# vismaychuriwala/Fast-Image-Editing-with-Generative-Models

Hardware: AMD Instinct MI355X
Metric: PIE-Bench images/sec @1024^2 SSD-1B fp16 4-step (higher is better)
Workload: dtype f16; 1 GPU; ssd-1b fp16 + ControlNet-Canny(full) LCM img2img, num_inference_steps=4, strength=0.5, guidance=1.5, 1024x1024, batch=1 image per GPU, one edit at a time; unet_preset=ssd-1b-A1, controlnet_preset=controlnet-canny-sdxl-full, unet_evals=2, cfg_batch=2, parallelism=image-parallel x1, launch=hipGraph replay, weights=f16

## Files before the change

fast-image-editing-with-generative-models_amd/csrc/gemm_common.h:

```cpp
#pragma once
#include "fie_internal.h"
#include "gemm_addr.h"

namespace fie_gemm {

constexpr int BK = 64;

struct GemmArgs {
    const half_t* A1; int64_t lda1; int K1;
    const half_t* A2; int64_t lda2;
    const half_t* A3; int64_t lda3; int C2x, C3x; int64_t a3_bytes;
    int H, W, Cin, OH, OW, stride, pt, pl, ups;
    const half_t* Wt; int64_t ldw;
    half_t* C; int64_t ldc;
    int M, N, K;
    const half_t* bias;
    const half_t* rowbias; int64_t ld_rowbias; int rows_per_batch;
    const half_t* res; int64_t ldr;
    float scale; int act;
    int nbm, nbn;
    int64_t a1_bytes, a2_bytes, w_bytes;
    int taps2, oscat, opy, opx;
    int64_t w_par_stride;
    int gn_nch, gn_chunk0;
    float* gn_partial; int gn_rows, gn_G, gn_cg;
    const float* w_scale;
    unsigned* stamps;
    int epi_prefetch;
    int probe;
    int splitk; float* sk_slabs; unsigned* sk_tickets;
    float a_scale; int out_f8; float out_inv_scale;
    int order;
    int frag_ld;
    const float* ln_tab; float ln_eps;
    const float* gna_tab; int gna_silu;
};

__device__ __forceinline__ int take_parity(GemmArgs& p, int bid) {
    if (p.oscat != 2) return bid;
    const int par = bid & 3;
    p.opy = par >> 1; p.opx = par & 1; p.pt = 1 - p.opy; p.pl = 1 - p.opx;
    p.Wt += (int64_t)par * p.w_par_stride;
    p.gn_chunk0 = par * ((p.OH * p.OW) >> 5);
    return bid >> 2;
}

__host__ __device__ __forceinline__ ConvGeom conv_geom(const GemmArgs& p, int taps2) { return {p.M, p.OH, p.OW, p.H, p.W, p.Cin, p.stride, p.pt, p.pl, p.ups, taps2}; }

constexpr int kBufRsrcFlags = 0x00020000;
__device__ __forceinline__ __amdgpu_buffer_rsrc_t buf_rsrc(const void* ptr, int64_t bytes) {
    return __builtin_amdgcn_make_buffer_rsrc(const_cast<void*>(ptr), 0, (int)bytes, kBufRsrcFlags);
}

template <class F, int... I>
__device__ __forceinline__ void static_for(F&& f, std::integer_sequence<int, I...>) { (f(std::integral_constant<int, I>{}), ...); }

__device__ __forceinline__ int lds_off(int row, int chunk) { return row * BK + ((chunk ^ (row & 7)) << 3); }

typedef unsigned u32x2 __attribute__((ext_vector_type(2)));

__device__ __forceinline__ float row16_sum(float v) {
    v += __builtin_bit_cast(float, __builtin_amdgcn_update_dpp(0, __builtin_bit_cast(int, v), 0xB1, 0xF, 0xF, true));
    v += __builtin_bit_cast(float, __builtin_amdgcn_update_dpp(0, __builtin_bit_cast(int, v), 0x4E, 0xF, 0xF, true));
    v += __builtin_bit_cast(float, __builtin_amdgcn_update_dpp(0, __builtin_bit_cast(int, v), 0x141, 0xF, 0xF, true));
    v += __builtin_bit_cast(float, __builtin_amdgcn_update_dpp(0, __builtin_bit_cast(int, v), 0x140, 0xF, 0xF, true));
    return v;
}

template <int FM, int FN>
struct EpiPre {
    u32x2 bias[FN];
    u32x2 res[FM][FN];
    bool on;
};
template <int FM, int FN, int WM, int WN>
__device__ __forceinline__ void epilogue_prefetch(const GemmArgs& p, EpiPre<FM, FN>& pre, int m0, int n0, int wm, int wn, int lane) {
    const int fr = lane & 15, fq = lane >> 4;
    const int mrow = m0 + wm * WM + fr, ncol = n0 + wn * WN + fq * 4;
    pre.on = true;
#pragma unroll
    for (int i = 0; i < FN; ++i) pre.bias[i] = (u32x2){0u, 0u};
#pragma unroll
    for (int j = 0; j < FM; ++j)
#pragma unroll
        for (int i = 0; i < FN; ++i) pre.res[j][i] = (u32x2){0u, 0u};
    if (p.bias) {
        const __amdgpu_buffer_rsrc_t rb = buf_rsrc(p.bias, p.N * 2);
#pragma unroll
        for (int i = 0; i < FN; ++i) pre.bias[i] = __builtin_amdgcn_raw_buffer_load_b64(rb, (unsigned)(ncol + i * 16) * 2u, 0, 0);
    }
    if (p.res) {
        const __amdgpu_buffer_rsrc_t rs = buf_rsrc(p.res, (int)(((int64_t)(p.M - 1) * p.ldr + p.N) * 2));
#pragma unroll
        for (int j = 0; j < FM; ++j) {
            const int m = mrow + j * 16;
            const unsigned ro = m < p.M ? (unsigned)m * (unsigned)p.ldr * 2u : 0x80000000u;
#pragma unroll
            for (int i = 0; i < FN; ++i) {
                const int n = ncol + i * 16;
                pre.res[j][i] = __builtin_amdgcn_raw_buffer_load_b64(rs, ro + (n < p.N ? (unsigned)n << 1 : 0xC0000000u), 0, 0);
            }
        }
    }
}

template <int FM, int FN, int WM, int WN>
__device__ __forceinline__ void epilogue_lean(const GemmArgs& p, f32x4 (&acc)[FN][FM], int m0, int n0, int wm, int wn, int lane, const EpiPre<FM, FN>& pre) {
    const int fr = lane & 15, fq = lane >> 4;
    const int mrow = m0 + wm * WM + fr, ncol = n0 + wn * WN + fq * 4;
    const __amdgpu_buffer_rsrc_t rs_c = buf_rsrc(p.C, (int)(((int64_t)(p.M - 1) * p.ldc + p.N) * 2));
#pragma unroll
    for (int j = 0; j < FM; ++j) {
        const int m = mrow + j * 16;
        const unsigned ro = m < p.M ? (unsigned)m * (unsigned)p.ldc * 2u : 0x80000000u;
#pragma unroll
        for (int i = 0; i < FN; ++i) {
            const int n = ncol + i * 16;
            f16x4 b, r, o;
            __builtin_memcpy(&b, &pre.bias[i], 8);
            __builtin_memcpy(&r, &pre.res[j][i], 8);
#pragma unroll
            for (int q = 0; q < 4; ++q) o[q] = (half_t)(acc[i][j][q] + (float)b[q] + (float)r[q]);
            u32x2 bits;
            __builtin_memcpy(&bits, &o, 8);
            __builtin_amdgcn_raw_buffer_store_b64(bits, rs_c, ro + (n < p.N ? (unsigned)n << 1 : 0xC0000000u), 0, 0);
        }
    }
}

template <int FM, int FN, int WM, int WN>
__device__ __forceinline__ void epilogue_lean_scaled(const GemmArgs& p, f32x4 (&acc)[FN][FM], int m0, int n0, int wm, int wn, int lane, const EpiPre<FM, FN>& pre,
                                                     const f32x4 (&ws)[FN]) {
    const int fr = lane & 15, fq = lane >> 4;
    const int mrow = m0 + wm * WM + fr, ncol = n0 + wn * WN + fq * 4;
    const __amdgpu_buffer_rsrc_t rs_c = buf_rsrc(p.C, (int)(((int64_t)(p.M - 1) * p.ldc + p.N) * 2));
#pragma unroll
    for (int j = 0; j < FM; ++j) {
        const int m = mrow + j * 16;
        const unsigned ro = m < p.M ? (unsigned)m * (unsigned)p.ldc * 2u : 0x80000000u;
#pragma unroll
        for (int i = 0; i < FN; ++i) {
            const int n = ncol + i * 16;
            f16x4 b, r, o;
            __builtin_memcpy(&b, &pre.bias[i], 8);
            __builtin_memcpy(&r, &pre.res[j][i], 8);
#pragma unroll
            for (int q = 0; q < 4; ++q) o[q] = (half_t)((acc[i][j][q] * (ws[i][q] * p.a_scale) + (float)b[q]) + (float)r[q]);
            u32x2 bits;
            __builtin_memcpy(&bits, &o, 8);
            __builtin_amdgcn_raw_buffer_store_b64(bits, rs_c, ro + (n < p.N ? (unsigned)n << 1 : 0xC0000000u), 0, 0);
        }
    }
}

__device__ __forceinline__ void ln_dot(const f16x8& f, float& s, float& q) {
    const f16x2 one = {(half_t)1.f, (half_t)1.f};
#pragma unroll
    for (int t = 0; t < 4; ++t) {
        const f16x2 v = {f[2 * t], f[2 * t + 1]};
        s = __builtin_amdgcn_fdot2(v, one, s, false);
        q = __builtin_amdgcn_fdot2(v, v, q, false);
    }
}

template <int FN>
struct LnTab { f32x4 lo[FN], hi[FN]; };
__device__ __forceinline__ void ln_tab_load(const GemmArgs& p, int n, f32x4& lo, f32x4& hi) {
    const __amdgpu_buffer_rsrc_t rt = buf_rsrc(p.ln_tab, p.N * 8);
    lo = __builtin_bit_cast(f32x4, __builtin_amdgcn_raw_buffer_load_b128(rt, (unsigned)n * 8u, 0, 0));
    hi = __builtin_bit_cast(f32x4, __builtin_amdgcn_raw_buffer_load_b128(rt, (unsigned)n * 8u + 16u, 0, 0));
}

template <int FM, int FN, int WM, int WN>
__device__ __forceinline__ void epilogue_lean_ln(const GemmArgs& p, f32x4 (&acc)[FN][FM], int m0, int n0, int wm, int wn, int lane, const LnTab<FN>& tab,
                                                 const float (&mean)[FM], const float (&rstd)[FM]) {
    const int fr = lane & 15, fq = lane >> 4;
    const int mrow = m0 + wm * WM + fr, ncol = n0 + wn * WN + fq * 4;
    const __amdgpu_buffer_rsrc_t rs_c = buf_rsrc(p.C, (int)(((int64_t)(p.M - 1) * p.ldc + p.N) * 2));
#pragma unroll
    for (int j = 0; j < FM; ++j) {
        const int m = mrow + j * 16;
        const unsigned ro = m < p.M ? (unsigned)m * (unsigned)p.ldc * 2u : 0x80000000u;
#pragma unroll
        for (int i = 0; i < FN; ++i) {
            const int n = ncol + i * 16;
            f16x4 o;
            o[0] = (half_t)((acc[i][j][0] - mean[j] * tab.lo[i][0]) * rstd[j] + tab.lo[i][1]);
            o[1] = (half_t)((acc[i][j][1] - mean[j] * tab.lo[i][2]) * rstd[j] + tab.lo[i][3]);
            o[2] = (half_t)((acc[i][j][2] - mean[j] * tab.hi[i][0]) * rstd[j] + tab.hi[i][1]);
            o[3] = (half_t)((acc[i][j][3] - mean[j] * tab.hi[i][2]) * rstd[j] + tab.hi[i][3]);
            u32x2 bits;
            __builtin_memcpy(&bits, &o, 8);
            __builtin_amdgcn_raw_buffer_store_b64(bits, rs_c, ro + (n < p.N ? (unsigned)n << 1 : 0xC0000000u), 0, 0);
        }
    }
}

template <int FM, int FN, int WM, int WN, bool LN = false>
__device__ __forceinline__ void epilogue_geglu_lean(const GemmArgs& p, f32x4 (&acc)[FN][FM], int m0, int n0, int wm, int wn, int lane,
                                                    const float* mean = nullptr, const float* rstd = nullptr) {
    static_assert(FM % 4 == 0, "left-over fragment columns are transposed over four row fragments");
    const int fr = lane & 15, fq = lane >> 4;
    const int mrow = m0 + wm * WM + fr, nbase = n0 + wn * WN;
    const __amdgpu_buffer_rsrc_t rs_c = buf_rsrc(p.C, (int)(((int64_t)(p.M - 1) * p.ldc + (p.N >> 1)) * 2));
    const __amdgpu_buffer_rsrc_t rs_b = buf_rsrc(p.bias, p.bias ? p.N * 2 : 0);
    auto bias4 = [&](int i) { return __builtin_amdgcn_raw_buffer_load_b64(rs_b, (unsigned)(nbase + i * 16 + fq * 4) * 2u, 0, 0); };
    auto pair = [&](const f32x4& a, u32x2 bb) {
        f16x4 b;
        __builtin_memcpy(&b, &bb, 8);
        f16x2 o;
        o[0] = (half_t)((a[0] + (float)b[0]) * fie_gelu(a[1] + (float)b[1]) * 1.0f);
        o[1] = (half_t)((a[2] + (float)b[2]) * fie_gelu(a[3] + (float)b[3]) * 1.0f);
        unsigned bits;
        __builtin_memcpy(&bits, &o, 4);
        return bits;
    };
    auto transpose4 = [](unsigned& r0, unsigned& r1, unsigned& r2, unsigned& r3) {
        asm volatile("s_nop 1\n\tv_permlane16_swap_b32 %0, %1" : "+v"(r0), "+v"(r1));
        asm volatile("s_nop 1\n\tv_permlane16_swap_b32 %0, %1" : "+v"(r2), "+v"(r3));
        asm volatile("s_nop 1\n\tv_permlane32_swap_b32 %0, %1" : "+v"(r0), "+v"(r2));
        asm volatile("s_nop 1\n\tv_permlane32_swap_b32 %0, %1" : "+v"(r1), "+v"(r3));
    };
    auto rowoff = [&](int m) { return m < p.M ? (unsigned)m * (unsigned)p.ldc * 2u : 0x80000000u; };
    struct Tab { f32x4 lo, hi; };
    auto tab4 = [&](int i) { Tab t; ln_tab_load(p, nbase + i * 16 + fq * 4, t.lo, t.hi); return t; };
    auto pair_ln = [&](const f32x4& a, const Tab& t, int j) {
        const float mu = mean[j], rs = rstd[j];
        f16x2 o;
        o[0] = (half_t)(((a[0] - mu * t.lo[0]) * rs + t.lo[1]) * fie_gelu((a[1] - mu * t.lo[2]) * rs + t.lo[3]) * 1.0f);
        o[1] = (half_t)(((a[2] - mu * t.hi[0]) * rs + t.hi[1]) * fie_gelu((a[3] - mu * t.hi[2]) * rs + t.hi[3]) * 1.0f);
        unsigned bits;
        __builtin_memcpy(&bits, &o, 4);
        return bits;
    };
    static_for([&](auto gc) {
        constexpr int I0 = 4 * decltype(gc)::value;
        const int nst = nbase + (I0 + fq) * 16;
        const unsigned co = nst < p.N ? (unsigned)nst : 0xC0000000u;
        if constexpr (LN) {
            const Tab t0 = tab4(I0), t1 = tab4(I0 + 1), t2 = tab4(I0 + 2), t3 = tab4(I0 + 3);
#pragma unroll
            for (int j = 0; j < FM; ++j) {
                unsigned r0 = pair_ln(acc[I0][j], t0, j), r1 = pair_ln(acc[I0 + 1][j], t1, j), r2 = pair_ln(acc[I0 + 2][j], t2, j), r3 = pair_ln(acc[I0 + 3][j], t3, j);
                transpose4(r0, r1, r2, r3);
                const u32x4 v = {r0, r1, r2, r3};
                __builtin_amdgcn_raw_buffer_store_b128(v, rs_c, rowoff(mrow + j * 16) + co, 0, 0);
            }
        } else {
            const u32x2 b0 = bias4(I0), b1 = bias4(I0 + 1), b2 = bias4(I0 + 2), b3 = bias4(I0 + 3);
#pragma unroll
            for (int j = 0; j < FM; ++j) {
                unsigned r0 = pair(acc[I0][j], b0), r1 = pair(acc[I0 + 1][j], b1), r2 = pair(acc[I0 + 2][j], b2), r3 = pair(acc[I0 + 3][j], b3);
                transpose4(r0, r1, r2, r3);
                const u32x4 v = {r0, r1, r2, r3};
                __builtin_amdgcn_raw_buffer_store_b128(v, rs_c, rowoff(mrow + j * 16) + co, 0, 0);
            }
        }
    }, std::make_integer_sequence<int, FN / 4>{});
    static_for([&](auto ic) {
        constexpr int I = FN / 4 * 4 + decltype(ic)::value;
        const int n = nbase + I * 16;
        const unsigned co = n < p.N ? (unsigned)n : 0xC0000000u;
        if constexpr (LN) {
            const Tab t = tab4(I);
#pragma unroll
            for (int h = 0; h < FM / 4; ++h) {
                unsigned r0 = pair_ln(acc[I][4 * h], t, 4 * h), r1 = pair_ln(acc[I][4 * h + 1], t, 4 * h + 1), r2 = pair_ln(acc[I][4 * h + 2], t, 4 * h + 2), r3 = pair_ln(acc[I][4 * h + 3], t, 4 * h + 3);
                transpose4(r0, r1, r2, r3);
                const u32x4 v = {r0, r1, r2, r3};
                __builtin_amdgcn_raw_buffer_store_b128(v, rs_c, rowoff(mrow + (4 * h + fq) * 16) + co, 0, 0);
            }
        } else {
            const u32x2 b = bias4(I);
#pragma unroll
            for (int h = 0; h < FM / 4; ++h) {
                unsigned r0 = pair(acc[I][4 * h], b), r1 = pair(acc[I][4 * h + 1], b), r2 = pair(acc[I][4 * h + 2], b), r3 = pair(acc[I][4 * h + 3], b);
                transpose4(r0, r1, r2, r3);
                const u32x4 v = {r0, r1, r2, r3};
                __builtin_amdgcn_raw_buffer_store_b128(v, rs_c, rowoff(mrow + (4 * h + fq) * 16) + co, 0, 0);
            }
        }
    }, std::make_integer_sequence<int, FN % 4>{});
}

template <int FM, int FN, int WM, int WN, bool BUF = false, bool PATCH = false>
__device__ __forceinline__ void epilogue(const GemmArgs& p, f32x4 (&acc)[FN][FM], int m0, int n0, int wm, int wn, int lane, const EpiPre<FM, FN>* pre = nullptr) {
    const int fr = lane & 15, fq = lane >> 4;
    const bool have_pre = pre != nullptr && pre->on;
    if (p.probe == 4 && p.M > 0) return;
    const bool geglu = p.act == FIE_ACT_GEGLU;
    const int fld = PATCH ? p.frag_ld : 16;
    const int mrow = m0 + wm * FM * fld + fr, ncol = n0 + wn * WN + fq * 4;
    auto col = [&](int i) { const int n = ncol + i * 16; return n < p.N ? n : p.N - 4; };
    auto row = [&](int j) { const int m = mrow + j * fld; return m < p.M ? m : p.M - 1; };
    constexpr unsigned kRowOut = 0x80000000u, kColOut = 0xC0000000u;
    auto coff = [&](int i, bool half) { const int n = ncol + i * 16; return n < p.N ? (unsigned)n << (half ? 0 : 1) : kColOut; };
    auto roff = [&](int j, int64_t ld) { const int m = mrow + j * fld; return m < p.M ? (unsigned)m * (unsigned)ld * 2u : kRowOut; };
    auto coff_row = [&](int j) {
        const int m = mrow + j * fld;
        if (m >= p.M) return kRowOut;
        if (!p.oscat) return (unsigned)m * (unsigned)p.ldc * 2u;
        const OutPixel o = out_pixel(p.OH, p.OW, m);
        return (unsigned)((o.b * 2 * p.OH + 2 * o.oh + p.opy) * (2 * p.OW) + 2 * o.ow + p.opx) * (unsigned)p.ldc * 2u;
    };
    auto as_h4 = [](u32x2 v) { f16x4 h; __builtin_memcpy(&h, &v, 8); return h; };

    if (p.w_scale) {
        const float as = p.a_scale != 0.f ? p.a_scale : 1.f;
#pragma unroll
        for (int i = 0; i < FN; ++i) {
            float4 ws = *reinterpret_cast<const float4*>(p.w_scale + col(i));
            ws.x *= as; ws.y *= as; ws.z *= as; ws.w *= as;
#pragma unroll
            for (int j = 0; j < FM; ++j) { acc[i][j][0] *= ws.x; acc[i][j][1] *= ws.y; acc[i][j][2] *= ws.z; acc[i][j][3] *= ws.w; }
        }
    }
    if (p.bias) {
        f16x4 b[FN];
#pragma unroll
        for (int i = 0; i < FN; ++i) b[i] = have_pre ? as_h4(pre->bias[i]) : *reinterpret_cast<const f16x4*>(p.bias + col(i));
#pragma unroll
        for (int i = 0; i < FN; ++i)
#pragma unroll
            for (int j = 0; j < FM; ++j)
#pragma unroll
                for (int r = 0; r < 4; ++r) acc[i][j][r] += (float)b[i][r];
    }
    if (p.rowbias) {
#pragma unroll
        for (int j = 0; j < FM; ++j) {
            const half_t* rb = p.rowbias + (int64_t)(row(j) / p.rows_per_batch) * p.ld_rowbias;
            f16x4 b[FN];
#pragma unroll
            for (int i = 0; i < FN; ++i) b[i] = *reinterpret_cast<const f16x4*>(rb + col(i));
#pragma unroll
            for (int i = 0; i < FN; ++i)
#pragma unroll
                for (int r = 0; r < 4; ++r) acc[i][j][r] += (float)b[i][r];
        }
    }
    auto sweep = [&](auto f) {
#pragma unroll
        for (int i = 0; i < FN; ++i)
#pragma unroll
            for (int j = 0; j < FM; ++j)
#pragma unroll
                for (int r = 0; r < 4; ++r) acc[i][j][r] = f(acc[i][j][r]) * p.scale;
    };
    if (geglu) {
#pragma unroll
        for (int i = 0; i < FN; ++i)
#pragma unroll
            for (int j = 0; j < FM; ++j) {
                acc[i][j][0] = acc[i][j][0] * fie_gelu(acc[i][j][1]) * p.scale;
                acc[i][j][1] = acc[i][j][2] * fie_gelu(acc[i][j][3]) * p.scale;
            }
    } else if (p.act == FIE_ACT_SILU) sweep([](float x) { return fie_silu(x); });
    else if (p.act == FIE_ACT_GELU) sweep([](float x) { return fie_gelu(x); });
    else if (p.act == FIE_ACT_QUICK_GELU) sweep([](float x) { return fie_qgelu(x); });
    else if (p.scale != 1.f) sweep([](float x) { return x; });
    if (p.res) {
        const __amdgpu_buffer_rsrc_t rs = buf_rsrc(p.res, BUF ? ((int64_t)(p.M - 1) * p.ldr + p.N) * 2 : 0);
#pragma unroll
        for (int j = 0; j < FM; ++j) {
            f16x4 b[FN];
            if (have_pre) {
#pragma unroll
                for (int i = 0; i < FN; ++i) b[i] = as_h4(pre->res[j][i]);
            } else if constexpr (BUF) {
                const unsigned ro = roff(j, p.ldr);
#pragma unroll
                for (int i = 0; i < FN; ++i) b[i] = as_h4(__builtin_amdgcn_raw_buffer_load_b64(rs, ro + coff(i, false), 0, 0));
            } else {
                const half_t* rr = p.res + (int64_t)row(j) * p.ldr;
#pragma unroll
                for (int i = 0; i < FN; ++i) b[i] = *reinterpret_cast<const f16x4*>(rr + col(i));
            }
#pragma unroll
            for (int i = 0; i < FN; ++i)
#pragma unroll
                for (int r = 0; r < 4; ++r) acc[i][j][r] += (float)b[i][r];
            if (FM * FN > 16) __builtin_amdgcn_sched_barrier(0);
        }
    }
    if (p.gn_partial) {
        static_assert(FM % 2 == 0, "row granules are two fragments");
        const int nch = p.gn_nch ? p.gn_nch : p.gn_rows >> 5;
#pragma unroll
        for (int jj = 0; jj < FM / 2; ++jj) {
            float sum[FN], sq[FN];
#pragma unroll
            for (int i = 0; i < FN; ++i) sum[i] = sq[i] = 0.f;
#pragma unroll
            for (int dj = 0; dj < 2; ++dj) {
                const bool ok = mrow + (2 * jj + dj) * fld < p.M;
#pragma unroll
                for (int i = 0; i < FN; ++i)
#pragma unroll
                    for (int r = 0; r < 4; ++r) {
                        const float x = ok ? (float)(half_t)acc[i][2 * jj + dj][r] : 0.f;
                        sum[i] += x;
                        sq[i] += x * x;
                    }
            }
            const int mg = m0 + (wm * FM + 2 * jj) * fld;
            const int b = mg / p.gn_rows, rem = mg - b * p.gn_rows;
            const int chunk = p.gn_chunk0 + (PATCH ? ((rem / p.frag_ld) >> 1) * (p.frag_ld >> 4) + ((rem % p.frag_ld) >> 4) : rem >> 5);
#pragma unroll
            for (int i = 0; i < FN; ++i) {
                const float rs = row16_sum(sum[i]), rq = row16_sum(sq[i]);
                float ts[4], tq[4];
#pragma unroll
                for (int k = 0; k < 4; ++k) {
                    ts[k] = __builtin_bit_cast(float, __builtin_amdgcn_readlane(__builtin_bit_cast(int, rs), 16 * k));
                    tq[k] = __builtin_bit_cast(float, __builtin_amdgcn_readlane(__builtin_bit_cast(int, rq), 16 * k));
                }
                if (p.gn_cg == 16) { ts[0] = (ts[0] + ts[1]) + (ts[2] + ts[3]); tq[0] = (tq[0] + tq[1]) + (tq[2] + tq[3]); }
                else if (p.gn_cg == 8) { ts[0] += ts[1]; tq[0] += tq[1]; ts[1] = ts[2] + ts[3]; tq[1] = tq[2] + tq[3]; }
                const int ngrp = 16 / p.gn_cg;
                const int nfrag = n0 + wn * WN + i * 16;
                if (lane < ngrp && mg < p.M && nfrag + lane * p.gn_cg < p.N) {
                    const float vs = lane == 0 ? ts[0] : lane == 1 ? ts[1] : lane == 2 ? ts[2] : ts[3];
                    const float vq = lane == 0 ? tq[0] : lane == 1 ? tq[1] : lane == 2 ? tq[2] : tq[3];
                    float2* dst = reinterpret_cast<float2*>(p.gn_partial) + ((int64_t)b * nch + chunk) * p.gn_G + nfrag / p.gn_cg + lane;
                    *dst = make_float2(vs, vq);
                }
            }
        }
    }
    if constexpr (BUF) {
        if (p.out_f8) {
            const __amdgpu_buffer_rsrc_t rs8 = buf_rsrc(p.C, (int64_t)(p.M - 1) * p.ldc + (geglu ? p.N >> 1 : p.N));
            const float inv = p.out_inv_scale;
            auto q = [&](float x) { return fie_sat448(x * inv); };
#pragma unroll
            for (int j = 0; j < FM; ++j) {
                const int m = mrow + j * fld;
                const unsigned ro = m < p.M ? (unsigned)m * (unsigned)p.ldc : kRowOut;
#pragma unroll
                for (int i = 0; i < FN; ++i) {
                    const int n = ncol + i * 16;
                    if (geglu) {
                        const int pk = __builtin_amdgcn_cvt_pk_fp8_f32(q(acc[i][j][0]), q(acc[i][j][1]), 0, false);
                        __builtin_amdgcn_raw_buffer_store_b16((unsigned short)(pk & 0xffff), rs8, ro + (n < p.N ? (unsigned)(n >> 1) : kColOut), 0, 0);
                    } else {
                        int pk = __builtin_amdgcn_cvt_pk_fp8_f32(q(acc[i][j][0]), q(acc[i][j][1]), 0, false);
                        pk = __builtin_amdgcn_cvt_pk_fp8_f32(q(acc[i][j][2]), q(acc[i][j][3]), pk, true);
                        __builtin_amdgcn_raw_buffer_store_b32((unsigned)pk, rs8, ro + (n < p.N ? (unsigned)n : kColOut), 0, 0);
                    }
                }
            }
            return;
        }
    }
    const __amdgpu_buffer_rsrc_t rs_c = buf_rsrc(p.C, BUF ? ((int64_t)(p.oscat ? 4 * (int64_t)p.M : p.M) - 1) * p.ldc * 2 + (geglu ? p.N >> 1 : p.N) * 2 : 0);
#pragma unroll
    for (int j = 0; j < FM; ++j) {
        const int m = mrow + j * fld;
        const unsigned ro = coff_row(j);
#pragma unroll
        for (int i = 0; i < FN; ++i) {
            const int n = ncol + i * 16;
            if (geglu) {
                f16x2 o;
                o[0] = (half_t)acc[i][j][0]; o[1] = (half_t)acc[i][j][1];
                if constexpr (BUF) {
                    unsigned bits; __builtin_memcpy(&bits, &o, 4);
                    __builtin_amdgcn_raw_buffer_store_b32(bits, rs_c, ro + coff(i, true), 0, 0);
                } else if (m < p.M && n < p.N) {
                    *reinterpret_cast<f16x2*>(p.C + (int64_t)m * p.ldc + (n >> 1)) = o;
                }
            } else {
                f16x4 o;
#pragma unroll
                for (int r = 0; r < 4; ++r) o[r] = (half_t)acc[i][j][r];
                if constexpr (BUF) {
                    u32x2 bits; __builtin_memcpy(&bits, &o, 8);
                    __builtin_amdgcn_raw_buffer_store_b64(bits, rs_c, ro + coff(i, false), 0, 0);
                } else if (m < p.M && n < p.N) {
                    *reinterpret_cast<f16x4*>(p.C + (int64_t)m * p.ldc + n) = o;
                }
            }
        }
        __builtin_amdgcn_sched_barrier(0);
    }
}

constexpr unsigned kOob = 0x80000000u;

__device__ __forceinline__ void bload16(__amdgpu_buffer_rsrc_t rsrc, half_t* lds_dst, unsigned voff, unsigned soff) {
    __builtin_amdgcn_raw_ptr_buffer_load_lds(rsrc, (__attribute__((address_space(3))) void*)lds_dst, 16, voff, soff, 0, 0);
}

template <int N>
__device__ __forceinline__ void wait_vm() {
    static_assert(N >= 0 && N < 64, "vmcnt is a 6-bit counter");
    asm volatile("s_waitcnt vmcnt(%0)" ::"n"(N) : "memory");
}

template <int N>
__device__ __forceinline__ void wait_vm_barrier() {
    static_assert(N >= 0 && N < 64, "vmcnt is a 6-bit counter");
    asm volatile("s_waitcnt vmcnt(%0)\n\ts_barrier" ::"n"(N) : "memory");
}

template <int FM, int FN, int NW>
__device__ __forceinline__ bool splitk_reduce(const GemmArgs& p, f32x4 (&acc)[FN][FM], int tile, int slice, int tid, void* lds) {
    constexpr int kTile = FM * FN * NW * 64 * 4;
    const int S = p.splitk;
    float* base = p.sk_slabs + (size_t)tile * S * kTile;
    {
        const __amdgpu_buffer_rsrc_t rs = buf_rsrc(base + (size_t)slice * kTile, kTile * 4);
// ... 60 lines not shown
```

fast-image-editing-with-generative-models_amd/csrc/gemm_conv.hip:

```cpp
#include <algorithm>
#include <cstdio>
#include <cstdlib>
#include <cstring>
#include <utility>

#include "gemm_common.h"
#include "gemm_tiles.h"

using namespace fie_gemm;

namespace {

template <int BM, int BN, int MODE>
__global__ __launch_bounds__(256) void gemm_kernel(GemmArgs p) {
    constexpr int WM = BM / 2, WN = BN / 2;
    constexpr int FM = WM / 16, FN = WN / 16;
    constexpr int RA = BM / 32, RW = BN / 32;
    __shared__ __attribute__((aligned(16))) half_t smem[2 * (BM + BN) * BK];

    const int tid = threadIdx.x;
    const int lane = tid & 63, wave = tid >> 6;
    const int wm = wave & 1, wn = wave >> 1;

    const int bid = xcd_remap(blockIdx.x, gridDim.x);
// ... 40 lines not shown
            while (ci >= p.Cin) { ci -= p.Cin; ++tap; }
        } else {
            const bool k1 = k < p.K1;
            const half_t* src = k1 ? p.A1 : p.A2;
            const int64_t ld = k1 ? p.lda1 : p.lda2;
            const int kk = k1 ? k : k - p.K1;
#pragma unroll
            for (int i = 0; i < RA; ++i) {
                const bool ok = a_row[i].ok && k < p.K;
                ra[i] = ok ? *reinterpret_cast<const f16x8*>(src + a_base[i] * ld + kk) : zero8;
            }
        }
#pragma unroll
        for (int i = 0; i < RW; ++i)
            rw[i] = *reinterpret_cast<const f16x8*>(p.Wt + (int64_t)(n0 + r0 + 32 * i) * p.ldw + k);
    };
    auto store_tiles = [&](int buf) {
        half_t* sa = smem + buf * (BM + BN) * BK;
        half_t* sw = sa + BM * BK;
#pragma unroll
        for (int i = 0; i < RA; ++i) *reinterpret_cast<f16x8*>(sa + lds_off(r0 + 32 * i, c8)) = ra[i];
#pragma unroll
        for (int i = 0; i < RW; ++i) *reinterpret_cast<f16x8*>(sw + lds_off(r0 + 32 * i, c8)) = rw[i];
    };

    f32x4 acc[FN][FM];
#pragma unroll
    for (int i = 0; i < FN; ++i)
#pragma unroll
        for (int j = 0; j < FM; ++j) acc[i][j] = (f32x4){0.f, 0.f, 0.f, 0.f};

    const int nk = (p.K + BK - 1) / BK;
    load_tiles(0);
    store_tiles(0);
    __syncthreads();

    const int fr = lane & 15, fq = lane >> 4;
    for (int kt = 0; kt < nk; ++kt) {
        const int buf = kt & 1;
        if (kt + 1 < nk) load_tiles(kt + 1);
        const half_t* sa = smem + buf * (BM + BN) * BK;
        const half_t* sw = sa + BM * BK;
#pragma unroll
        for (int kk = 0; kk < 2; ++kk) {
            f16x8 fw[FN], fa[FM];
#pragma unroll
            for (int i = 0; i < FN; ++i)
                fw[i] = *reinterpret_cast<const f16x8*>(sw + lds_off(wn * WN + i * 16 + fr, kk * 4 + fq));
#pragma unroll
            for (int j = 0; j < FM; ++j)
                fa[j] = *reinterpret_cast<const f16x8*>(sa + lds_off(wm * WM + j * 16 + fr, kk * 4 + fq));
#pragma unroll
            for (int i = 0; i < FN; ++i)
#pragma unroll
                for (int j = 0; j < FM; ++j)
                    acc[i][j] = __builtin_amdgcn_mfma_f32_16x16x32_f16(fw[i], fa[j], acc[i][j], 0, 0, 0);
        }
        if (kt + 1 < nk) store_tiles(buf ^ 1);
        __syncthreads();
    }

    epilogue<FM, FN, WM, WN>(p, acc, m0, n0, wm, wn, lane);
}

template <int NP, int ST>
__device__ __forceinline__ void wait_stage(int later) {
    if (ST >= 3 && later >= 1) wait_vm_barrier<(ST >= 3 ? 1 : 0) * NP>();
    else wait_vm_barrier<0>();
}

template <int OFF>
__device__ __forceinline__ f16x8 lds_read16_async(unsigned addr) {
    f16x8 v;
    asm volatile("ds_read_b128 %0, %1 offset:%2" : "=v"(v) : "v"(addr), "n"(OFF));
    return v;
}
template <int N, int... I>
__device__ __forceinline__ void read_frags(f16x8 (&f)[N], unsigned addr, std::integer_sequence<int, I...>) {
    ((f[I] = lds_read16_async<I * 16 * BK * 2>(addr)), ...);
}

template <int BM, int BN, int ST, int MODE, int NW, bool PF = false, bool STAMP = false, bool ALT = false, int LEAN = 0>
__global__ __launch_bounds__(NW * 64) void gemm3_kernel(GemmArgs p) {
    constexpr bool LNF = LEAN == 2;
    static_assert(!LNF || (MODE == 0 && !STAMP), "LayerNorm fold: GEMM view only");
    static_assert(!ALT || (NW == 8 && MODE == 0 && !PF && !STAMP), "ALT: 8-wave GEMM-view tiles without the fragment prefetch");
    constexpr int WGN = (LEAN == 2 && BM * BN / (NW * 256) <= 16 && (BM / NW) % 16 == 0) ? 1 : (BN / (NW / 2)) % 16 == 0 ? NW / 2 : 1, WGM = NW / WGN;
    constexpr int WM = BM / WGM, WN = BN / WGN;
    constexpr int FM = WM / 16, FN = WN / 16;
    constexpr int NPW = BN / 8;
    constexpr int RA = BM / (8 * NW), RW = (NPW + NW - 1) / NW;
    constexpr int NP = RA + RW;
    constexpr int STAGE = (BM + BN) * BK;
    extern __shared__ __attribute__((aligned(16))) half_t smem[];

    const int tid = threadIdx.x;
    const int lane = tid & 63;
    const int wave = __builtin_amdgcn_readfirstlane(tid >> 6);
    const int wm = wave % WGM, wn = wave / WGM;

    const int bid_all = xcd_remap(blockIdx.x, gridDim.x);
    const int nsplit = p.splitk > 1 ? p.splitk : 1;
    const int tile_all = bid_all / nsplit, slice = bid_all - tile_all * nsplit;
    const int bid = take_parity(p, tile_all);
    const int m0 = (p.order ? bid % p.nbm : bid / p.nbn) * BM;
    const int n0 = (p.order ? bid / p.nbm : bid % p.nbn) * BN;
    const int lr = lane >> 3;
    const int c8 = (lane & 7) ^ lr;

    const int live = p.probe == 1 ? 0 : 1;
    const __amdgpu_buffer_rsrc_t rs_a1 = buf_rsrc(p.A1, (int)p.a1_bytes * live);
    const __amdgpu_buffer_rsrc_t rs_a2 = buf_rsrc(p.A2, (int)p.a2_bytes * live);
    const __amdgpu_buffer_rsrc_t rs_w = buf_rsrc(p.Wt, (int)p.w_bytes * live);
    const __amdgpu_buffer_rsrc_t rs_a3 = buf_rsrc(p.A3, (int)p.a3_bytes * live);
    const int lm0 = p.probe == 2 ? 0 : m0, ln0 = p.probe == 2 ? 0 : n0;

    unsigned a_off1[RA], a_off2[RA];
    unsigned a_off3[RA];
    const ConvGeom g = conv_geom(p, p.taps2);
    ConvRow a_row[RA];
    unsigned a_img[RA];
#pragma unroll
    for (int i = 0; i < RA; ++i) {
        const int m = lm0 + (wave + NW * i) * 8 + lr;
        if (MODE == 2) {
            a_row[i] = conv_row(g, m);
            a_img[i] = (unsigned)a_row[i].b * (unsigned)(p.H * p.W) * (unsigned)p.Cin * 2u;
            a_off1[i] = kOob;
            a_off2[i] = a_row[i].ok ? (unsigned)m * (unsigned)p.lda2 * 2u + c8 * 16u : kOob;
            a_off3[i] = a_row[i].ok ? (unsigned)m * (unsigned)p.lda3 * 2u + c8 * 16u : kOob;
        } else {
            a_off1[i] = a_off2[i] = a_off3[i] = a_img[i] = 0;
            a_row[i] = ConvRow{};
        }
    }
    const unsigned a_base1 = (unsigned)(lm0 + wave * 8 + lr) * (unsigned)p.lda1 * 2u + c8 * 16u;
    const unsigned a_base2 = (unsigned)(lm0 + wave * 8 + lr) * (unsigned)p.lda2 * 2u + c8 * 16u;
    const unsigned a_step1 = (unsigned)(NW * 8) * (unsigned)p.lda1 * 2u, a_step2 = (unsigned)(NW * 8) * (unsigned)p.lda2 * 2u;
    const unsigned w_base = (unsigned)(ln0 + wave * 8 + lr) * (unsigned)p.ldw * 2u + c8 * 16u;
    const unsigned w_step = (unsigned)(NW * 8) * (unsigned)p.ldw * 2u;

    const int csteps = MODE == 2 ? p.Cin / BK : 1;
    const int k1_steps = p.K1 / BK;
    const int nk_all = (p.K + BK - 1) / BK;
    const KSlice ks(nk_all, slice, nsplit, csteps);
    const int kbeg = ks.kbeg, nk = ks.nk;
    const bool ktail = (p.K % BK) != 0;
    int ftap = ks.ftap, cs = ks.cs;
    bool tap_fresh = true;

    const int ntaps = conv_taps(g);
    auto issue = [&](int kt, int stage) {
        half_t* sa = smem + stage * STAGE;
        if (MODE == 2 && ftap >= ntaps) {
            const int e = kt - ntaps * csteps, x2 = p.C2x / BK;
            if (e < x2) {
#pragma unroll
                for (int i = 0; i < RA; ++i) bload16(rs_a2, sa + (wave + NW * i) * 512, a_off2[i], (unsigned)e * (BK * 2));
            } else {
#pragma unroll
                for (int i = 0; i < RA; ++i) bload16(rs_a3, sa + (wave + NW * i) * 512, a_off3[i], (unsigned)(e - x2) * (BK * 2));
            }
        } else if (MODE == 2) {
            if (cs == 0 || tap_fresh) {
                tap_fresh = false;
                const TapYX t = tap_yx(g, ftap);
#pragma unroll
                for (int i = 0; i < RA; ++i)
                    a_off1[i] = conv_inside(g, a_row[i], t.ky, t.kx) ? a_img[i] + (unsigned)conv_index(g, a_row[i], t.ky, t.kx) * (unsigned)p.Cin * 2u + c8 * 16u : kOob;
            }
            const unsigned so = (unsigned)cs * (BK * 2);
#pragma unroll
            for (int i = 0; i < RA; ++i) bload16(rs_a1, sa + (wave + NW * i) * 512, a_off1[i], so);
            if (++cs == csteps) { cs = 0; ++ftap; }
        } else {
            if (ktail && kt == nk_all - 1) {
                const bool in_k = kt * BK + c8 * 8 < p.K;
#pragma unroll
                for (int i = 0; i < RA; ++i) bload16(rs_a1, sa + (wave + NW * i) * 512, in_k ? a_base1 + (unsigned)i * a_step1 : kOob, (unsigned)kt * (BK * 2));
            } else if (kt < k1_steps || k1_steps == 0) {
                const unsigned so = (unsigned)kt * (BK * 2);
#pragma unroll
                for (int i = 0; i < RA; ++i) bload16(rs_a1, sa + (wave + NW * i) * 512, a_base1 + (unsigned)i * a_step1, so);
            } else {
                const unsigned so = (unsigned)(kt - k1_steps) * (BK * 2);
#pragma unroll
                for (int i = 0; i < RA; ++i) bload16(rs_a2, sa + (wave + NW * i) * 512, a_base2 + (unsigned)i * a_step2, so);
            }
        }
    };
    auto issue_w = [&](int kt, int stage) {
        half_t* sw = smem + stage * STAGE + BM * BK;
        const unsigned sow = (unsigned)kt * (BK * 2);
#pragma unroll
        for (int i = 0; i < RW; ++i) {
            const int ii = (NPW % NW == 0 || wave + NW * i < NPW) ? i : 0;
            bload16(rs_w, sw + (wave + NW * ii) * 512, w_base + (unsigned)ii * w_step, sow);
        }
    };

    const int grp = wave >> 2, lw = wave & 3;
    const unsigned alt_a1 = (unsigned)(lm0 + lw * 8 + lr) * (unsigned)p.lda1 * 2u + c8 * 16u, alt_a2 = (unsigned)(lm0 + lw * 8 + lr) * (unsigned)p.lda2 * 2u + c8 * 16u;
    const unsigned alt_sa1 = 32u * (unsigned)p.lda1 * 2u, alt_sa2 = 32u * (unsigned)p.lda2 * 2u;
    const unsigned alt_w = (unsigned)(ln0 + lw * 8 + lr) * (unsigned)p.ldw * 2u + c8 * 16u, alt_sw = 32u * (unsigned)p.ldw * 2u;
    auto issue_alt = [&](int kt, int stage) {
        half_t* sa = smem + stage * STAGE;
        half_t* sw = sa + BM * BK;
        if (ktail && kt == nk_all - 1) {
            const bool in_k = kt * BK + c8 * 8 < p.K;
#pragma unroll
            for (int i = 0; i < 2 * RA; ++i) bload16(rs_a1, sa + (lw + 4 * i) * 512, in_k ? alt_a1 + (unsigned)i * alt_sa1 : kOob, (unsigned)kt * (BK * 2));
        } else if (kt < k1_steps || k1_steps == 0) {
            const unsigned so = (unsigned)kt * (BK * 2);
#pragma unroll
            for (int i = 0; i < 2 * RA; ++i) bload16(rs_a1, sa + (lw + 4 * i) * 512, alt_a1 + (unsigned)i * alt_sa1, so);
        } else {
            const unsigned so = (unsigned)(kt - k1_steps) * (BK * 2);
#pragma unroll
            for (int i = 0; i < 2 * RA; ++i) bload16(rs_a2, sa + (lw + 4 * i) * 512, alt_a2 + (unsigned)i * alt_sa2, so);
        }
        const unsigned sow = (unsigned)kt * (BK * 2);
#pragma unroll
        for (int i = 0; i < 2 * RW; ++i) bload16(rs_w, sw + (lw + 4 * i) * 512, alt_w + (unsigned)i * alt_sw, sow);
    };

    f32x4 acc[FN][FM];
#pragma unroll
    for (int i = 0; i < FN; ++i)
#pragma unroll
        for (int j = 0; j < FM; ++j) acc[i][j] = (f32x4){0.f, 0.f, 0.f, 0.f};

    EpiPre<FM, FN> pre;
    pre.on = false;
    LnTab<(LNF && FM * FN <= 16) ? FN : 1> ln_pre;
    if constexpr (FM * FN <= 16) {
        if constexpr (LNF) {
        } else if (LEAN || (nsplit == 1 && p.epi_prefetch)) epilogue_prefetch<FM, FN, WM, WN>(p, pre, m0, n0, wm, wn, lane);
    }
    constexpr int LJ = LNF ? FM : 1;
    float ln_s[LJ], ln_q[LJ];
#pragma unroll
    for (int t = 0; t < LJ; ++t) ln_s[t] = ln_q[t] = 0.f;
    auto ln_unit = [&](auto jc, auto tc, const f16x8& f) {
        constexpr int j = decltype(jc)::value, t = decltype(tc)::value;
        const f16x2 one = {(half_t)1.f, (half_t)1.f};
        const f16x2 v = {f[2 * t], f[2 * t + 1]};
        ln_s[j] = __builtin_amdgcn_fdot2(v, one, ln_s[j], false);
        ln_q[j] = __builtin_amdgcn_fdot2(v, v, ln_q[j], false);
    };
    auto ln_slice = [&](auto ic, auto nic, auto j0c, auto cntc, const f16x8* fa) {
        if constexpr (LNF) {
            constexpr int I = decltype(ic)::value, NI = decltype(nic)::value, J0 = decltype(j0c)::value, U = 4 * decltype(cntc)::value;
            constexpr int u0 = I * U / NI, u1 = (I + 1) * U / NI;
            static_for([&](auto uc) {
                constexpr int u = u0 + decltype(uc)::value;
                ln_unit(std::integral_constant<int, J0 + u / 4>{}, std::integral_constant<int, u % 4>{}, fa[u / 4]);
            }, std::make_integer_sequence<int, u1 - u0>{});
        }
    };
    auto ln_pin = [&]() {
        if constexpr (LNF) {
#pragma unroll
            for (int t = 0; t < LJ; ++t) asm volatile("" : "+v"(ln_s[t]), "+v"(ln_q[t]));
        }
    };
    using c0_t = std::integral_constant<int, 0>;

#pragma unroll
    for (int s = 0; s < ST - 1; ++s)
        if (s < nk) { issue(kbeg + s, s); issue_w(kbeg + s, s); }

    const int fr = lane & 15, fq = lane >> 4;
    int stage = 0, fill = ST - 1;
    auto frags = [&](f16x8* fw, f16x8* fa, const half_t* sa, int kk) {
        const half_t* sw = sa + BM * BK;
#pragma unroll
        for (int i = 0; i < FN; ++i) fw[i] = *reinterpret_cast<const f16x8*>(sw + lds_off(wn * WN + i * 16 + fr, kk * 4 + fq));
#pragma unroll
        for (int j = 0; j < FM; ++j) fa[j] = *reinterpret_cast<const f16x8*>(sa + lds_off(wm * WM + j * 16 + fr, kk * 4 + fq));
    };
    auto mfmas = [&](const f16x8* fw, const f16x8* fa) {
        if (NW == 8) __builtin_amdgcn_s_setprio(1);
        static_for([&](auto ic) {
            constexpr int i = decltype(ic)::value;
#pragma unroll
            for (int j = 0; j < FM; ++j) acc[i][j] = __builtin_amdgcn_mfma_f32_16x16x32_f16(fw[i], fa[j], acc[i][j], 0, 0, 0);
            ln_slice(ic, std::integral_constant<int, FN>{}, std::integral_constant<int, 0>{}, std::integral_constant<int, FM>{}, fa);
        }, std::make_integer_sequence<int, FN>{});
        if (NW == 8) __builtin_amdgcn_s_setprio(0);
    };
    unsigned seg[12] = {0, 0, 0, 0, 0, 0, 0, 0, 0, 0, 0, 0}, tprev = 0;
    auto stamp = [&](int i) {
        if constexpr (STAMP) {
            __builtin_amdgcn_sched_barrier(0);
            const unsigned t = (unsigned)__builtin_amdgcn_s_memtime();
            seg[i] += t - tprev;
            tprev = t;
            __builtin_amdgcn_sched_barrier(0);
        }
    };
    if constexpr (STAMP) tprev = seg[9] = (unsigned)__builtin_amdgcn_s_memtime();
    if constexpr (PF) {
        static_assert(FM + FN <= 15, "lgkmcnt is a 4-bit counter");
        const unsigned lds0 = (unsigned)(uintptr_t)(__attribute__((address_space(3))) half_t*)smem;
        unsigned a_rd[2], w_rd[2];
#pragma unroll
        for (int kk = 0; kk < 2; ++kk) {
            a_rd[kk] = lds0 + 2u * (unsigned)lds_off(wm * WM + fr, kk * 4 + fq);
            w_rd[kk] = lds0 + 2u * (unsigned)(BM * BK + lds_off(wn * WN + fr, kk * 4 + fq));
        }
        f16x8 fw0[FN], fa0[FM], fw1[FN], fa1[FM];
        auto reads = [&](f16x8 (&fw)[FN], f16x8 (&fa)[FM], int st, int kk) {
            const unsigned so = (unsigned)st * (STAGE * 2);
            read_frags(fw, w_rd[kk] + so, std::make_integer_sequence<int, FN>{});
            read_frags(fa, a_rd[kk] + so, std::make_integer_sequence<int, FM>{});
        };
        auto landed = [&](f16x8 (&fw)[FN], f16x8 (&fa)[FM]) {
#pragma unroll
            for (int i = 0; i < FN; ++i) asm volatile("" : "+v"(fw[i]));
#pragma unroll
            for (int j = 0; j < FM; ++j) asm volatile("" : "+v"(fa[j]));
        };
        wait_stage<NP, ST>(min(ST - 2, nk - 1));
        reads(fw0, fa0, 0, 0);
        for (int kt = 0; kt < nk; ++kt) {
            stamp(kt == 0 ? 7 : 0);
            const bool more = kt + ST - 1 < nk && p.probe != 3;
            if (more) { issue(kbeg + kt + ST - 1, fill); if (NW != 8) issue_w(kbeg + kt + ST - 1, fill); }
            ln_pin();
            reads(fw1, fa1, stage, 1);
            asm volatile("s_waitcnt lgkmcnt(%0)" ::"n"(FM + FN) : "memory");
            landed(fw0, fa0);
            mfmas(fw0, fa0);
            if (more && NW == 8) issue_w(kbeg + kt + ST - 1, fill);
            stage = stage + 1 == ST ? 0 : stage + 1;
            fill = fill + 1 == ST ? 0 : fill + 1;
            asm volatile("s_waitcnt lgkmcnt(0)" ::: "memory");
            landed(fw1, fa1);
            if (kt + 1 < nk) {
                wait_stage<NP, ST>(min(kt + ST - 1, nk - 1) - (kt + 1));
                ln_pin();
                reads(fw0, fa0, stage, 0);
            }
            mfmas(fw1, fa1);
        }
    } else
    for (int kt = 0; kt < nk; ++kt) {
        const int later = min(kt + ST - 2, nk - 1) - kt;
        if constexpr (ALT && ST >= 3) {
            if (later >= 1 && kt >= ST - 1 && (kt & 1) != grp) wait_vm_barrier<2 * NP>();
            else wait_vm_barrier<0>();
        } else
        wait_stage<NP, ST>(later);
        stamp(kt == 0 ? 7 : 0);
        const bool more = kt + ST - 1 < nk;
        const half_t* sa = smem + stage * STAGE;
#pragma unroll
        for (int kk = 0; kk < 2; ++kk) {
            if (more && p.probe != 3) {
                if constexpr (ALT) {
                    if (kk == 0 && ((kt + ST - 1) & 1) == grp) issue_alt(kbeg + kt + ST - 1, fill);
                } else {
                    if (kk == 0) { issue(kbeg + kt + ST - 1, fill); if (NW != 8) issue_w(kbeg + kt + ST - 1, fill); }
                    else if (NW == 8) issue_w(kbeg + kt + ST - 1, fill);
                }
            }
            stamp(1 + 3 * kk);
            if constexpr (FM * FN > 16) {
                constexpr int HM = FM / 2;
                const half_t* sw = sa + BM * BK;
                f16x8 fw[FN];
#pragma unroll
                for (int i = 0; i < FN; ++i) fw[i] = *reinterpret_cast<const f16x8*>(sw + lds_off(wn * WN + i * 16 + fr, kk * 4 + fq));
#pragma unroll
                for (int jh = 0; jh < 2; ++jh) {
                    f16x8 fa[HM];
#pragma unroll
                    for (int j = 0; j < HM; ++j) fa[j] = *reinterpret_cast<const f16x8*>(sa + lds_off(wm * WM + (jh * HM + j) * 16 + fr, kk * 4 + fq));
                    __builtin_amdgcn_s_setprio(1);
                    static_for([&](auto ic) {
                        constexpr int i = decltype(ic)::value;
#pragma unroll
                        for (int j = 0; j < HM; ++j) acc[i][jh * HM + j] = __builtin_amdgcn_mfma_f32_16x16x32_f16(fw[i], fa[j], acc[i][jh * HM + j], 0, 0, 0);
                        if (jh == 0) ln_slice(ic, std::integral_constant<int, FN>{}, c0_t{}, std::integral_constant<int, HM>{}, fa);
                        else ln_slice(ic, std::integral_constant<int, FN>{}, std::integral_constant<int, HM>{}, std::integral_constant<int, HM>{}, fa);
                    }, std::make_integer_sequence<int, FN>{});
                    __builtin_amdgcn_s_setprio(0);
                }
            } else {
                f16x8 fw[FN], fa[FM];
                frags(fw, fa, sa, kk);
                if constexpr (STAMP) asm volatile("s_waitcnt lgkmcnt(0)" ::: "memory");
                stamp(2 + 3 * kk);
                mfmas(fw, fa);
                stamp(3 + 3 * kk);
            }
        }
        stage = stage + 1 == ST ? 0 : stage + 1;
        fill = fill + 1 == ST ? 0 : fill + 1;
    }
    stamp(11);
    float ln_mean[LNF ? FM : 1], ln_rstd[LNF ? FM : 1];
    if constexpr (LNF && FM * FN <= 16) {
#pragma unroll
        for (int i = 0; i < FN; ++i) ln_tab_load(p, n0 + wn * WN + i * 16 + (lane >> 4) * 4, ln_pre.lo[i], ln_pre.hi[i]);
    }
    if constexpr (LNF) {
        const float inv_k = 1.f / (float)p.K;
#pragma unroll
        for (int j = 0; j < FM; ++j) {
            float sx = ln_s[j], sq = ln_q[j];
            sx += __shfl_xor(sx, 16); sx += __shfl_xor(sx, 32);
            sq += __shfl_xor(sq, 16); sq += __shfl_xor(sq, 32);
            const float mu = sx * inv_k;
            ln_mean[j] = mu;
            ln_rstd[j] = rsqrtf(fmaxf(sq * inv_k - mu * mu, 0.f) + p.ln_eps);
        }
    }
    if constexpr (FM * FN <= 16 && !LEAN) {
        if (nsplit > 1 && !splitk_reduce<FM, FN, NW>(p, acc, tile_all, slice, tid, smem)) return;
    }
    if constexpr (LNF && FM * FN > 16) {
        epilogue_geglu_lean<FM, FN, WM, WN, true>(p, acc, m0, n0, wm, wn, lane, ln_mean, ln_rstd);
    } else if constexpr (LNF) {
        epilogue_lean_ln<FM, FN, WM, WN>(p, acc, m0, n0, wm, wn, lane, ln_pre, ln_mean, ln_rstd);
    } else
    if constexpr (FM * FN > 16) {
        if (p.act == FIE_ACT_GEGLU && p.epi_prefetch && !p.rowbias && !p.res && p.scale == 1.f && !p.gn_partial && !p.out_f8 && !p.w_scale && !p.oscat && p.probe == 0) {
            epilogue_geglu_lean<FM, FN, WM, WN>(p, acc, m0, n0, wm, wn, lane);
        } else {
        static_for([&](auto cc) {
            constexpr int C = decltype(cc)::value;
            epilogue<FM, 2, WM, WN, true>(p, reinterpret_cast<f32x4(&)[2][FM]>(acc[2 * C]), m0, n0 + 32 * C, wm, wn, lane);
        }, std::make_integer_sequence<int, FN / 2>{});
        if constexpr (FN & 1)
            epilogue<FM, 1, WM, WN, true>(p, reinterpret_cast<f32x4(&)[1][FM]>(acc[FN - 1]), m0, n0 + 16 * (FN - 1), wm, wn, lane);
        }
    } else {
        if constexpr (LEAN == 1) epilogue_lean<FM, FN, WM, WN>(p, acc, m0, n0, wm, wn, lane, pre);
        else epilogue<FM, FN, WM, WN, true>(p, acc, m0, n0, wm, wn, lane, &pre);
    }
    if constexpr (STAMP) {
        asm volatile("s_waitcnt vmcnt(0)" ::: "memory");
        stamp(8);
        seg[10] = tprev;
        if (p.stamps && lane == 0) {
#pragma unroll
            for (int i = 0; i < 12; ++i) p.stamps[((size_t)bid * NW + wave) * 12 + i] = seg[i];
        }
    }
}

enum Family { kGeneric, kRing, kPhased, kHalo, kHaloEdge, kThin };
enum : unsigned { kSplitK = 1, kStamps = 2, kGemmOnly = 4, kLnFold = 8, kPF = 16, kAlt = 32 };
using LaunchFn = int (*)(fie_ctx*, GemmArgs&, dim3 grid);
struct Tile {
    int code, bm, bn;
    Family family;
    const char* name;
    unsigned flags;
    int w8, x8;
    LaunchFn gemm, conv, ln;
    hipError_t (*attr)();
};

template <int BM, int BN, int ST, int NW, unsigned F = 0>
struct RingTile {
    static constexpr bool PF = F & kPF, STAMP = F & kStamps, ALT = F & kAlt;
    static constexpr int lds = ST * (BM + BN) * BK * (int)sizeof(half_t);
    template <int MODE>
    static constexpr bool has_lean = MODE == 0 && !STAMP && BM * BN / (NW * 64) <= 64;
    static_assert(!((F & kLnFold) && STAMP) && !((F & kSplitK) && (STAMP || BM * BN / (NW * 64) > 64)), "no LN fold or split-K with stamps; split-K on <= 16 fragments per lane");
    template <int MODE, int LEAN>
    static constexpr auto kernel() { return &gemm3_kernel<BM, BN, ST, MODE, NW, PF, STAMP, ALT, LEAN>; }
    template <int MODE, bool LN = false>
    static int launch(fie_ctx* ctx, GemmArgs& a, dim3 grid) {
        auto k = kernel<MODE, LN ? 2 : 0>();
        if constexpr (!LN && has_lean<MODE>) {
            if (a.epi_prefetch && a.splitk <= 1 && !a.rowbias && a.act == FIE_ACT_NONE && a.scale == 1.f && !a.gn_partial && !a.out_f8 && !a.w_scale && !a.oscat &&
                a.probe == 0)
                k = kernel<MODE, 1>();
        }
        fie_launch(ctx, k, grid, dim3(NW * 64), lds, a);
        FIE_LAUNCH_CHECK();
        return FIE_OK;
    }
    static hipError_t attr() {
        hipError_t e = hipSuccess;
        auto set = [&](auto* k) { if (e == hipSuccess) e = hipFuncSetAttribute(reinterpret_cast<const void*>(k), hipFuncAttributeMaxDynamicSharedMemorySize, lds); };
        set(kernel<0, 0>());
        if constexpr (has_lean<0>) set(kernel<0, 1>());
        if constexpr (!(F & kGemmOnly)) set(kernel<2, 0>());
        if constexpr (F & kLnFold) set(kernel<0, 2>());
        return e;
    }
    static constexpr Tile row(int code, const char* name, int w8, int x8) {
        Tile t = {code, BM, BN, kRing, name, F, w8, x8, &launch<0>, nullptr, nullptr, &attr};
        if constexpr (!(F & kGemmOnly)) t.conv = &launch<2>;
        if constexpr (F & kLnFold) t.ln = &launch<0, true>;
        return t;
    }
};

template <int BM, int BN, int MODE>
int launch_generic(fie_ctx* ctx, GemmArgs& a, dim3 grid) {
    fie_launch(ctx, (gemm_kernel<BM, BN, MODE>), grid, dim3(256), 0, a);
    FIE_LAUNCH_CHECK();
    return FIE_OK;
}
template <int BM, int BN>
constexpr Tile generic_row(int code, int w8, int x8) { return {code, BM, BN, kGeneric, "gemm_kernel", 0, w8, x8, &launch_generic<BM, BN, 0>, &launch_generic<BM, BN, 1>}; }
template <int CONV, int VARIANT>
int launch_phased(fie_ctx* ctx, GemmArgs& a, dim3) { return fie_launch_gemm8(ctx, a, CONV, VARIANT); }
template <int VARIANT>
int launch_halo(fie_ctx* ctx, GemmArgs& a, dim3) { return fie_launch_conv_halo(ctx, a, VARIANT); }
int launch_thin(fie_ctx* ctx, GemmArgs& a, dim3) { return fie_launch_conv_thin(ctx, a); }

constexpr Tile kTiles[] = {
    generic_row<128, 128>(1, 62, 43),
    generic_row<128, 64>(2, 42, 42),
    generic_row<64, 64>(3, 43, 43),
    RingTile<128, 64, 3, 4, kSplitK | kLnFold>::row(42, "gemm3_kernel", 42, 42),
    RingTile<64, 64, 3, 4, kSplitK>::row(43, "gemm3_kernel", 43, 43),
    RingTile<128, 64, 2, 4, kSplitK>::row(44, "gemm3_kernel", 42, 42),
    RingTile<64, 64, 2, 4, kSplitK>::row(46, "gemm3_kernel", 43, 43),
    RingTile<128, 96, 3, 4, kSplitK>::row(47, "gemm3_kernel", 62, 47),
    RingTile<128, 80, 3, 4, kSplitK>::row(48, "gemm3_kernel", 62, 0),
    RingTile<128, 128, 3, 8, kSplitK>::row(51, "gemm3_kernel", 62, 51),
    RingTile<128, 128, 2, 8, kSplitK>::row(52, "gemm3_kernel", 52, 52),
    RingTile<192, 128, 2, 8, kSplitK>::row(54, "gemm3_kernel", 54, 54),
    RingTile<256, 256, 2, 8>::row(61, "gemm3_kernel", 62, 62),
    RingTile<256, 128, 3, 8, kSplitK>::row(62, "gemm3_kernel", 62, 62),
    RingTile<256, 320, 2, 8, kGemmOnly>::row(63, "gemm3_kernel", 62, 63),
    RingTile<256, 320, 2, 8, kGemmOnly | kAlt | kLnFold>::row(64, "gemm3_kernel", 62, 63),
    RingTile<128, 128, 3, 8, kPF | kSplitK>::row(95, "gemm3_kernel+prefetch", 62, 51),
    RingTile<256, 128, 3, 8, kPF | kSplitK | kLnFold>::row(96, "gemm3_kernel+prefetch", 62, 62),
    RingTile<256, 128, 3, 8, kStamps>::row(97, "gemm3_kernel+prefetch", 62, 0),
    RingTile<256, 128, 3, 8, kPF | kStamps>::row(98, "gemm3_kernel+prefetch", 62, 0),
    RingTile<128, 64, 3, 4, kStamps>::row(94, "gemm3_kernel+prefetch", 62, 0),
    {81, 256, 256, kPhased, "gemm8_kernel", 0, 62, 62, &launch_phased<0, 0>, &launch_phased<1, 0>},
    {82, 256, 256, kPhased, "gemm8_kernel", 0, 62, 0, &launch_phased<0, 1>, &launch_phased<1, 1>},
    {71, 256, 128, kHalo, "conv_halo_kernel", 0, 62, 0, nullptr, &launch_halo<0>},
    {73, 256, 128, kHalo, "conv_halo_kernel", kStamps, 62, 0, nullptr, &launch_halo<1>},
    {72, 256, 128, kHalo, "conv_halo2_kernel", 0, 62, 0, nullptr, &launch_halo<2>},
    {74, 256, 128, kHalo, "conv_halo2_kernel", kStamps, 62, 0, nullptr, &launch_halo<4>},
    {76, 256, 128, kHalo, "conv_halo2_kernel", 0, 62, 0, nullptr, &launch_halo<5>},
    {78, 256, 128, kHaloEdge, "conv_halo2_kernel+edge", 0, 62, 0, nullptr, &launch_halo<6>},
    {77, 64, 16, kThin, "conv_thin_kernel", 0, 62, 0, &launch_thin, &launch_thin},
};
constexpr const Tile* find_tile(int code) {
    for (const Tile& t : kTiles)
        if (t.code == code) return &t;
    return nullptr;
}
constexpr bool is_family(int code, Family f) { return find_tile(code) && find_tile(code)->family == f; }

constexpr int kCandF16[] = {43, 46, 42, 44, 51, 52, 54, 96, 81, 63, 47, 48, 64, 72, 78};
constexpr int kCandW8[] = {43, 42, 62, 52, 54};
constexpr int kCandX8[] = {43, 42, 47, 51, 52, 54, 62, 63};
struct SplitCand { int code, per_cu; };
constexpr SplitCand kSplitF16[] = {{96, 1}, {95, 1}, {47, 1}, {54, 2}, {52, 2}};
constexpr SplitCand kSplitX8[] = {{62, 1}, {51, 1}, {47, 1}, {54, 2}, {52, 2}};

template <size_t N>
constexpr bool f8_built(const fie_f8_tile (&built)[N], int code) {
    const Tile* t = find_tile(code);
    for (const fie_f8_tile& b : built)
        if (t && b.code == code && b.bm == t->bm && b.bn == t->bn) return true;
    return false;
}
constexpr int table_error() {
    for (const Tile& t : kTiles) {
        int n = 0;
        for (const Tile& u : kTiles) n += u.code == t.code;
        if (n != 1) return 1;
        if (!f8_built(kFieW8Tiles, t.w8) || (t.x8 && !f8_built(kFieX8Tiles, t.x8))) return 2;
        if ((t.flags & kSplitK) && t.family != kRing) return 3;
        if ((!t.conv && !(t.flags & kGemmOnly)) || (!t.gemm && t.family != kHalo && t.family != kHaloEdge)) return 4;
    }
    for (int c : kCandF16) if (!find_tile(c)) return 5;
// ... 8 lines not shown
template <int MODE>
int heuristic_code(const fie_ctx* ctx, const GemmArgs& a, bool dma_ok) {
    auto blocks = [&](int bm, int bn) { return (int64_t)((a.M + bm - 1) / bm) * ((a.N + bn - 1) / bn); };
    const int64_t cus = ctx->num_cus;
    const int64_t b256 = blocks(256, 256), b62 = blocks(256, 128), b51 = blocks(128, 128), b42 = blocks(128, 64);
    int code;
    if (!dma_ok) {
        code = b42 >= cus ? 2 : 3;
    } else if (MODE == 1 && fie_conv_halo_ok(a) && 4 * (int64_t)(a.M / 256) * ((a.N + 127) / 128) >= 3 * cus && a.C2x + a.C3x <= 4 * BK &&
               std::find(std::begin(ctx->tune_exclude), std::end(ctx->tune_exclude), 72) == std::end(ctx->tune_exclude)) {
        code = 72;
    } else if (MODE == 1 && fie_conv_halo_edge_ok(a) && 4 * fie_conv_halo_patches(a) * ((a.N + 127) / 128) >= 3 * cus && a.C2x + a.C3x <= 4 * BK &&
               std::find(std::begin(ctx->tune_exclude), std::end(ctx->tune_exclude), 78) == std::end(ctx->tune_exclude)) {
        code = 78;
    } else if (MODE == 1) {
        if (!a.A2 && ((b256 >= cus && (a.N % 256 == 0 || (a.N % 128 != 0 && a.K >= 5760))) ||
            (a.N % 256 == 0 && a.K >= 8192 && 2 * b256 >= cus))) code = 81;
        else if (a.N % 128 == 0 && b62 >= 150) code = 96;
        else if (a.N % 128 == 0 && a.K >= 5760 && b51 >= 100) code = 51;
        else if (2 * b42 < 3 * cus) code = 43;
        else code = 42;
    } else if (MODE == 0 && a.N % 320 == 0 && a.N >= 5120 && 4 * blocks(256, 320) >= 3 * cus) {
        code = 64;
    } else if (a.N % 256 == 0 && a.K >= 4096 && b256 >= cus) {
        code = 81;
    } else if (a.N % 128 == 0 && b62 >= 150 && (a.N >= 1536 || a.K >= 2048 || a.M >= 16384)) {
        code = 96;
    } else if (a.N >= 2048 && a.K >= 1024 && b51 >= cus) {
        code = 51;
    } else if (a.K <= 640 && a.N <= 640) {
        code = 43;
    } else if (b42 >= cus * 7 / 2 || a.K >= 4096 || (a.K >= 1024 && b42 >= cus)) {
        code = 42;
    } else {
        code = 43;
    }
    return code;
}

constexpr int64_t kSkTickets = 4096;

inline int splitk_fit(const fie_ctx* ctx, const GemmArgs& a, const Tile& t, int want) {
    const int bm = t.bm, bn = t.bn;
    if (want <= 1 || !(t.flags & kSplitK) || !ctx->sk_ws || !ctx->splitk_mode || (a.w_scale && a.a_scale == 0.f)) return 1;
    const int64_t tiles = (int64_t)((a.M + bm - 1) / bm) * ((a.N + bn - 1) / bn) * (a.oscat == 2 ? 4 : 1);
    const int nk = (a.K + BK - 1) / BK / (a.a_scale != 0.f ? 2 : 1);
    int s = want;
    while (s > 1 && (nk / s < 4 || tiles > kSkTickets || (int64_t)(kSkTickets * 4 + tiles * s * bm * bn * 4) > ctx->sk_bytes)) --s;
    return s;
}

template <int MODE>
int run_code(fie_ctx* ctx, GemmArgs& a, int code, int order, bool dma_ok, int split = 1) {
    const Tile* t = find_tile(code);
    FIE_REQUIRE(t != nullptr, "unknown tile code %d", code);
    const Family fam = t->family;
    FIE_REQUIRE(fam == kGeneric || fam == kThin || dma_ok, "tile code %d: shape not eligible for the LDS-DMA kernels (operands >= 2 GiB, Cin %% 64 != 0, or A = [A1 | A2] with K1 %% 64 != 0 or K %% 64 != 0)", code);
    FIE_REQUIRE(!(a.taps2 && (fam == kGeneric || a.w_scale)), "tile code %d: the 2x2 parity convs run on the f16 LDS-DMA kernels only", code);
    FIE_REQUIRE(!(MODE == 1 && a.A2 && (fam == kGeneric || fam == kPhased || a.w_scale)), "tile code %d: conv + 1x1 side inputs run on the f16 ring kernels and the halo-resident kernel (72) only", code);
    FIE_REQUIRE(!(fam == kHalo && (MODE != 1 || !dma_ok || !fie_conv_halo_ok(a))), "tile code %d (halo-resident conv): stride-1 same-size 3x3 conv with H, W %% 16 == 0, Cin %% 64 == 0, f16 weights only", code);
    FIE_REQUIRE(!(fam == kHaloEdge && (MODE != 1 || !dma_ok || !fie_conv_halo_edge_ok(a))), "tile code 78 (halo-resident conv, edge patches): stride-1 same-size 3x3 conv with H or W %% 16 != 0, "
                "Cin %% 64 == 0, Cin >= 128, N %% 64 == 0, f16 weights, no activation / scale / GroupNorm sums only");
    if (order < 0) {
        const int64_t nbm = (a.M + t->bm - 1) / t->bm, nbn = (a.N + t->bn - 1) / t->bn;
        const int64_t per_xcd = (nbm * nbn + 7) / 8;
        const double a_tile = (double)t->bm * a.K * 2 * (MODE == 1 ? 1.0 / 9 : 1.0), w_tile = (double)t->bn * a.K * 2;
        auto fabric = [&](int64_t fast, int64_t slow, double fast_tile, double slow_tile) {
            const int64_t rows = (per_xcd + fast - 1) / fast;
            return (double)(rows < slow ? rows : slow) * slow_tile + (double)(per_xcd < fast ? per_xcd : fast) * fast_tile;
        };
        order = fabric(nbm, nbn, a_tile, w_tile) < fabric(nbn, nbm, w_tile, a_tile) ? 1 : 0;
    }
    const bool x8 = a.w_scale && a.a_scale != 0.f;
    if (x8) {
        FIE_REQUIRE(dma_ok && !a.A2 && !a.taps2, "fp8 activations: plain GEMM / 3x3 conv views on the LDS-DMA kernels only");
        FIE_REQUIRE(t->x8 != 0, "tile code %d has no fp8-activation kernel", code);
        t = find_tile(t->x8);
        if (MODE == 1 && (t->flags & kGemmOnly)) t = find_tile(62);
    } else if (a.w_scale) {
        FIE_REQUIRE(dma_ok, "fp8 weights: shape not eligible for the LDS-DMA kernels (operands >= 2 GiB, Cin %% 64 != 0, or A = [A1 | A2] with K1 %% 64 != 0 or K %% 64 != 0)");
        t = find_tile(t->w8);
    }
    code = t->code;
    a.nbm = (a.M + t->bm - 1) / t->bm;
    a.nbn = (a.N + t->bn - 1) / t->bn;
    split = splitk_fit(ctx, a, *t, split);
    a.splitk = split;
    a.sk_tickets = static_cast<unsigned*>(ctx->sk_ws);
    a.sk_slabs = reinterpret_cast<float*>(static_cast<char*>(ctx->sk_ws) + kSkTickets * 4);
    a.order = order;
    a.probe = ctx->gemm_probe;
    a.epi_prefetch = ctx->epi_prefetch;
    a.stamps = (t->flags & kStamps) ? ctx->gemm_stamps : nullptr;
    if (x8) snprintf(ctx->last_kernel, sizeof(ctx->last_kernel), "gemm3x8_kernel<%dx%d> (gemm, fp8 activations x fp8 weights, tile code %d)", t->bm, t->bn, code);
    else if (a.w_scale) snprintf(ctx->last_kernel, sizeof(ctx->last_kernel), "gemm3w8_kernel<%dx%d> (%s, fp8 weights, tile code %d)", t->bm, t->bn, MODE == 1 ? "conv3x3" : "gemm", code);
    else snprintf(ctx->last_kernel, sizeof(ctx->last_kernel), "%s<%dx%d> (%s, tile code %d)", t->name, t->bm, t->bn, MODE == 1 ? "conv3x3" : "gemm", code);
    if (split > 1) snprintf(ctx->last_kernel + strlen(ctx->last_kernel) - 1, 24, ", split-K %d)", split);
    if (ctx->oplog) {
        char rebuild[256];
        snprintf(rebuild, sizeof(rebuild), " | b=%d pad=%d C2=%d C3=%d K1=%d parity=%d w8=%d bias=%d rowbias=%d rpb=%d res=%d act=%d scale=%.9g gn=%d gnrows=%d f8out=%d ln=%d gna=%d",
                 MODE == 1 ? a.M / (a.OH * a.OW) : 1, MODE == 1 && !a.taps2 && a.pt == 0 ? 1 : 0, a.C2x, a.C3x, a.K1, a.taps2, a.w_scale ? (a.a_scale != 0.f ? 2 : 1) : 0,
                 a.bias != nullptr, a.rowbias != nullptr, a.rowbias ? a.rows_per_batch : 0, a.res != nullptr, a.act, (double)a.scale, a.gn_partial ? a.gn_G : 0,
                 a.gn_partial ? a.gn_rows : 0, a.out_f8, a.ln_tab != nullptr, a.gna_tab != nullptr);
        if (MODE == 1)
            FIE_DESC(ctx, "conv M=%d N=%d K=%d in=%dx%dx%d s%d u%d%s%s code=%d flop=%.0f%s", a.M * (a.oscat == 2 ? 4 : 1), a.N, a.K, a.H, a.W, a.Cin, a.stride, a.ups,
                     a.taps2 ? " up2x-parity" : "", a.A2 ? " +1x1" : "", code + 10000 * (split > 1 ? split : 0), 2.0 * a.M * a.N * a.K * (a.oscat == 2 ? 4 : 1), rebuild);
        else
            FIE_DESC(ctx, "gemm M=%d N=%d K=%d act=%d%s%s%s code=%d flop=%.0f%s", a.M, a.N, a.K, a.act, a.res ? " +res" : "", a.ln_tab ? " +ln" : "", a.w_scale ? (a.a_scale != 0.f ? " a8w8" : " w8") : "",
                     code + 10000 * (split > 1 ? split : 0), 2.0 * a.M * a.N * a.K, rebuild);
    }
    if (x8) return fie_launch_gemm_x8(ctx, a, code, MODE == 1);
    if (a.w_scale) return fie_launch_gemm_w8(ctx, a, MODE == 1, code);
    const dim3 grid((unsigned)(a.nbm * a.nbn * (a.oscat == 2 ? 4 : 1) * split));
    if (a.ln_tab) {
        FIE_REQUIRE(MODE == 0 && t->ln && split == 1, "LayerNorm-folded GEMM: tile code %d not built for it", code);
        FIE_REQUIRE((code == 64) == (a.act == FIE_ACT_GEGLU), "LayerNorm-folded GEMM: GEGLU runs on tile 64 and nothing else does (code %d, act %d)", code, a.act);
        return t->ln(ctx, a, grid);
    }
    const LaunchFn fn = MODE == 1 ? t->conv : t->gemm;
    FIE_REQUIRE(fn != nullptr, "tile code %d (%dx%d%s) is built for the GEMM view only", code, t->bm, t->bn, (t->flags & kAlt) ? ", alternating refill" : "");
    return fn(ctx, a, grid);
}

constexpr size_t kFlushBytes = 384u << 20;

template <int MODE>
std::vector<int> tune_candidates(const fie_ctx* ctx, const GemmArgs& a, int guess) {
    static const bool use47 = !(getenv("FIE_TUNE_47") && getenv("FIE_TUNE_47")[0] == '0');
    std::vector<int> out;
    auto blocks = [&](int bm, int bn) { return (int64_t)((a.M + bm - 1) / bm) * ((a.N + bn - 1) / bn); };
    const bool x8 = a.w_scale && a.a_scale != 0.f;
    const int* cand = x8 ? kCandX8 : a.w_scale ? kCandW8 : kCandF16;
    const size_t ncand = x8 ? std::size(kCandX8) : a.w_scale ? std::size(kCandW8) : std::size(kCandF16);
    auto excluded = [&](int c) {
        for (int e : ctx->tune_exclude)
            if (e == c) return e != 0;
        return false;
    };
    for (size_t i = 0; i < ncand; ++i) {
        const int c = cand[i];
        if (c == guess || excluded(c)) continue;
        if ((c == 43 || c == 46) && blocks(64, 64) > 64 * ctx->num_cus) continue;
        if ((c == 81 || c == 96 || c == 62) && 2 * blocks(256, 128) < ctx->num_cus) continue;
        if ((c == 63 || c == 64) && (MODE != 0 || a.N % 320 != 0 || 2 * blocks(256, 320) < ctx->num_cus)) continue;
        if (c == 47 && !use47) continue;
        if (c == 48 && (a.N % 80 != 0 || blocks(128, 80) > 2 * ctx->num_cus)) continue;
        if (x8 && MODE == 1 && c == 63) continue;
        if (x8 && (c == 62 || c == 51) && 2 * blocks(c == 62 ? 256 : 128, 128) < ctx->num_cus) continue;
        if (c == 81 && MODE == 1 && a.A2) continue;
        if (c == 72 && (MODE != 1 || !fie_conv_halo_ok(a) || 2 * (int64_t)(a.M / 256) * ((a.N + 127) / 128) < ctx->num_cus)) continue;
        if (c == 78 && (MODE != 1 || !fie_conv_halo_edge_ok(a) || 2 * fie_conv_halo_patches(a) * ((a.N + 127) / 128) < ctx->num_cus)) continue;
        out.push_back(c);
    }
    if ((!a.w_scale || x8) && ctx->sk_ws && ctx->splitk_mode && !excluded(10000)) {
        for (const SplitCand& c : x8 ? kSplitX8 : kSplitF16) {
            if (excluded(c.code)) continue;
            const Tile& t = *find_tile(c.code);
            const int64_t nb = blocks(t.bm, t.bn) * (a.oscat == 2 ? 4 : 1);
            if (nb >= ctx->num_cus * c.per_cu) continue;
            for (int sp = 2; sp <= 4; ++sp) {
                if (nb * sp > (int64_t)ctx->num_cus * c.per_cu * 21 / 20) break;
                if (splitk_fit(ctx, a, t, sp) != sp) continue;
                out.push_back(c.code + 10000 * sp);
            }
        }
    }
    return out;
}

template <int MODE>
int autotune(fie_ctx* ctx, GemmArgs& a, int guess, bool dma_ok) {
    const size_t bytes = (size_t)a.M * (a.oscat ? 4 : 1) * (size_t)a.ldc * sizeof(half_t);
    if (bytes > ctx->tune_bytes) {
        if (ctx->tune_buf) (void)hipFree(ctx->tune_buf);
        ctx->tune_buf = nullptr;
        ctx->tune_bytes = 0;
        if (hipMalloc(&ctx->tune_buf, bytes) != hipSuccess) { (void)hipGetLastError(); return guess; }
        ctx->tune_bytes = bytes;
    }
    if (!ctx->tune_flush && hipMalloc(&ctx->tune_flush, kFlushBytes) != hipSuccess) { (void)hipGetLastError(); ctx->tune_flush = nullptr; return guess; }
    hipEvent_t e0, e1;
    if (hipEventCreate(&e0) != hipSuccess || hipEventCreate(&e1) != hipSuccess) return guess;
    (void)hipDeviceSynchronize();
    GemmArgs t = a;
    t.C = static_cast<half_t*>(ctx->tune_buf);
    auto time_of = [&](int code, int split = 1) -> float {
        float ms[7];
        for (int rep = -1; rep < 7; ++rep) {
            (void)hipMemsetAsync(ctx->tune_flush, rep & 1, kFlushBytes, ctx->stream);
            if ((size_t)a.a1_bytes <= kFlushBytes) (void)hipMemcpyAsync(ctx->tune_flush, a.A1, (size_t)a.a1_bytes, hipMemcpyDeviceToDevice, ctx->stream);
            if (a.A2 && a.A2 != a.A1 && (size_t)a.a2_bytes <= kFlushBytes) (void)hipMemcpyAsync(ctx->tune_flush, a.A2, (size_t)a.a2_bytes, hipMemcpyDeviceToDevice, ctx->stream);
            (void)hipEventRecord(e0, ctx->stream);
            if (run_code<MODE>(ctx, t, code, -1, dma_ok, split) != FIE_OK) return 1e30f;
            (void)hipEventRecord(e1, ctx->stream);
            if (hipEventSynchronize(e1) != hipSuccess) return 1e30f;
            if (rep >= 0) (void)hipEventElapsedTime(&ms[rep], e0, e1);
        }
        std::sort(ms, ms + 7);
        return (ms[2] + ms[3] + ms[4]) / 3.f;
    };
    static const bool verbose = getenv("FIE_TUNE_VERBOSE") && getenv("FIE_TUNE_VERBOSE")[0] == '1';
    const float t_guess = time_of(guess);
    if (verbose) fprintf(stderr, "[fie tune] %s M=%d N=%d K=%d: rule %d %.1f us", MODE == 1 ? "conv" : "gemm", a.M, a.N, a.K, guess, t_guess * 1e3f);
    int best = guess;
    float t_best = t_guess * 0.97f;
    for (const int enc : tune_candidates<MODE>(ctx, a, guess)) {
        const int c = enc % 10000, sp = enc / 10000 > 1 ? enc / 10000 : 1;
        const float tc = time_of(c, sp);
        if (verbose) {
            if (sp > 1) fprintf(stderr, ", %d/s%d %.1f", c, sp, tc * 1e3f);
            else fprintf(stderr, ", %d %.1f", c, tc * 1e3f);
        }
        if (tc < t_best) { t_best = tc; best = enc; }
    }
    if (verbose) fprintf(stderr, " -> %d\n", best);
    (void)hipEventDestroy(e0);
    (void)hipEventDestroy(e1);
    return best;
}

template <int MODE>
int launch(fie_ctx* ctx, GemmArgs& a) {
    const int64_t c_span = ((int64_t)((a.oscat ? 4 * (int64_t)a.M : a.M) - 1) * a.ldc + a.N) * 2, r_span = a.res ? ((int64_t)(a.M - 1) * a.ldr + a.N) * 2 : 0;
    const bool dma_ok = a.a1_bytes < (1ll << 31) && a.a2_bytes < (1ll << 31) && a.w_bytes < (1ll << 31) && c_span <= (1ll << 30) && r_span <= (1ll << 30) &&
                        (MODE == 1 ? a.Cin % (a.a_scale != 0.f ? 2 * BK : BK) == 0 : (a.K1 == a.K || (a.K1 % BK == 0 && a.K % BK == 0)));
    FIE_REQUIRE(!(MODE == 1 && a.A2 && !dma_ok), "conv + 1x1 side inputs: tensors too large for the LDS-DMA kernels");
    if (MODE == 1 && a.gna_tab) {
        FIE_REQUIRE(dma_ok && fie_conv_halo_gna_ok(a), "fie_conv3x3_gn_nhwc_f16: shape / epilogue not built for the fused form (ask fie_conv3x3_gn_ok first)");
        return run_code<MODE>(ctx, a, 72, -1, dma_ok, 1);
    }
    if (MODE == 0 && a.ln_tab) {
        FIE_REQUIRE(dma_ok, "fie_gemm_ln_f16: operands too large for the LDS-DMA kernels");
        auto blocks = [&](int bm, int bn) { return (int64_t)((a.M + bm - 1) / bm) * ((a.N + bn - 1) / bn); };
        int code;
        if (a.act == FIE_ACT_GEGLU) code = 64;
        else if (a.N % 128 == 0 && blocks(256, 128) >= 150 && (a.N >= 1536 || a.M >= 16384)) code = 96;
        else code = 42;
        const int forced = ctx->force_tile % 1000;
        if (forced && find_tile(forced) && find_tile(forced)->ln && (forced == 64) == (a.act == FIE_ACT_GEGLU)) code = forced;
        return run_code<MODE>(ctx, a, code, -1, dma_ok, 1);
    }
    int code = heuristic_code<MODE>(ctx, a, dma_ok);
    int order = -1;
    int split = 1;
    bool pinned = false;
    auto decode = [&](int v) { split = v / 10000 > 1 ? v / 10000 : 1; v %= 10000; order = v >= 2000 ? 1 : v >= 1000 ? 0 : -1; code = v % 1000; };
    for (int i = 0; i < ctx->n_overrides; ++i) {
        const fie_tile_override& o = ctx->overrides[i];
        if (o.mode == (MODE == 1) && o.M == a.M && o.N == a.N && o.K == a.K) { decode(o.code); pinned = true; }
    }
    if (ctx->force_tile) { decode(ctx->force_tile); pinned = true; }
    const fie_tune_key key{MODE, a.M, a.N, a.K, a.K1, MODE == 1 ? a.stride * 2 + a.ups + 8 * a.taps2 + 16 * (a.A2 != nullptr) + 32 * (a.A3 != nullptr) : 0, a.w_scale == nullptr ? 0 : a.a_scale != 0.f ? 2 : 1};
    auto note_candidates = [&](int rule, const std::vector<int>& cands) {
        char line[256];
        int n = snprintf(line, sizeof(line), "%s M=%d N=%d K=%d K1=%d geom=%d w8=%d rule=%d cands=", MODE == 1 ? "conv" : "gemm", key.M, key.N, key.K, key.K1, key.geom, key.w8, rule);
        for (size_t i = 0; i < cands.size() && n < (int)sizeof(line) - 8; ++i) n += snprintf(line + n, sizeof(line) - n, i ? ",%d" : "%d", cands[i]);
        ctx->tune_cands->push_back(line);
    };
    if (MODE == 1 && !pinned && !ctx->gemm_probe && fie_conv_thin_ok(a) && a.M >= 131072 &&
        std::find(std::begin(ctx->tune_exclude), std::end(ctx->tune_exclude), 77) == std::end(ctx->tune_exclude)) {
        if (ctx->tune_cands) note_candidates(77, {});
        return run_code<MODE>(ctx, a, 77, 0, dma_ok, 1);
    }
    if (ctx->tune_cands && !pinned && !ctx->gemm_probe) {
        note_candidates(code, dma_ok ? tune_candidates<MODE>(ctx, a, code) : std::vector<int>{});
        return run_code<MODE>(ctx, a, code, order, dma_ok, split);
    }
    if (ctx->autotune && !pinned && dma_ok && !ctx->gemm_probe) {
        auto it = ctx->tuned.find(key);
        if (it != ctx->tuned.end()) {
            decode(it->second);
        } else if (ctx->autotune == 1 && !ctx->recording) {
            hipStreamCaptureStatus cap = hipStreamCaptureStatusNone;
            if (hipStreamIsCapturing(ctx->stream, &cap) == hipSuccess && cap == hipStreamCaptureStatusNone) {
                const int best = autotune<MODE>(ctx, a, code, dma_ok);
                ctx->tuned[key] = best;
                decode(best);
            }
        }
    }
    if (MODE == 1 && !pinned && ((is_family(code, kHalo) && !fie_conv_halo_ok(a)) || (is_family(code, kHaloEdge) && !fie_conv_halo_edge_ok(a)))) {
        code = heuristic_code<MODE>(ctx, a, dma_ok);
        order = -1;
        split = 1;
    }
    return run_code<MODE>(ctx, a, code, order, dma_ok, split);
}

int check_epilogue(const char* who, int N, int64_t ldc, const void* res, int64_t ldr, int act) {
    FIE_REQUIRE(act >= FIE_ACT_NONE && act <= FIE_ACT_GEGLU, "%s: unknown act %d", who, act);
    FIE_REQUIRE(N % 4 == 0, "%s: N=%d must be a multiple of 4", who, N);
    FIE_REQUIRE(ldc % 4 == 0 || act == FIE_ACT_GEGLU, "%s: ldc=%lld must be a multiple of 4", who, (long long)ldc);
    FIE_REQUIRE(!res || ldr % 4 == 0, "%s: ldr=%lld must be a multiple of 4", who, (long long)ldr);
    FIE_REQUIRE(!(res && act == FIE_ACT_GEGLU), "%s: GEGLU epilogue takes no residual", who);
    return FIE_OK;
}

__global__ void pack_rows_kernel(const half_t* src, int64_t ld_src, int N, int K, half_t* dst, int64_t ldw, int Npad,
                                 int interleave2) {
    const int64_t total = (int64_t)Npad * ldw;
    for (int64_t i = blockIdx.x * (int64_t)blockDim.x + threadIdx.x; i < total; i += (int64_t)gridDim.x * blockDim.x) {
        const int n = (int)(i / ldw), k = (int)(i - (int64_t)n * ldw);
        half_t v = (half_t)0.f;
        if (n < N && k < K) {
            const int sn = interleave2 ? ((n & 1) ? (N / 2 + (n >> 1)) : (n >> 1)) : n;
            v = src[(int64_t)sn * ld_src + k];
        }
        dst[i] = v;
    }
}

__global__ void pack_conv_kernel(const half_t* src, int Cout, int Cin, int cin_pad, half_t* dst, int64_t ldw, int Npad) {
    const int64_t total = (int64_t)Npad * ldw;
    for (int64_t i = blockIdx.x * (int64_t)blockDim.x + threadIdx.x; i < total; i += (int64_t)gridDim.x * blockDim.x) {
        const int n = (int)(i / ldw), k = (int)(i - (int64_t)n * ldw);
        half_t v = (half_t)0.f;
        const int tap = k / cin_pad, ci = k - tap * cin_pad;
        if (n < Cout && tap < 9 && ci < Cin) v = src[((int64_t)n * Cin + ci) * 9 + tap];
        dst[i] = v;
    }
}

}

int fie_gemm_init(void) {
    hipError_t e = hipSuccess;
    for (const Tile& t : kTiles)
        if (e == hipSuccess && t.attr) e = t.attr();
    if (e != hipSuccess) {
        fie_set_error("gemm: hipFuncSetAttribute failed: %s", hipGetErrorString(e));
        return FIE_EHIP;
    }
    return FIE_OK;
}

extern "C" {

int fie_debug_force_tile(fie_ctx* ctx, int t) {
    FIE_REQUIRE(ctx != nullptr, "fie_debug_force_tile: ctx is NULL");
    ctx->force_tile = t;
    return FIE_OK;
}

int fie_debug_tile_override(fie_ctx* ctx, const char* spec) {
    FIE_REQUIRE(ctx != nullptr, "fie_debug_tile_override: ctx is NULL");
    ctx->n_overrides = 0;
    if (!spec) return 0;
    const char* q = spec;
    while (*q && ctx->n_overrides < 32) {
        fie_tile_override o;
        int used = 0;
        if (sscanf(q, "%d,%d,%d,%d=%d%n", &o.mode, &o.M, &o.N, &o.K, &o.code, &used) != 5) break;
        ctx->overrides[ctx->n_overrides++] = o;
        q += used;
        if (*q == ';') ++q;
    }
    return ctx->n_overrides;
}

int fie_debug_gemm_probe(fie_ctx* ctx, int mode) {
    FIE_REQUIRE(ctx != nullptr && mode >= 0 && mode <= 4, "fie_debug_gemm_probe: bad argument");
    ctx->gemm_probe = mode;
    return FIE_OK;
}

int fie_debug_epilogue_prefetch(fie_ctx* ctx, int on) {
    FIE_REQUIRE(ctx != nullptr, "fie_debug_epilogue_prefetch: ctx is NULL");
    ctx->epi_prefetch = on ? 1 : 0;
// ... 50 lines not shown
}

int fie_gemm_autotune_report(fie_ctx* ctx, char* buf, int cap) {
    FIE_REQUIRE(ctx != nullptr && buf != nullptr && cap > 0, "fie_gemm_autotune_report: bad argument");
    int n = 0;
    buf[0] = 0;
    for (const auto& kv : ctx->tuned) {
        const fie_tune_key& k = kv.first;
        const int w = snprintf(buf + n, (size_t)(cap - n), "%s M=%d N=%d K=%d K1=%d geom=%d w8=%d -> %d\n", k.mode ? "conv" : "gemm", k.M, k.N, k.K, k.K1, k.geom, k.w8, kv.second);
        if (w < 0 || w >= cap - n) break;
        n += w;
    }
    return (int)ctx->tuned.size();
}

int fie_gemm_autotune_load(fie_ctx* ctx, const char* text) {
    FIE_REQUIRE(ctx != nullptr && text != nullptr, "fie_gemm_autotune_load: NULL argument");
    int n = 0;
    for (const char* q = text; *q;) {
        char kind[8] = "";
        fie_tune_key k{};
        int code = 0;
        if (sscanf(q, "%7s M=%d N=%d K=%d K1=%d geom=%d w8=%d -> %d", kind, &k.M, &k.N, &k.K, &k.K1, &k.geom, &k.w8, &code) == 8 &&
            (!strcmp(kind, "gemm") || !strcmp(kind, "conv")) && code > 0) {
            k.mode = kind[0] == 'c';
            ctx->tuned[k] = code;
            ++n;
        }
        const char* nl = strchr(q, '\n');
        if (!nl) break;
        q = nl + 1;
    }
    return n;
}

int fie_debug_gemm_stamps(fie_ctx* ctx, void* buf) {
    FIE_REQUIRE(ctx != nullptr, "fie_debug_gemm_stamps: NULL ctx");
    ctx->gemm_stamps = static_cast<unsigned*>(buf);
    return FIE_OK;
}

const char* fie_debug_last_gemm_kernel(fie_ctx* ctx) { return ctx ? ctx->last_kernel : ""; }

int fie_debug_tune_candidates(fie_ctx* ctx, int on) {
    FIE_REQUIRE(ctx != nullptr, "fie_debug_tune_candidates: ctx is NULL");
    delete ctx->tune_cands;
    ctx->tune_cands = on ? new std::vector<std::string>() : nullptr;
    return FIE_OK;
}

int64_t fie_debug_tune_candidates_read(fie_ctx* ctx, char* buf, int64_t cap) {
    if (!ctx || !ctx->tune_cands) return 0;
    int64_t n = 0;
    for (const std::string& l : *ctx->tune_cands) n += (int64_t)l.size() + 1;
    if (buf && cap > n) {
        char* q = buf;
        for (const std::string& l : *ctx->tune_cands) { memcpy(q, l.data(), l.size()); q += l.size(); *q++ = '\n'; }
        *q = 0;
    }
    return n;
}

struct GnTarget { float* partial; int64_t rows; int groups; };
static GnTarget grab_gn_target(fie_ctx* ctx) {
    GnTarget t = {nullptr, 0, 0};
    if (ctx) { t = {ctx->gn_target, ctx->gn_target_rows, ctx->gn_target_groups}; ctx->gn_target = nullptr; }
    return t;
}

static int take_gn_target(const char* who, const GnTarget& t, GemmArgs& a) {
    if (!t.partial) return FIE_OK;
    a.gn_partial = t.partial;
    a.gn_rows = (int)t.rows;
    a.gn_G = t.groups;
    FIE_REQUIRE(a.act != FIE_ACT_GEGLU && a.N % a.gn_G == 0, "%s: GroupNorm statistics: N=%d not divisible into %d groups", who, a.N, a.gn_G);
    a.gn_cg = a.N / a.gn_G;
    FIE_REQUIRE(a.gn_cg == 4 || a.gn_cg == 8 || a.gn_cg == 16, "%s: GroupNorm statistics need 4, 8 or 16 channels per group (got %d)", who, a.gn_cg);
    FIE_REQUIRE(a.gn_rows > 0 && a.gn_rows % 32 == 0 && a.M % a.gn_rows == 0, "%s: GroupNorm statistics: M=%d rows, %d per image (must be a multiple of 32)", who, a.M, a.gn_rows);
    return FIE_OK;
}

static int gemm_impl(const char* who, fie_ctx* ctx, const void* A1, int64_t lda1, int K1, const void* A2, int64_t lda2,
                     const void* Wpacked, int64_t ldw, const float* w_scale, void* C, int64_t ldc, int M, int N, int K, const void* bias,
                     const void* rowbias, int64_t ld_rowbias, int rows_per_batch, const void* residual, int64_t ldr, float scale, int act) {
    const GnTarget gn = grab_gn_target(ctx);
    FIE_REQUIRE(ctx && A1 && Wpacked && C, "%s: NULL ctx/A1/W/C", who);
    FIE_REQUIRE(M > 0 && N > 0 && K > 0, "%s: bad shape M=%d N=%d K=%d", who, M, N, K);
    FIE_REQUIRE(K % 8 == 0 && K1 % 8 == 0 && K1 > 0 && K1 <= K, "%s: K=%d K1=%d must be multiples of 8", who, K, K1);
    FIE_REQUIRE(lda1 % 8 == 0 && lda1 >= K1, "%s: lda1=%lld invalid", who, (long long)lda1);
    FIE_REQUIRE(K1 == K || (A2 && lda2 % 8 == 0 && lda2 >= K - K1), "%s: A2/lda2 invalid for K1 < K", who);
    FIE_REQUIRE(ldw % BK == 0 && ldw >= K, "%s: ldw=%lld must be a multiple of 64 covering K", who, (long long)ldw);
    FIE_REQUIRE(!rowbias || rows_per_batch > 0, "%s: rowbias needs rows_per_batch", who);
    if (int e = check_epilogue(who, N, ldc, residual, ldr, act)) return e;
    GemmArgs a = {};
    a.A1 = (const half_t*)A1; a.lda1 = lda1; a.K1 = K1; a.A2 = (const half_t*)A2; a.lda2 = lda2;
    a.Wt = (const half_t*)Wpacked; a.ldw = ldw; a.w_scale = w_scale; a.C = (half_t*)C; a.ldc = ldc; a.M = M; a.N = N; a.K = K;
    a.bias = (const half_t*)bias; a.rowbias = (const half_t*)rowbias; a.ld_rowbias = ld_rowbias;
    a.rows_per_batch = rows_per_batch > 0 ? rows_per_batch : 1;
    a.res = (const half_t*)residual; a.ldr = ldr; a.scale = scale; a.act = act;
    a.a1_bytes = ((int64_t)(M - 1) * lda1 + K1) * 2;
    a.a2_bytes = A2 ? ((int64_t)(M - 1) * lda2 + (K - K1)) * 2 : 0;
    a.w_bytes = fie_roundup(N, 128) * ldw * (w_scale ? 1 : 2);
    if (int rc = take_gn_target(who, gn, a)) return rc;
    return launch<0>(ctx, a);
}

int fie_gemm_f16(fie_ctx* ctx, const void* A1, int64_t lda1, int K1, const void* A2, int64_t lda2,
                 const void* Wpacked, int64_t ldw, void* C, int64_t ldc, int M, int N, int K, const void* bias,
                 const void* rowbias, int64_t ld_rowbias, int rows_per_batch, const void* residual, int64_t ldr,
                 float scale, int act) {
    return gemm_impl("fie_gemm_f16", ctx, A1, lda1, K1, A2, lda2, Wpacked, ldw, nullptr, C, ldc, M, N, K, bias, rowbias, ld_rowbias,
                     rows_per_batch, residual, ldr, scale, act);
}

int fie_gemm_ln_f16(fie_ctx* ctx, const void* X, int64_t ldx, const void* Wfolded, int64_t ldw, const float* ln_tab, float eps, void* C, int64_t ldc,
                    int M, int N, int K, int act) {
    const GnTarget gn = grab_gn_target(ctx);
    (void)gn;
    FIE_REQUIRE(ctx && X && Wfolded && ln_tab && C, "fie_gemm_ln_f16: NULL ctx/X/W/ln_tab/C");
    FIE_REQUIRE(M > 0 && N > 0 && K > 0 && K % BK == 0, "fie_gemm_ln_f16: bad shape M=%d N=%d K=%d (K must be a multiple of 64)", M, N, K);
    FIE_REQUIRE(ldx % 8 == 0 && ldx >= K, "fie_gemm_ln_f16: ldx=%lld invalid", (long long)ldx);
    FIE_REQUIRE(ldw % BK == 0 && ldw >= K, "fie_gemm_ln_f16: ldw=%lld must be a multiple of 64 covering K", (long long)ldw);
    FIE_REQUIRE(act == FIE_ACT_NONE || (act == FIE_ACT_GEGLU && N % 320 == 0), "fie_gemm_ln_f16: act %d (none, or GEGLU with N %% 320 == 0)", act);
    FIE_REQUIRE(eps > 0.f, "fie_gemm_ln_f16: eps must be positive");
    if (int e = check_epilogue("fie_gemm_ln_f16", N, ldc, nullptr, 0, act)) return e;
    GemmArgs a = {};
    a.A1 = (const half_t*)X; a.lda1 = ldx; a.K1 = K;
    a.Wt = (const half_t*)Wfolded; a.ldw = ldw; a.C = (half_t*)C; a.ldc = ldc; a.M = M; a.N = N; a.K = K;
    a.rows_per_batch = 1; a.scale = 1.f; a.act = act;
    a.a1_bytes = ((int64_t)(M - 1) * ldx + K) * 2;
    a.w_bytes = fie_roundup(N, 128) * ldw * 2;
    a.ln_tab = ln_tab; a.ln_eps = eps;
    return launch<0>(ctx, a);
}

int fie_gemm_w8_f16(fie_ctx* ctx, const void* A1, int64_t lda1, int K1, const void* A2, int64_t lda2, const void* W8packed,
                    int64_t ldw, const float* w_scale, void* C, int64_t ldc, int M, int N, int K, const void* bias, const void* rowbias,
                    int64_t ld_rowbias, int rows_per_batch, const void* residual, int64_t ldr, float scale, int act) {
    FIE_REQUIRE(w_scale != nullptr, "fie_gemm_w8_f16: w_scale is NULL");
    return gemm_impl("fie_gemm_w8_f16", ctx, A1, lda1, K1, A2, lda2, W8packed, ldw, w_scale, C, ldc, M, N, K, bias, rowbias, ld_rowbias,
                     rows_per_batch, residual, ldr, scale, act);
}

int fie_gemm_x8_f16(fie_ctx* ctx, const void* A8, int64_t lda, const void* W8packed, int64_t ldw, const float* w_scale, float a_scale, void* C, int64_t ldc,
                    int M, int N, int K, const void* bias, const void* rowbias, int64_t ld_rowbias, int rows_per_batch, const void* residual, int64_t ldr,
                    float scale, int act, int out_f8, float out_inv_scale) {
    const char* who = "fie_gemm_x8_f16";
    (void)grab_gn_target(ctx);
    FIE_REQUIRE(ctx && A8 && W8packed && w_scale && C, "%s: NULL ctx/A/W/scale/C", who);
    FIE_REQUIRE(M > 0 && N > 0 && K > 0 && K % 16 == 0 && lda % 16 == 0 && lda >= K, "%s: bad shape M=%d N=%d K=%d lda=%lld (K, lda %% 16 == 0)", who, M, N, K, (long long)lda);
    FIE_REQUIRE(ldw % 128 == 0 && ldw >= K, "%s: ldw=%lld must be a multiple of 128 covering K", who, (long long)ldw);
    FIE_REQUIRE(a_scale > 0.f && (!out_f8 || out_inv_scale > 0.f), "%s: scales must be positive", who);
    FIE_REQUIRE(!rowbias || rows_per_batch > 0, "%s: rowbias needs rows_per_batch", who);
    if (int e = check_epilogue(who, N, out_f8 ? 4 : ldc, residual, ldr, act)) return e;
    FIE_REQUIRE(!out_f8 || (ldc % 4 == 0 && !residual), "%s: fp8 output: ldc %% 4 == 0, no residual", who);
    GemmArgs a = {};
    a.A1 = (const half_t*)A8; a.lda1 = lda; a.K1 = K;
    a.Wt = (const half_t*)W8packed; a.ldw = ldw; a.w_scale = w_scale; a.a_scale = a_scale; a.C = (half_t*)C; a.ldc = ldc; a.M = M; a.N = N; a.K = K;
    a.bias = (const half_t*)bias; a.rowbias = (const half_t*)rowbias; a.ld_rowbias = ld_rowbias;
    a.rows_per_batch = rows_per_batch > 0 ? rows_per_batch : 1;
    a.res = (const half_t*)residual; a.ldr = ldr; a.scale = scale; a.act = act;
    a.out_f8 = out_f8; a.out_inv_scale = out_inv_scale;
    a.a1_bytes = (int64_t)(M - 1) * lda + K;
    a.w_bytes = fie_roundup(N, 128) * ldw;
    return launch<0>(ctx, a);
}

static int conv_impl(const char* who, fie_ctx* ctx, const void* X, int B, int H, int W, int Cin, int upsample2x, int stride, int pad_mode,
                     const void* Wpacked, int64_t ldw, const float* w_scale, void* Y, int64_t ldc, int Cout, const void* bias,
                     const void* rowbias, int64_t ld_rowbias, const void* residual, int64_t ldr, float scale, int act,
                     const void* X2 = nullptr, int64_t ld2 = 0, int C2 = 0, const void* X3 = nullptr, int64_t ld3 = 0, int C3 = 0,
                     const float* gna_tab = nullptr, int gna_silu = 0) {
    const GnTarget gn = grab_gn_target(ctx);
    FIE_REQUIRE(ctx && X && Wpacked && Y, "%s: NULL ctx/X/W/Y", who);
    FIE_REQUIRE(B > 0 && H > 0 && W > 0 && Cin > 0 && Cout > 0, "%s: bad shape", who);
    FIE_REQUIRE(Cin % 8 == 0, "%s: Cin=%d must be a multiple of 8 (pad the tensor)", who, Cin);
    FIE_REQUIRE(stride == 1 || stride == 2, "%s: stride %d", who, stride);
    FIE_REQUIRE(pad_mode == 0 || pad_mode == 1, "%s: pad_mode %d", who, pad_mode);
    FIE_REQUIRE(act != FIE_ACT_GEGLU, "%s: GEGLU not supported", who);
    FIE_REQUIRE((X2 != nullptr) == (C2 > 0) && (X3 != nullptr) == (C3 > 0) && (!X3 || X2) && C2 % BK == 0 && C3 % BK == 0 && (!X2 || (Cin % BK == 0 && !w_scale && ld2 >= C2 && (!X3 || ld3 >= C3))),
                "%s: side inputs need Cin, C2, C3 %% 64 == 0 (C2=%d C3=%d)", who, C2, C3);
    const int K = 9 * Cin + C2 + C3;
    FIE_REQUIRE(ldw % BK == 0 && ldw >= K, "%s: ldw=%lld must be a multiple of 64 covering 9*Cin (+ side inputs)", who, (long long)ldw);
    if (int e = check_epilogue(who, Cout, ldc, residual, ldr, act)) return e;
    const int ups = upsample2x ? 1 : 0;
    const int Hin = H << ups, Win = W << ups;
    const int pads = pad_mode == 0 ? 2 : 1;
    const int OH = (Hin + pads - 3) / stride + 1, OW = (Win + pads - 3) / stride + 1;
    FIE_REQUIRE((int64_t)B * OH * OW < (1ll << 31), "%s: too many output pixels", who);
    GemmArgs a = {};
    a.A1 = (const half_t*)X; a.H = H; a.W = W; a.Cin = Cin; a.OH = OH; a.OW = OW; a.stride = stride;
    a.pt = a.pl = pad_mode == 0 ? 1 : 0; a.ups = ups;
    a.Wt = (const half_t*)Wpacked; a.ldw = ldw; a.w_scale = w_scale; a.C = (half_t*)Y; a.ldc = ldc;
    a.M = B * OH * OW; a.N = Cout; a.K = K; a.K1 = K;
    a.bias = (const half_t*)bias; a.rowbias = (const half_t*)rowbias; a.ld_rowbias = ld_rowbias;
    a.rows_per_batch = OH * OW; a.res = (const half_t*)residual; a.ldr = ldr; a.scale = scale; a.act = act;
    a.a1_bytes = (int64_t)B * H * W * Cin * 2;
    a.a2_bytes = 0;
    if (X2) {
        FIE_REQUIRE(stride == 1 && !ups && pad_mode == 0, "%s: side inputs need the plain same-size conv", who);
        a.A2 = (const half_t*)X2; a.lda2 = ld2; a.C2x = C2; a.a2_bytes = ((int64_t)(a.M - 1) * ld2 + C2) * 2;
        a.A3 = (const half_t*)X3; a.lda3 = ld3; a.C3x = C3; a.a3_bytes = X3 ? ((int64_t)(a.M - 1) * ld3 + C3) * 2 : 0;
        FIE_REQUIRE(a.a2_bytes < (1ll << 31) && a.a3_bytes < (1ll << 31), "%s: side inputs too large", who);
    }
    a.w_bytes = fie_roundup(Cout, 128) * ldw * (w_scale ? 1 : 2);
    a.gna_tab = gna_tab; a.gna_silu = gna_silu;
    if (int rc = take_gn_target(who, gn, a)) return rc;
    return launch<1>(ctx, a);
}

int fie_conv3x3_x8_nhwc_f16(fie_ctx* ctx, const void* X8, int B, int H, int W, int Cin, int upsample2x, int stride, int pad_mode, const void* W8packed,
                            int64_t ldw, const float* w_scale, float a_scale, void* Y, int64_t ldc, int Cout, const void* bias, const void* rowbias,
                            int64_t ld_rowbias, const void* residual, int64_t ldr, float scale, int act) {
    const char* who = "fie_conv3x3_x8_nhwc_f16";
    const GnTarget gn = grab_gn_target(ctx);
    FIE_REQUIRE(ctx && X8 && W8packed && w_scale && Y, "%s: NULL ctx/X/W/scale/Y", who);
// ... 120 lines not shown
```

fast-image-editing-with-generative-models_amd/hip.py:

```python
import ctypes
import numbers
import os
import subprocess

import torch

from . import header

_CSRC = os.path.join(os.path.dirname(os.path.abspath(__file__)), "csrc")
LIB_PATH = os.environ.get("FIE_LIB_PATH") or os.path.join(_CSRC, "libfie_hip.so")

_P, _I, _F = ctypes.c_void_p, ctypes.c_int, ctypes.c_float

ACT_NONE, ACT_SILU, ACT_GELU, ACT_QUICK_GELU, ACT_GEGLU = (header.DEFINES["ACT_" + n] for n in ("NONE", "SILU", "GELU", "QUICK_GELU", "GEGLU"))
ACT_RELU = header.DEFINES["ACT_RELU"]
SIGNATURES = {name: args for name, (_, args) in header.FUNCTIONS.items()}

_lib = None


def build(force=False):
    if force:
        subprocess.run(["make", "-C", _CSRC, "clean"], check=True, capture_output=True)
    r = subprocess.run(["make", "-C", _CSRC, "-j4"], capture_output=True, text=True)
    if r.returncode != 0:
        raise RuntimeError("building libfie_hip.so failed:\n" + r.stdout[-4000:] + r.stderr[-4000:])
    return LIB_PATH


def lib():
    global _lib
    if _lib is None:
        if not os.path.exists(LIB_PATH):
            raise RuntimeError(f"{LIB_PATH} is missing: run `python -c 'import __graft_entry__ as g; g.build()'` "
                               "(there is no non-HIP fallback for the hot path)")
        _lib = ctypes.CDLL(LIB_PATH)
        for name, (ret, args) in header.FUNCTIONS.items():
            fn = getattr(_lib, name)
            fn.argtypes, fn.restype = args, ret
    return _lib


def last_gemm_kernel(ctx=None):
    ctx = ctx or context(torch.cuda.current_device())
    return lib().fie_debug_last_gemm_kernel(ctx.h).decode()


class FieError(RuntimeError):
    pass


def fold_layernorm_tables(w, bias, gamma, beta, geglu=False):
    w = w.float()
    n = w.shape[0]
    wf = (w * gamma.float()[None, :]).to(torch.float16)
    b = w @ beta.float()
    if bias is not None:
        b = b + bias.float()
    tab = torch.stack([wf.float().sum(1), b], 1)
    if geglu:
        tab = torch.stack([tab[: n // 2], tab[n // 2:]], 1).reshape(n, 2)
    return wf, tab.contiguous()


def _chk(rc):
    if rc != 0:
        raise FieError(f"libfie_hip error {rc}: {lib().fie_last_error().decode()}")


def _p(t):
    return None if t is None else t.data_ptr()


GRAPH_NAMES = ("unet_forward", "controlnet_forward", "vae_encode", "vae_decode", "clip_text_forward")


class VaeConfig(ctypes.Structure):
    _fields_ = header.STRUCTS["fie_vae_config"]


class ClipConfig(ctypes.Structure):
    _fields_ = header.STRUCTS["fie_clip_config"]


class UnetConfig(ctypes.Structure):
    _fields_ = header.STRUCTS["fie_unet_config"]


class Program:

    def __init__(self, ctx):
        self.ctx, self.h, self.keep, self.outputs = ctx, _P(), [], None

    def __len__(self):
        return lib().fie_program_launches(self.h)

    def run(self):
        self.ctx.sync_stream()
        _chk(lib().fie_program_run(self.ctx.h, self.h))
        return self.outputs

    def register(self, name):
        assert name in GRAPH_NAMES, name
        _chk(lib().fie_graph_register(self.ctx.h, name.encode(), self.h))

    def close(self):
        if self.h:
            lib().fie_program_destroy(self.ctx.h, self.h)
            self.h = _P()


class W8:

    def __init__(self, q, scale):
        self.q, self.scale = q, scale

    def stride(self, d):
        return self.q.stride(d)

    def dequant(self):
        return self.q.view(torch.float8_e4m3fn).float() * self.scale[:, None]


class Context:

    def __init__(self, device=0, dtype=torch.float16):
        if dtype not in (torch.float16, torch.float32):
            raise ValueError(f"dtype {dtype} not supported (float16 or float32)")
        self.dtype = dtype
        self.f32 = dtype == torch.float32
        if not torch.cuda.is_available():
            raise RuntimeError("no HIP device visible: the fie_amd hot path has no CPU fallback")
        self.device = torch.device("cuda", device)
        h = _P()
        _chk(lib().fie_ctx_create(device, None, ctypes.byref(h)))
        self.h = h
        self._err = torch.zeros(4, device=self.device, dtype=torch.int32)
        self._err_host = torch.zeros(4, dtype=torch.int32).pin_memory()
        _chk(lib().fie_ctx_error_flag(self.h, self._err.data_ptr()))
        self._stream = None
        self._gn_ws = {}
        self._gn_stats = {}
        self._ws_retired = []
        self._gn_gen = 0
        self._sk_ws = {}
        self._sk_bound = None
        self._sk_pinned = False
        self._cap_stream = None
        self._prog_ws = []
        self.splitk_bytes = int(os.environ.get("FIE_SPLITK_MB", "96")) << 20
        self.gn_from_epilogue = os.environ.get("FIE_GN_FROM_EPILOGUE", "1") != "0"
        self.gn_quads = os.environ.get("FIE_GN_QUADS", "1") != "0"
        self._epi_prefetch = True
        self.up2x_parity = os.environ.get("FIE_UP2X_PARITY", "1") != "0"
        self.ln_fold = os.environ.get("FIE_LN_FOLD", "1") != "0"
        self.kv_group = os.environ.get("FIE_KV_GROUP", "1") != "0"
        self.ln_fold_which = os.environ.get("FIE_LN_FOLD_WHICH", "qkv,q2")
        self.ln_fold_ff1 = os.environ.get("FIE_LN_FOLD_FF1", "0") != "0"
        self.conv_plus_shortcut = os.environ.get("FIE_CONV_PLUS", "1") != "0"
        self._resize_tables = {}
        self.ws_tag = 0
        self._keep = None
        self.w8 = False
        self.a8 = os.environ.get("FIE_A8", "1") != "0"
        self.gn_fuse_conv = os.environ.get("FIE_GN_FUSE_CONV", "0") == "1"
        self.calib = False
        self.tune_frozen = os.environ.get("FIE_TUNE_FROZEN", "0") == "1"
        self.tune_table_entries = 0
        self.load_tune_table()

    def fetch_device_errors(self):
        self._err_host.copy_(self._err, non_blocking=True)

    def check_device_errors(self, fetch=True):
        if fetch:
            self.fetch_device_errors()
            torch.cuda.current_stream(self.device).synchronize()
        code = int(self._err_host[0])
        if code:
            self._err.zero_()
            self._err_host.zero_()
            what = {1: "fie_time_embed_f16: the in-launch barrier timed out (a workgroup never arrived); the timestep embedding of that "
                       "launch is invalid"}.get(code, "unknown device error")
            raise FieError(f"device error {code}: {what}")

    def sync_stream(self):
        s = torch.cuda.current_stream(self.device).cuda_stream
        if s != self._stream:
            _chk(lib().fie_ctx_set_stream(self.h, s))
            self._stream = s

    def load_tune_table(self, path=None):
        path = path or os.environ.get("FIE_TUNE_TABLE")
        if not path or self.f32:
            return 0
        with open(path) as f:
            n = lib().fie_gemm_autotune_load(self.h, f.read().encode())
        if n < 0:
            raise FieError(f"fie_gemm_autotune_load: {lib().fie_last_error().decode()}")
        self.tune_table_entries = n
        return n

    def _bind_splitk(self):
        if self._sk_pinned or self.f32 or not self.splitk_bytes:
            return
        key = (self._stream, self.ws_tag)
        if key == self._sk_bound:
            return
        ws = self._sk_ws.get(key)
        if ws is None:
            ws = self._sk_ws[key] = torch.zeros(self.splitk_bytes, device=self.device, dtype=torch.uint8)
        _chk(lib().fie_splitk_workspace(self.h, ws.data_ptr(), ws.numel()))
        self._sk_bound = key

    def capture_stream(self):
        if self._cap_stream is None:
            self._cap_stream = torch.cuda.Stream(device=self.device)
        with torch.cuda.stream(self._cap_stream):
            self.sync_stream()
            self._bind_splitk()
        torch.cuda.synchronize(self.device)
        return self._cap_stream

    def splitk_counters_clear(self):
        torch.cuda.synchronize(self.device)
        live = list(self._sk_ws.values()) + [w for w in (r() for r in self._prog_ws) if w is not None]
        return all(int(ws[:16384].view(torch.int32).abs().max()) == 0 for ws in live)

    def record(self):
        import contextlib

        @contextlib.contextmanager
        def cm():
            prog = Program(self)
            self.sync_stream()
            own = None
            if not self.f32 and self.splitk_bytes:
                own = torch.zeros(self.splitk_bytes, device=self.device, dtype=torch.uint8)
                prog.keep.append(own)
                import weakref
                self._prog_ws = [r for r in self._prog_ws if r() is not None] + [weakref.ref(own)]
# ... 84 lines not shown
    def gemm_probe(self, mode):
        _chk(lib().fie_debug_gemm_probe(self.h, int(mode)))

    @property
    def epi_prefetch(self):
        return self._epi_prefetch

    @epi_prefetch.setter
    def epi_prefetch(self, on):
        _chk(lib().fie_debug_epilogue_prefetch(self.h, int(bool(on))))
        self._epi_prefetch = bool(on)

    def tile_override(self, spec):
        return lib().fie_debug_tile_override(self.h, spec.encode() if spec else None)

    def close(self):
        if self.h:
            lib().fie_ctx_destroy(self.h)
            self.h = None

    def pack_linear(self, w, geglu=False, quant=True):
        self.sync_stream()
        if self.f32:
            w = w.to(self.device, torch.float32)
            if geglu:
                n = w.shape[0]
                w = torch.stack([w[: n // 2], w[n // 2:]], 1).reshape(n, -1)
            return w.contiguous()
        w = w.to(self.device, torch.float16).contiguous()
        n, k = w.shape
        npad, kpad = (n + 127) // 128 * 128, (k + 63) // 64 * 64
        if self.w8 and quant and self.a8:
            kpad = (k + 127) // 128 * 128
        if self.w8 and quant:
            q = torch.empty((npad, kpad), device=self.device, dtype=torch.uint8)
            scale = torch.empty((npad,), device=self.device, dtype=torch.float32)
            _chk(lib().fie_pack_rows_f8(self.h, _p(w), k, n, k, _p(q), kpad, npad, _p(scale), int(geglu)))
            return W8(q, scale)
        out = torch.empty((npad, kpad), device=self.device, dtype=torch.float16)
        _chk(lib().fie_pack_rows_f16(self.h, _p(w), k, n, k, _p(out), kpad, npad, int(geglu)))
        return out

    def pack_conv3x3(self, w, cin_pad=None, quant=True):
        self.sync_stream()
        if self.f32:
            co, ci = w.shape[:2]
            cp = cin_pad or (ci + 7) // 8 * 8
            out = torch.zeros((co, 3, 3, cp), device=self.device, dtype=torch.float32)
            out[..., :ci] = w.to(self.device, torch.float32).permute(0, 2, 3, 1)
            return out.reshape(co, 9 * cp)
        w = w.to(self.device, torch.float16).contiguous()
        co, ci = w.shape[:2]
        cin_pad = cin_pad or (ci + 7) // 8 * 8
        npad, kpad = (co + 127) // 128 * 128, (9 * cin_pad + 63) // 64 * 64
        if self.w8 and quant and cin_pad % 64 == 0:
            q = torch.empty((npad, kpad), device=self.device, dtype=torch.uint8)
            scale = torch.empty((npad,), device=self.device, dtype=torch.float32)
            _chk(lib().fie_pack_conv3x3_f8(self.h, _p(w), co, ci, cin_pad, _p(q), kpad, npad, _p(scale)))
            return W8(q, scale)
        out = torch.empty((npad, kpad), device=self.device, dtype=torch.float16)
        _chk(lib().fie_pack_conv3x3_f16(self.h, _p(w), co, ci, cin_pad, _p(out), kpad, npad))
        return out

    def _gn_stats_arm(self, rows_total, n, rows_per_image, groups):
        if not self.gn_from_epilogue or self.f32 or not groups or n % groups:
            return None
        if rows_per_image % 32 or rows_total % rows_per_image:
            return None
        cg, pgroups = n // groups, groups
        if cg not in (4, 8, 16):
            if cg % 4 or rows_per_image < 4096 or not self.gn_quads:
                return None
            pgroups = n // 4
        b = rows_total // rows_per_image
        need = lib().fie_gn_stats_bytes(b, rows_per_image, pgroups)
        key = (self._stream, self.ws_tag)
        buf = self._scratch(self._gn_stats, key, need)
        if self._keep is not None:
            self._keep.append(buf)
        _chk(lib().fie_gn_stats_target(self.h, _p(buf), rows_per_image, pgroups))
        self._gn_gen += 1
        return (buf, groups, n, rows_per_image, b, self._gn_gen, key, pgroups)

    def gemm(self, a, wp, n, out=None, a2=None, bias=None, rowbias=None, rows_per_batch=0, residual=None, scale=1.0,
             act=ACT_NONE, k=None, gn_stats=None, a_scale=1.0, out_f8=False, out_inv_scale=1.0):
        self.sync_stream()
        self._bind_splitk()
        m, k1 = a.shape
        ktot = k1 + (a2.shape[1] if a2 is not None else 0)
        if k is not None:
            assert k == ktot
        nout = n // 2 if act == ACT_GEGLU else n
        if out is None:
            out = self._alloc((m, nout), torch.uint8 if out_f8 else None)
        assert a.stride(1) == 1 and out.stride(1) == 1
        if self.f32:
            return self.gemm_f32(a, wp, n, out, a2=a2, bias=bias, rowbias=rowbias, rows_per_batch=rows_per_batch, residual=residual, scale=scale, act=act)
        if a.dtype == torch.uint8:
            assert isinstance(wp, W8) and a2 is None and wp.stride(0) % 128 == 0, "fp8 activations need fp8 weights packed with Kpad % 128 == 0"
            if out_f8 and out.dtype != torch.uint8:
                raise ValueError("out_f8 needs a uint8 output tensor")
            _chk(lib().fie_gemm_x8_f16(self.h, _p(a), a.stride(0), _p(wp.q), wp.stride(0), _p(wp.scale), float(a_scale), _p(out), out.stride(0), m, n, ktot,
                                       _p(bias), _p(rowbias), rowbias.stride(0) if rowbias is not None else 0, rows_per_batch, _p(residual),
                                       residual.stride(0) if residual is not None else 0, float(scale), act, int(out_f8), float(out_inv_scale)))
            return out
        if isinstance(wp, W8):
            _chk(lib().fie_gemm_w8_f16(self.h, _p(a), a.stride(0), k1, _p(a2), a2.stride(0) if a2 is not None else 0,
                                       _p(wp.q), wp.stride(0), _p(wp.scale), _p(out), out.stride(0), m, n, ktot, _p(bias), _p(rowbias),
                                       rowbias.stride(0) if rowbias is not None else 0, rows_per_batch, _p(residual),
                                       residual.stride(0) if residual is not None else 0, float(scale), act))
            return out
        tag = self._gn_stats_arm(m, n, gn_stats[0], gn_stats[1]) if gn_stats and act != ACT_GEGLU and out.stride(0) == n else None
        _chk(lib().fie_gemm_f16(self.h, _p(a), a.stride(0), k1, _p(a2), a2.stride(0) if a2 is not None else 0,
                                _p(wp), wp.stride(0), _p(out), out.stride(0), m, n, ktot, _p(bias), _p(rowbias),
                                rowbias.stride(0) if rowbias is not None else 0, rows_per_batch, _p(residual),
                                residual.stride(0) if residual is not None else 0, float(scale), act))
        out._gn_tag = tag
        return out

    def gemm_f32(self, a, wp, n, out=None, a2=None, bias=None, rowbias=None, rows_per_batch=0, residual=None, scale=1.0, act=ACT_NONE):
        self.sync_stream()
        m, k1 = a.shape
        ktot = k1 + (a2.shape[1] if a2 is not None else 0)
        if out is None:
            out = self._alloc((m, n // 2 if act == ACT_GEGLU else n), torch.float32)
        assert a.stride(1) == 1 and out.stride(1) == 1 and a.dtype == torch.float32 and wp.dtype == torch.float32 and out.dtype == torch.float32
        _chk(lib().fie_gemm_f32(self.h, _p(a), a.stride(0), k1, _p(a2), a2.stride(0) if a2 is not None else 0, _p(wp),
                                wp.stride(0), 0, _p(out), out.stride(0), m, n, ktot, _p(bias), _p(rowbias),
                                rowbias.stride(0) if rowbias is not None else 0, rows_per_batch, _p(residual),
                                residual.stride(0) if residual is not None else 0, float(scale), act, 1, 1, 0, 0, 0, 0, 0, 0))
        return out

    def fold_layernorm(self, w, bias, gamma, beta, geglu=False):
        dev = lambda t: None if t is None else t.to(self.device)
        wf, tab = fold_layernorm_tables(dev(w), dev(bias), dev(gamma), dev(beta), geglu=geglu)
        return self.pack_linear(wf, geglu=geglu, quant=False), tab

    def gemm_ln(self, x, wp, n, tab, eps=1e-5, act=ACT_NONE, out=None):
        self.sync_stream()
        m, k = x.shape
        nout = n // 2 if act == ACT_GEGLU else n
        if out is None:
            out = self._alloc((m, nout))
        assert x.stride(1) == 1 and out.stride(1) == 1 and tab.dtype == torch.float32 and tab.shape == (n, 2) and not self.f32
        _chk(lib().fie_gemm_ln_f16(self.h, _p(x), x.stride(0), _p(wp), wp.stride(0), _p(tab), float(eps), _p(out), out.stride(0), m, n, k, act))
        out._gn_tag = None
        return out

    def conv3x3_plus(self, x, wp, cout, x2, x3=None, bias=None, rowbias=None, scale=1.0, act=ACT_NONE, gn_groups=None, out=None):
        self.sync_stream()
        self._bind_splitk()
        b, h, w, cin = x.shape
        assert x.is_contiguous() and not self.f32 and x2.stride(1) == 1 and (x3 is None or x3.stride(1) == 1)
        if out is None:
            out = self._alloc((b, h, w, cout))
        tag = self._gn_stats_arm(b * h * w, cout, h * w, gn_groups) if gn_groups else None
        _chk(lib().fie_conv3x3_plus_nhwc_f16(self.h, _p(x), b, h, w, cin, _p(wp), wp.stride(0), _p(out), out.stride(2), cout, _p(bias), _p(rowbias),
                                             rowbias.stride(0) if rowbias is not None else 0, float(scale), act, _p(x2), x2.stride(0), x2.shape[1],
                                             _p(x3), x3.stride(0) if x3 is not None else 0, x3.shape[1] if x3 is not None else 0))
        out._gn_tag = tag
        return out

    def pack_conv_up2x(self, w):
        w = w.to(self.device, torch.float32)
        sets = (((0,), (1, 2)), ((0, 1), (2,)))
        mats = []
        for py in range(2):
            for px in range(2):
                taps = [sum(w[:, :, ky, kx] for ky in sets[py][a] for kx in sets[px][b]) for a in range(2) for b in range(2)]
                mats.append(self.pack_linear(torch.stack(taps, 1).reshape(w.shape[0], -1).to(torch.float16), quant=False))
        return torch.stack(mats).contiguous()

    def conv_up2x(self, x, wp4, cout, bias=None, rowbias=None, scale=1.0, act=ACT_NONE, gn_groups=None, out=None):
        self.sync_stream()
        self._bind_splitk()
        b, h, w, cin = x.shape
        assert x.is_contiguous() and not self.f32 and cin % 64 == 0
        if out is None:
            out = self._alloc((b, 2 * h, 2 * w, cout))
        tag = self._gn_stats_arm(b * 4 * h * w, cout, 4 * h * w, gn_groups) if gn_groups else None
        _chk(lib().fie_conv_up2x_nhwc_f16(self.h, _p(x), b, h, w, cin, _p(wp4), wp4.stride(1), wp4.shape[1], _p(out), out.stride(2), cout,
                                          _p(bias), _p(rowbias), rowbias.stride(0) if rowbias is not None else 0, float(scale), act))
        out._gn_tag = tag
        return out

    def conv3x3(self, x, wp, cout, out=None, stride=1, pad_mode=0, upsample=False, bias=None, rowbias=None,
                residual=None, scale=1.0, act=ACT_NONE, ldc=None, gn_groups=None, a_scale=1.0):
        self.sync_stream()
        self._bind_splitk()
        b, h, w, cin = x.shape
        assert x.is_contiguous()
        hin, win = (h * 2, w * 2) if upsample else (h, w)
        pads = 2 if pad_mode == 0 else 1
        oh, ow = (hin + pads - 3) // stride + 1, (win + pads - 3) // stride + 1
        ldc = ldc or cout
        if out is None:
            out = self._alloc((b, oh, ow, ldc), zero=ldc != cout)
        if x.dtype == torch.uint8:
            assert isinstance(wp, W8) and cin % 128 == 0 and wp.stride(0) % 128 == 0
            tag = self._gn_stats_arm(b * oh * ow, cout, oh * ow, gn_groups) if gn_groups and ldc == cout else None
            _chk(lib().fie_conv3x3_x8_nhwc_f16(self.h, _p(x), b, h, w, cin, int(upsample), stride, pad_mode, _p(wp.q), wp.stride(0), _p(wp.scale), float(a_scale),
                                               _p(out), out.stride(2), cout, _p(bias), _p(rowbias), rowbias.stride(0) if rowbias is not None else 0,
                                               _p(residual), residual.stride(2) if residual is not None else 0, float(scale), act))
            out._gn_tag = tag
            return out
        if isinstance(wp, W8):
            _chk(lib().fie_conv3x3_w8_nhwc_f16(self.h, _p(x), b, h, w, cin, int(upsample), stride, pad_mode, _p(wp.q), wp.stride(0),
                                               _p(wp.scale), _p(out), out.stride(2), cout, _p(bias), _p(rowbias),
                                               rowbias.stride(0) if rowbias is not None else 0, _p(residual),
                                               residual.stride(2) if residual is not None else 0, float(scale), act))
            return out
        if self.f32:
            out = self.conv3x3_f32(x, wp, cout, out, stride=stride, pad_mode=pad_mode, upsample=upsample, bias=bias, rowbias=rowbias, residual=residual,
                                   scale=scale, act=act)
            out._gn_tag = None
            return out
        tag = self._gn_stats_arm(b * oh * ow, cout, oh * ow, gn_groups) if gn_groups and ldc == cout else None
        _chk(lib().fie_conv3x3_nhwc_f16(self.h, _p(x), b, h, w, cin, int(upsample), stride, pad_mode, _p(wp),
                                        wp.stride(0), _p(out), out.stride(2), cout, _p(bias), _p(rowbias),
                                        rowbias.stride(0) if rowbias is not None else 0, _p(residual),
                                        residual.stride(2) if residual is not None else 0, float(scale), act))
        out._gn_tag = tag
        return out

    def conv3x3_f32(self, x, wp, cout, out, stride=1, pad_mode=0, upsample=False, bias=None, rowbias=None, residual=None, scale=1.0, act=ACT_NONE):
        self.sync_stream()
        b, h, w, cin = x.shape
# ... 711 lines not shown
```

fast-image-editing-with-generative-models_amd/nn.py:

```python
import torch

from . import hip
from .presets import time_embed_dim

F16 = torch.float16


def _dev(ctx, t):
    return t.to(ctx.device, ctx.dtype).contiguous()


class Linear:
    def __init__(self, ctx, sd, name, geglu=False, w=None, b=None, quant=True):
        w = sd[name + ".weight"] if w is None else w
        b = sd.get(name + ".bias") if b is None and name else b
        w = w.reshape(w.shape[0], -1)
        self.n, self.k = w.shape
        self.act = hip.ACT_GEGLU if geglu else hip.ACT_NONE
        self.wp = ctx.pack_linear(w, geglu=geglu, quant=quant)
        if b is not None:
            b = _dev(ctx, b)
            if geglu:
                b = torch.stack([b[: self.n // 2], b[self.n // 2:]], 1).reshape(-1).contiguous()
        self.b = b
        self.a8 = isinstance(self.wp, hip.W8) and ctx.a8 and self.wp.stride(0) % 128 == 0 and self.k % 16 == 0

    def __call__(self, ctx, a, a2=None, residual=None, act=None, scale=1.0, out=None, rowbias=None, rows_per_batch=0, gn_stats=None,
                 a_scale=1.0, out_f8=False, out_inv_scale=1.0):
        return ctx.gemm(a, self.wp, self.n, a2=a2, bias=self.b, residual=residual, scale=scale, out=out,
                        act=self.act if act is None else act, rowbias=rowbias, rows_per_batch=rows_per_batch, gn_stats=gn_stats,
                        a_scale=a_scale, out_f8=out_f8, out_inv_scale=out_inv_scale)


class Conv3:
    def __init__(self, ctx, sd, name, cin_pad=None, cout_pad=None):
        w = sd[name + ".weight"]
        self.cout, self.cin = w.shape[:2]
        self.cin_pad = cin_pad or (self.cin + 7) // 8 * 8
        self.ldc = cout_pad or self.cout
        self.n = (self.cout + 3) // 4 * 4
        a8_ok = bool(ctx.w8 and ctx.a8 and getattr(ctx, "a8_conv", True) and self.cin_pad == self.cin and self.cin % 128 == 0
                     and name.endswith((".conv1", ".conv2")))
        self.wp = ctx.pack_conv3x3(w, self.cin_pad, quant=self.cout < 1280 or a8_ok)
        self.a8 = a8_ok and isinstance(self.wp, hip.W8) and self.wp.stride(0) % 128 == 0
        self.wp4 = None
        if ("upsamplers" in name and self.cin % 64 == 0 and self.cin_pad == self.cin and ctx.up2x_parity and not ctx.f32
                and torch.is_tensor(self.wp) and self.ldc <= self.n == self.cout):
            self.wp4 = ctx.pack_conv_up2x(w)
        b = sd.get(name + ".bias")
        if b is not None:
            bb = torch.zeros(self.n, dtype=ctx.dtype, device=ctx.device)
            bb[: self.cout] = b.to(ctx.device, ctx.dtype)
            b = bb
        self.b = b

    def __call__(self, ctx, x, stride=1, pad_mode=0, upsample=False, rowbias=None, residual=None, act=hip.ACT_NONE, gn_groups=None, a_scale=1.0):
        if upsample and self.wp4 is not None and ctx.up2x_parity and residual is None and stride == 1 and pad_mode == 0:
            return ctx.conv_up2x(x, self.wp4, self.n, bias=self.b, rowbias=rowbias, act=act, gn_groups=gn_groups)
        return ctx.conv3x3(x, self.wp, self.n, stride=stride, pad_mode=pad_mode, upsample=upsample, bias=self.b,
                           rowbias=rowbias, residual=residual, act=act, ldc=max(self.ldc, self.n), gn_groups=gn_groups, a_scale=a_scale)


class Norm:
    def __init__(self, ctx, sd, name):
        self.g, self.b = _dev(ctx, sd[name + ".weight"]), _dev(ctx, sd[name + ".bias"])


class Resnet:
    def __init__(self, ctx, sd, p, groups, eps, temb_slot=None):
        self.groups, self.eps = groups, eps
        self.n1, self.n2 = Norm(ctx, sd, p + "norm1"), Norm(ctx, sd, p + "norm2")
        self.c1, self.c2 = Conv3(ctx, sd, p + "conv1"), Conv3(ctx, sd, p + "conv2")
        self.sc = Linear(ctx, sd, p + "conv_shortcut") if p + "conv_shortcut.weight" in sd else None
        self.temb_slot = temb_slot
        self.s8, self.amax = [1.0, 1.0], None
        self.wp_plus = None
        if self.sc is not None and torch.is_tensor(self.c2.wp) and torch.is_tensor(self.sc.wp) and self.c2.wp.dtype == torch.float16:
            k2, ksc = 9 * self.c2.cin_pad, sd[p + "conv_shortcut.weight"].shape[1]
            if self.c2.cin % 64 == 0 and self.c2.cin_pad == self.c2.cin and ksc % 64 == 0 and self.c2.n == self.c2.cout == self.sc.n and self.c2.ldc <= self.c2.n:
                self.wp_plus = torch.cat([self.c2.wp[:, :k2], self.sc.wp[:, :ksc]], 1).contiguous()
                zero = torch.zeros(self.c2.n, dtype=self.c2.wp.dtype, device=self.c2.wp.device)
                self.b_plus = (self.c2.b if self.c2.b is not None else zero) + (self.sc.b if self.sc.b is not None else zero)

    def _gn_conv(self, ctx, x, norm, conv, residual=None):
        if not (torch.is_tensor(conv.wp) and conv.wp.dtype == torch.float16 and conv.cin_pad == conv.cin == x.shape[-1] and conv.ldc <= conv.n == conv.cout
                and ctx.conv3x3_gn_ok(x, conv.n, self.groups)):
            return None
        coef = ctx.groupnorm_coef(x, norm.g, norm.b, self.groups, self.eps)
        if coef is None:
            return None
        return ctx.conv3x3_gn(x, coef, True, conv.wp, conv.n, bias=conv.b, residual=residual, gn_groups=self.groups)

    def __call__(self, ctx, x, temb_all=None, skip=None):
        b, h, w, _ = x.shape
        if skip is None and self.temb_slot is None and not ctx.calib:
            y = self._gn_conv(ctx, x, self.n1, self.c1)
            if y is not None:
                if self.sc is None:
                    out = self._gn_conv(ctx, y, self.n2, self.c2, residual=x)
                    if out is not None:
                        return out
                return self._tail(ctx, x, y, skip)
        calib = ctx.calib and self.amax is not None
        q1, q2 = self.c1.a8 and not calib, self.c2.a8 and self.wp_plus is None and not calib
        y = ctx.groupnorm(x, self.n1.g, self.n1.b, self.groups, self.eps, True, x2=skip, out_f8=q1, out_inv_scale=1.0 / self.s8[0])
        if calib and self.c1.a8:
            ctx.amax_into(y, self.amax[0:1])
        rb = temb_all[:, self.temb_slot[0]:self.temb_slot[1]] if self.temb_slot is not None else None
        y = self.c1(ctx, y, rowbias=rb, gn_groups=self.groups, a_scale=self.s8[0] if q1 else 1.0)
        return self._tail(ctx, x, y, skip, calib, q2)

    def _tail(self, ctx, x, y, skip, calib=False, q2=False):
        b, h, w, _ = x.shape
        y = ctx.groupnorm(y, self.n2.g, self.n2.b, self.groups, self.eps, True, out_f8=q2, out_inv_scale=1.0 / self.s8[1])
        if calib and self.c2.a8 and self.wp_plus is None:
            ctx.amax_into(y, self.amax[1:2])
        if self.wp_plus is not None and ctx.conv_plus_shortcut and x.shape[-1] % 64 == 0 and (skip is None or skip.shape[-1] % 64 == 0):
            return ctx.conv3x3_plus(y, self.wp_plus, self.c2.n, x.view(b * h * w, -1), None if skip is None else skip.view(b * h * w, -1),
                                    bias=self.b_plus, gn_groups=self.groups)
        if self.sc is not None:
            res = self.sc(ctx, x.view(b * h * w, -1), a2=None if skip is None else skip.view(b * h * w, -1))
            res = res.view(b, h, w, -1)
        else:
            res = x
        return self.c2(ctx, y, residual=res, gn_groups=self.groups, a_scale=self.s8[1] if q2 else 1.0)


class TBlock:
    def __init__(self, ctx, sd, p, c, head_dim):
        self.c, self.heads, self.hd = c, c // head_dim, head_dim
        self.ln = [Norm(ctx, sd, p + f"norm{i}") for i in (1, 2, 3)]
        wqkv = torch.cat([sd[p + f"attn1.to_{n}.weight"] for n in "qkv"], 0)
        self.qkv = Linear(ctx, None, None, w=wqkv)
        self.o1 = Linear(ctx, sd, p + "attn1.to_out.0")
        self.q2 = Linear(ctx, sd, p + "attn2.to_q")
        self._kv_raw = torch.cat([sd[p + "attn2.to_k.weight"], sd[p + "attn2.to_v.weight"]], 0)
        self.kv2 = Linear(ctx, None, None, w=self._kv_raw)
        self.kv_net, self.kv_slot = None, None
        self.o2 = Linear(ctx, sd, p + "attn2.to_out.0")
        self.ff1 = Linear(ctx, sd, p + "ff.net.0.proj", geglu=True)
        self.ff2 = Linear(ctx, sd, p + "ff.net.2")
        self.kv_cache = None
        self.folded = None
        if (not ctx.f32 and not ctx.w8 and c % 64 == 0 and (8 * c) % 320 == 0 and all(torch.is_tensor(l.wp) for l in (self.qkv, self.q2, self.ff1))):
            ln = [(sd[p + f"norm{i}.weight"], sd[p + f"norm{i}.bias"]) for i in (1, 2, 3)]
            self.folded = (ctx.fold_layernorm(wqkv, None, *ln[0]),
                           ctx.fold_layernorm(sd[p + "attn2.to_q.weight"], sd.get(p + "attn2.to_q.bias"), *ln[1]),
                           ctx.fold_layernorm(sd[p + "ff.net.0.proj.weight"], sd.get(p + "ff.net.0.proj.bias"), *ln[2], geglu=True))
        self.a8 = all(l.a8 for l in (self.qkv, self.o1, self.q2, self.o2, self.ff1, self.ff2)) and head_dim == 64
        self.s8, self.amax = [1.0] * 6, None

    def _text_kv(self, ctx, text):
        if self.kv_cache is None:
            net = self.kv_net
            if net is not None and ctx.kv_group and not ctx.calib:
                if net._kv_out is None:
                    net._kv_out = net.kv_all(ctx, text)
                self.kv_cache = net._kv_out[:, self.kv_slot[0]:self.kv_slot[1]]
            else:
                self.kv_cache = self.kv2(ctx, text)
        return self.kv_cache

    def _call_a8(self, ctx, h, text, batch, tokens, text_len):
        c, s = self.c, self.s8
        y = ctx.layernorm(h, self.ln[0].g, self.ln[0].b, out_f8=True, out_inv_scale=1.0 / s[0])
        qkv = self.qkv(ctx, y, a_scale=s[0])
        a = ctx.attention(qkv[:, :c], qkv[:, c:2 * c], qkv[:, 2 * c:], self.heads, self.hd, tokens, tokens, batch, out_f8=True, out_inv_scale=1.0 / s[1])
        h = self.o1(ctx, a, residual=h, a_scale=s[1])
        y = ctx.layernorm(h, self.ln[1].g, self.ln[1].b, out_f8=True, out_inv_scale=1.0 / s[2])
        q = self.q2(ctx, y, a_scale=s[2])
        kv = self._text_kv(ctx, text)[:batch * text_len]
        a = ctx.attention(q, kv[:, :c], kv[:, c:], self.heads, self.hd, tokens, text_len, batch, out_f8=True, out_inv_scale=1.0 / s[3])
        h = self.o2(ctx, a, residual=h, a_scale=s[3])
        y = ctx.layernorm(h, self.ln[2].g, self.ln[2].b, out_f8=True, out_inv_scale=1.0 / s[4])
        f = self.ff1(ctx, y, a_scale=s[4], out_f8=True, out_inv_scale=1.0 / s[5])
        return self.ff2(ctx, f, residual=h, a_scale=s[5])

    def __call__(self, ctx, h, text, batch, tokens, text_len):
        am = self.amax if ctx.calib and self.a8 else None
        if self.a8 and am is None:
            return self._call_a8(ctx, h, text, batch, tokens, text_len)
        rec = (lambda t, i: ctx.amax_into(t, am[i:i + 1])) if am is not None else (lambda t, i: None)
        c = self.c
        if self.folded is not None and ctx.ln_fold and am is None:
            (wq, tq), (w2, t2), (wf, tf) = self.folded
            which = ctx.ln_fold_which
            qkv = ctx.gemm_ln(h, wq, 3 * c, tq) if "qkv" in which else self.qkv(ctx, ctx.layernorm(h, self.ln[0].g, self.ln[0].b))
            a = ctx.attention(qkv[:, :c], qkv[:, c:2 * c], qkv[:, 2 * c:], self.heads, self.hd, tokens, tokens, batch)
            h = self.o1(ctx, a, residual=h)
            q = ctx.gemm_ln(h, w2, c, t2) if "q2" in which else self.q2(ctx, ctx.layernorm(h, self.ln[1].g, self.ln[1].b))
            kv = self._text_kv(ctx, text)[:batch * text_len]
            a = ctx.attention(q, kv[:, :c], kv[:, c:], self.heads, self.hd, tokens, text_len, batch)
            h = self.o2(ctx, a, residual=h)
            f = ctx.gemm_ln(h, wf, 8 * c, tf, act=hip.ACT_GEGLU) if ctx.ln_fold_ff1 else self.ff1(ctx, ctx.layernorm(h, self.ln[2].g, self.ln[2].b))
            return self.ff2(ctx, f, residual=h)
        y = ctx.layernorm(h, self.ln[0].g, self.ln[0].b)
        rec(y, 0)
        qkv = self.qkv(ctx, y)
        a = ctx.attention(qkv[:, :c], qkv[:, c:2 * c], qkv[:, 2 * c:], self.heads, self.hd, tokens, tokens, batch)
        rec(a, 1)
        h = self.o1(ctx, a, residual=h)
        y = ctx.layernorm(h, self.ln[1].g, self.ln[1].b)
        rec(y, 2)
        q = self.q2(ctx, y)
        kv = self._text_kv(ctx, text)[:batch * text_len]
        a = ctx.attention(q, kv[:, :c], kv[:, c:], self.heads, self.hd, tokens, text_len, batch)
        rec(a, 3)
        h = self.o2(ctx, a, residual=h)
        y = ctx.layernorm(h, self.ln[2].g, self.ln[2].b)
        rec(y, 4)
        f = self.ff1(ctx, y)
        rec(f, 5)
        return self.ff2(ctx, f, residual=h)


class Transformer2D:
    def __init__(self, ctx, sd, p, c, depth, head_dim, groups):
        self.groups = groups
        self.norm = Norm(ctx, sd, p + "norm")
        self.pin, self.pout = Linear(ctx, sd, p + "proj_in"), Linear(ctx, sd, p + "proj_out")
        self.blocks = [TBlock(ctx, sd, f"{p}transformer_blocks.{k}.", c, head_dim) for k in range(depth)]

    def __call__(self, ctx, x, text, text_len):
        b, hh, ww, c = x.shape
        xt = x.view(b * hh * ww, c)
        h = ctx.groupnorm(x, self.norm.g, self.norm.b, self.groups, 1e-6, False).view(b * hh * ww, c)
        h = self.pin(ctx, h)
        for blk in self.blocks:
            h = blk(ctx, h, text, b, hh * ww, text_len)
        o = self.pout(ctx, h, residual=xt, gn_stats=(hh * ww, self.groups))
        y = o.view(b, hh, ww, c)
        y._gn_tag = getattr(o, "_gn_tag", None)
        return y

    def reset(self):
        for blk in self.blocks:
            blk.kv_cache = None


class _CondNet:

    def __init__(self, ctx, cfg, sd):
        self.ctx, self.cfg = ctx, cfg
        g, eps, hd = cfg["norm_num_groups"], cfg["norm_eps"], cfg["head_dim"]
        chans = cfg["block_out_channels"]
        self.temb_names = []
        self.conv_in = Conv3(ctx, sd, "conv_in", cin_pad=8)
        self.t1, self.t2 = Linear(ctx, sd, "time_embedding.linear_1", quant=False), Linear(ctx, sd, "time_embedding.linear_2", quant=False)
        self.a1, self.a2 = Linear(ctx, sd, "add_embedding.linear_1", quant=False), Linear(ctx, sd, "add_embedding.linear_2", quant=False)
        te_dim, ch0 = time_embed_dim(cfg), chans[0]
        self.te = None
        if not ctx.f32 and te_dim % 64 == 0 and ch0 % 32 == 0 and ch0 <= 512:
            self.te = tuple(_dev(ctx, sd[k]) for k in ("time_embedding.linear_1.weight", "time_embedding.linear_1.bias",
                                                       "time_embedding.linear_2.weight", "time_embedding.linear_2.bias"))
            self.te_ws = {}
        self.down = []
        for i in range(len(chans)):
            layers = []
            for j in range(cfg["layers_per_block"]):
                r = self._resnet(sd, f"down_blocks.{i}.resnets.{j}.", g, eps)
                d = cfg["down_attn"][i][j]
                t = Transformer2D(ctx, sd, f"down_blocks.{i}.attentions.{j}.", chans[i], d, hd, g) if d else None
                layers.append((r, t))
            ds = Conv3(ctx, sd, f"down_blocks.{i}.downsamplers.0.conv") if i != len(chans) - 1 else None
            self.down.append((layers, ds))
        self.mid = [(self._resnet(sd, "mid_block.resnets.0.", g, eps), None)]
        for k in range(1, cfg["mid_resnets"]):
            t = Transformer2D(ctx, sd, f"mid_block.attentions.{k - 1}.", chans[-1], cfg["mid_attn"], hd, g) \
                if cfg["mid_attn"] else None
            self.mid.append((self._resnet(sd, f"mid_block.resnets.{k}.", g, eps), t))
        self._sd = sd

    def _resnet(self, sd, p, g, eps):
        r = Resnet(self.ctx, sd, p, g, eps)
        self.temb_names.append((p, r))
        return r

    def _finish_temb(self, sd):
        ws, bs, col = [], [], 0
        for p, r in self.temb_names:
            w = sd[p + "time_emb_proj.weight"]
            ws.append(w)
            bs.append(sd[p + "time_emb_proj.bias"])
            r.temb_slot = (col, col + w.shape[0])
            col += w.shape[0]
        self.temb_proj = Linear(self.ctx, None, None, w=torch.cat(ws, 0), b=torch.cat(bs, 0), quant=False)
        self._sd = None
        self._finish_kv()

    def _finish_kv(self):
        ctx = self.ctx
        blocks = [b for t in self.transformers() for b in t.blocks]
        self.kv_all, self._kv_out = None, None
        if len(blocks) > 1 and not ctx.f32 and not ctx.w8 and all(b._kv_raw is not None for b in blocks):
            self.kv_all = Linear(ctx, None, None, w=torch.cat([b._kv_raw for b in blocks], 0))
            off = 0
            for b in blocks:
                b.kv_net, b.kv_slot = self, (off, off + 2 * b.c)
                off += 2 * b.c
        for b in blocks:
            b._kv_raw = None

    def transformers(self):
        for layers, _ in self.down:
            for _, t in layers:
                if t:
                    yield t
        for _, t in self.mid:
            if t:
                yield t

    def begin_image(self, pooled, time_ids):
        ctx, cfg = self.ctx, self.cfg
        b = pooled.shape[0]
        ad = cfg["addition_time_embed_dim"]
        add_in = ctx._alloc((b, cfg["projection_class_embeddings_input_dim"]))
        add_in[:, : pooled.shape[1]] = pooled
        ctx.sinusoid(time_ids, ad, add_in, col0=pooled.shape[1])
        self.add_emb = self.a2(ctx, self.a1(ctx, add_in, act=hip.ACT_SILU))
        for t in self.transformers():
            t.reset()
        self._kv_out = None

    def time_rowbias(self, t_dev):
        ctx = self.ctx
        ch0 = self.cfg["block_out_channels"][0]
        add_emb = self.add_emb[:t_dev.shape[0]]
        if self.te is not None and t_dev.shape[0] <= 4:
            ctx.sync_stream()
            key = (ctx._stream, ctx.ws_tag)
            ws = self.te_ws.get(key)
            if ws is None:
                ws = self.te_ws[key] = ctx.time_embed_workspace(self.te[0].shape[0])
            return self.temb_proj(ctx, ctx.time_embed(t_dev, *self.te, ws, add=add_emb))
        s = ctx._alloc((t_dev.shape[0], ch0))
        ctx.sinusoid(t_dev, ch0, s)
        semb = self.t2(ctx, self.t1(ctx, s, act=hip.ACT_SILU), rowbias=add_emb, rows_per_batch=1, act=hip.ACT_SILU)
        return self.temb_proj(ctx, semb)

    def encode(self, x, temb_all, text, text_len):
        ctx = self.ctx
        skips = [x]
        for layers, ds in self.down:
            for r, t in layers:
                x = r(ctx, x, temb_all)
                if t:
                    x = t(ctx, x, text, text_len)
                skips.append(x)
            if ds is not None:
                x = ds(ctx, x, stride=2, gn_groups=self.cfg["norm_num_groups"])
                skips.append(x)
        for r, t in self.mid:
            if t:
                x = t(ctx, x, text, text_len)
            x = r(ctx, x, temb_all)
        return skips, x


class UNet(_CondNet):
    def __init__(self, ctx, cfg, sd):
        super().__init__(ctx, cfg, sd)
        g, eps, hd = cfg["norm_num_groups"], cfg["norm_eps"], cfg["head_dim"]
        rev = list(reversed(cfg["block_out_channels"]))
        self.up = []
        for i in range(len(rev)):
            layers = []
            for j in range(cfg["layers_per_block"] + 1):
                r = self._resnet(sd, f"up_blocks.{i}.resnets.{j}.", g, eps)
                d = cfg["up_attn"][i][j]
                t = Transformer2D(ctx, sd, f"up_blocks.{i}.attentions.{j}.", rev[i], d, hd, g) if d else None
                layers.append((r, t))
            us = Conv3(ctx, sd, f"up_blocks.{i}.upsamplers.0.conv") if i != len(rev) - 1 else None
            self.up.append((layers, us))
        self.norm_out = Norm(ctx, sd, "conv_norm_out")
        self.conv_out = Conv3(ctx, sd, "conv_out")
        self._finish_temb(sd)

    def transformers(self):
        yield from super().transformers()
        for layers, _ in self.up:
            for _, t in layers:
                if t:
                    yield t

    def decode(self, x, skips, temb_all, text, text_len):
        ctx, cfg = self.ctx, self.cfg
        skips = list(skips)
        for layers, us in self.up:
            for r, t in layers:
                x = r(ctx, x, temb_all, skip=skips.pop())
                if t:
                    x = t(ctx, x, text, text_len)
            if us is not None:
                x = us(ctx, x, upsample=True)
        y = ctx.groupnorm(x, self.norm_out.g, self.norm_out.b, cfg["norm_num_groups"], cfg["norm_eps"], True)
        return self.conv_out(ctx, y)


class ControlNet(_CondNet):
    def __init__(self, ctx, cfg, sd):
        super().__init__(ctx, cfg, sd)
        p = "controlnet_cond_embedding."
        nb = len(cfg["conditioning_embedding_out_channels"]) - 1
        self.ce_in = Conv3(ctx, sd, p + "conv_in", cin_pad=8)
        self.ce_blocks = [(Conv3(ctx, sd, f"{p}blocks.{2 * i}"), Conv3(ctx, sd, f"{p}blocks.{2 * i + 1}")) for i in range(nb)]
        self.ce_out = Conv3(ctx, sd, p + "conv_out")
        n_skip = 1 + sum(cfg["layers_per_block"] + (1 if i != len(cfg["block_out_channels"]) - 1 else 0)
                         for i in range(len(cfg["block_out_channels"])))
        self.zero = [Linear(ctx, sd, f"controlnet_down_blocks.{i}") for i in range(n_skip)]
        self.zero_mid = Linear(ctx, sd, "controlnet_mid_block")
        self._finish_temb(sd)

    def cond_embedding(self, cond):
        ctx = self.ctx
        c = self.ce_in(ctx, cond, act=hip.ACT_SILU)
        for a, b in self.ce_blocks:
            c = a(ctx, c, act=hip.ACT_SILU)
            c = b(ctx, c, stride=2, act=hip.ACT_SILU)
        return self.ce_out(ctx, c)

    def encode_cond(self, x_in, cond_emb, temb_all, text, text_len):
        x = self.conv_in(self.ctx, x_in, residual=cond_emb)
        return self.encode(x, temb_all, text, text_len)

    def add_residuals(self, skips, mid, scale, unet_skips, unet_mid):
        ctx = self.ctx
        out = []
        for z, s, u in zip(self.zero, skips, unet_skips):
            b, h, w, c = s.shape
            out.append(z(ctx, s.view(-1, c), scale=scale, residual=u.view(-1, c)).view(b, h, w, c))
        b, h, w, c = mid.shape
        m = self.zero_mid(ctx, mid.view(-1, c), scale=scale, residual=unet_mid.view(-1, c)).view(b, h, w, c)
        return out, m
```

include/fie.h:

```cpp
#ifndef FIE_H_
#define FIE_H_

#include <stdint.h>

#ifdef __cplusplus
extern "C" {
#endif

#define FIE_OK 0
#define FIE_EINVAL (-1)
#define FIE_EHIP (-2)
#define FIE_ENODEV (-3)

#define FIE_DEVERR_TIME_EMBED_BARRIER 1u

#define FIE_ACT_NONE 0
#define FIE_ACT_SILU 1
#define FIE_ACT_GELU 2
#define FIE_ACT_QUICK_GELU 3
#define FIE_ACT_GEGLU 4
#define FIE_ACT_RELU 5

typedef struct fie_ctx fie_ctx;

// ... 7 lines not shown
typedef struct fie_vae_config {
    int latent_h, latent_w;
    int num_blocks;
    int block_out_channels[8];
    int layers_per_block;
    int norm_num_groups;
    float norm_eps;
    int out_channels;
    const char* prefix;
} fie_vae_config;
typedef struct fie_clip_config {
    int batch, tokens;
    int hidden, heads, layers, intermediate;
    int projection_dim;
    int quick_gelu;
    float eps;
} fie_clip_config;
typedef struct fie_unet_config {
    int batch;
    int latent_h, latent_w;
    int text_len;
    int num_blocks;
    int block_out_channels[4];
    int layers_per_block;
    int down_attn[4][4];
    int up_attn[4][4];
    int mid_attn;
    int mid_resnets;
    int head_dim;
    int norm_num_groups;
    float norm_eps;
    int cross_attention_dim;
    int addition_time_embed_dim;
    int pooled_dim;
    int num_cond_channels;
    int cond_channels[8];
} fie_unet_config;
int fie_weights_register(fie_ctx* ctx, const char* name, const void* ptr, int64_t n, int64_t ld);
int fie_weights_clear(fie_ctx* ctx);
int fie_weights_clear_prefix(fie_ctx* ctx, const char* prefix);
int64_t fie_vae_decode_workspace_bytes(const fie_vae_config* cfg, int latent_h, int latent_w);
int fie_vae_decode_f16(fie_ctx* ctx, const fie_vae_config* cfg, const void* z, void* out, void* workspace, int64_t workspace_bytes);
int64_t fie_vae_encode_workspace_bytes(const fie_vae_config* cfg);
int fie_vae_encode_f16(fie_ctx* ctx, const fie_vae_config* cfg, const void* x, void* moments, void* workspace, int64_t workspace_bytes);
int64_t fie_clip_text_workspace_bytes(const fie_clip_config* cfg);
int fie_clip_text_forward_f16(fie_ctx* ctx, const fie_clip_config* cfg, const char* prefix, const int32_t* ids, const int32_t* eos_rows, void* penultimate,
                              void* pooled, void* workspace, int64_t workspace_bytes);
int fie_unet_num_residuals(const fie_unet_config* cfg);
int64_t fie_unet_workspace_bytes(const fie_unet_config* cfg);
int fie_unet_forward_f16(fie_ctx* ctx, const fie_unet_config* cfg, const char* prefix, const void* x, const float* t, const void* text, const void* pooled,
                         const float* time_ids, const void* const* down_residuals, const void* mid_residual, void* eps_out, void* workspace,
                         int64_t workspace_bytes);
int64_t fie_controlnet_workspace_bytes(const fie_unet_config* cfg);
int fie_controlnet_forward_f16(fie_ctx* ctx, const fie_unet_config* cfg, const char* prefix, const void* x, const float* t, const void* text, const void* pooled,
                               const float* time_ids, const void* cond, float conditioning_scale, void* const* down_out, void* mid_out, void* workspace,
                               int64_t workspace_bytes);
int64_t fie_unet_step_cache_bytes(const fie_unet_config* cfg, int controlnet);
int fie_step_cache_bind(fie_ctx* ctx, const char* prefix, void* ptr, int64_t bytes);
int fie_step_cache_reset(fie_ctx* ctx, const char* prefix);
int fie_add_f16(fie_ctx* ctx, const void* a, const void* b, void* out, int64_t n);
int fie_copy_rows_f16(fie_ctx* ctx, const void* src, int64_t ld_src, void* dst, int64_t ld_dst, int rows, int cols);

typedef struct fie_program fie_program;
int fie_program_begin(fie_ctx* ctx, fie_program** out);
int fie_program_end(fie_ctx* ctx);
int fie_program_launches(const fie_program* p);
int fie_program_run(fie_ctx* ctx, fie_program* p);
int fie_program_destroy(fie_ctx* ctx, fie_program* p);
int fie_graph_register(fie_ctx* ctx, const char* name, fie_program* p);
int fie_unet_forward(fie_ctx* ctx);
int fie_controlnet_forward(fie_ctx* ctx);
int fie_vae_encode(fie_ctx* ctx);
int fie_vae_decode(fie_ctx* ctx);
int fie_clip_text_forward(fie_ctx* ctx);

int fie_gemm_f16(fie_ctx* ctx, const void* A1, int64_t lda1, int K1, const void* A2, int64_t lda2,
                 const void* Wpacked, int64_t ldw, void* C, int64_t ldc, int M, int N, int K,
                 const void* bias, const void* rowbias, int64_t ld_rowbias, int rows_per_batch,
                 const void* residual, int64_t ldr, float scale, int act);

int fie_gemm_ln_f16(fie_ctx* ctx, const void* X, int64_t ldx, const void* Wfolded, int64_t ldw, const float* ln_tab, float eps, void* C, int64_t ldc,
                    int M, int N, int K, int act);

int fie_conv3x3_nhwc_f16(fie_ctx* ctx, const void* X, int B, int H, int W, int Cin, int upsample2x, int stride,
                         int pad_mode, const void* Wpacked, int64_t ldw, void* Y, int64_t ldc, int Cout,
                         const void* bias, const void* rowbias, int64_t ld_rowbias,
                         const void* residual, int64_t ldr, float scale, int act);

int fie_attention_f16(fie_ctx* ctx, const void* Q, int64_t ldq, const void* K, int64_t ldk, const void* V,
                      int64_t ldv, void* O, int64_t ldo, int B, int H, int Tq, int Tk, int D, float scale,
                      int causal);

int64_t fie_groupnorm_workspace_bytes(int B, int64_t rows_per_image, int groups);
int fie_groupnorm_nhwc_f16(fie_ctx* ctx, const void* X1, int C1, const void* X2, int C2, void* Y, int B,
                           int64_t rows_per_image, int groups, const void* gamma, const void* beta, float eps,
                           int silu, void* workspace);

int fie_layernorm_f16(fie_ctx* ctx, const void* X, int64_t ldx, void* Y, int64_t ldy, int64_t rows, int C,
                      const void* gamma, const void* beta, float eps);

int fie_sinusoid_f16(fie_ctx* ctx, const float* vals, int B, int nvals, int dim, void* out, int64_t ld_out,
                     int col0);

int64_t fie_time_embed_workspace_bytes(int E);
int fie_time_embed_f16(fie_ctx* ctx, const float* t, int B, int C0, int E, const void* W1, const void* b1, const void* W2,
                       const void* b2, const void* add, int64_t ld_add, void* out, int64_t ld_out, void* workspace);

int fie_clip_embed_f16(fie_ctx* ctx, const int32_t* ids, int B, int T, int C, const void* tok_table,
                       const void* pos_table, void* out);

int fie_pixels_in_u8_f16(fie_ctx* ctx, const uint8_t* src, int H, int W, int normalize, void* dst, int copies);
int fie_pixels_out_f16_u8(fie_ctx* ctx, const void* src, int64_t ld_in, int H, int W, uint8_t* dst);

int fie_latent_prep(fie_ctx* ctx, const void* moments, const float* eps_post, const float* noise, int64_t HW,
                    float scaling_factor, float sqrt_ab, float sqrt_1mab, float* latents_out, void* model_in,
                    int copies);

int fie_lcm_step(fie_ctx* ctx, const void* eps, int64_t ld_eps, int nb, float guidance, float* latents,
                 const float* noise, int64_t HW, float sqrt_ab_t, float sqrt_1mab_t, float c_skip, float c_out,
                 float sqrt_ab_prev, float sqrt_1mab_prev, void* model_in, int copies, float inv_scaling,
                 void* decode_in);

int fie_pack_rows_f16(fie_ctx* ctx, const void* src, int64_t ld_src, int N, int K, void* dst, int64_t ldw,
                      int Npad, int interleave2);
int fie_pack_conv3x3_f16(fie_ctx* ctx, const void* src_oihw, int Cout, int Cin, int cin_pad, void* dst,
                         int64_t ldw, int Npad);

int fie_pack_rows_f8(fie_ctx* ctx, const void* src, int64_t ld_src, int N, int K, void* dst, int64_t ldw, int Npad, float* scales,
                     int interleave2);
int fie_pack_conv3x3_f8(fie_ctx* ctx, const void* src_oihw, int Cout, int Cin, int cin_pad, void* dst, int64_t ldw, int Npad,
                        float* scales);
int fie_gemm_w8_f16(fie_ctx* ctx, const void* A1, int64_t lda1, int K1, const void* A2, int64_t lda2, const void* W8packed,
                    int64_t ldw, const float* w_scale, void* C, int64_t ldc, int M, int N, int K, const void* bias,
                    const void* rowbias, int64_t ld_rowbias, int rows_per_batch, const void* residual, int64_t ldr, float scale,
                    int act);
int fie_conv3x3_w8_nhwc_f16(fie_ctx* ctx, const void* X, int B, int H, int W, int Cin, int upsample2x, int stride, int pad_mode,
                            const void* W8packed, int64_t ldw, const float* w_scale, void* Y, int64_t ldc, int Cout,
                            const void* bias, const void* rowbias, int64_t ld_rowbias, const void* residual, int64_t ldr,
                            float scale, int act);

int fie_gemm_x8_f16(fie_ctx* ctx, const void* A8, int64_t lda, const void* W8packed, int64_t ldw, const float* w_scale, float a_scale, void* C, int64_t ldc,
                    int M, int N, int K, const void* bias, const void* rowbias, int64_t ld_rowbias, int rows_per_batch, const void* residual, int64_t ldr,
                    float scale, int act, int out_f8, float out_inv_scale);
int fie_layernorm_f16_o8(fie_ctx* ctx, const void* X, int64_t ldx, void* Y8, int64_t ldy8, int64_t rows, int C, const void* gamma, const void* beta,
                         float eps, float inv_scale);
int fie_attention_f16_o8(fie_ctx* ctx, const void* Q, int64_t ldq, const void* K, int64_t ldk, const void* V, int64_t ldv, void* O8, int64_t ldo8,
                         int B, int H, int Tq, int Tk, int D, float scale, int causal, float inv_scale);
int fie_quantize_f8(fie_ctx* ctx, const void* X, int64_t ldx, void* Y8, int64_t ldy, int64_t rows, int C, float inv_scale);
int fie_amax_f16(fie_ctx* ctx, const void* X, int64_t ldx, int64_t rows, int C, float* amax);
int fie_groupnorm_nhwc_f16_o8(fie_ctx* ctx, const void* X1, int C1, const void* X2, int C2, void* Y8, int B, int64_t rows_per_image, int groups,
                              const void* gamma, const void* beta, float eps, int silu, void* workspace, float inv_scale);
int fie_groupnorm_stats_nhwc_f16_o8(fie_ctx* ctx, const void* X, int C, void* Y8, int B, int64_t rows_per_image, int groups, const void* gamma,
                                    const void* beta, float eps, int silu, const void* partial, void* workspace, int partial_groups, float inv_scale);
int fie_conv3x3_x8_nhwc_f16(fie_ctx* ctx, const void* X8, int B, int H, int W, int Cin, int upsample2x, int stride, int pad_mode, const void* W8packed,
                            int64_t ldw, const float* w_scale, float a_scale, void* Y, int64_t ldc, int Cout, const void* bias, const void* rowbias,
                            int64_t ld_rowbias, const void* residual, int64_t ldr, float scale, int act);

int fie_gemm_f32(fie_ctx* ctx, const float* A1, int64_t lda1, int K1, const float* A2, int64_t lda2, const float* W,
                 int64_t ldw, int w_is_kn, float* C, int64_t ldc, int M, int N, int K, const float* bias,
                 const float* rowbias, int64_t ld_rowbias, int rows_per_batch, const float* residual, int64_t ldr,
                 float scale, int act, int nb1, int nb2, int64_t sA1, int64_t sA2, int64_t sW1, int64_t sW2, int64_t sC1,
                 int64_t sC2);
int fie_conv3x3_nhwc_f32(fie_ctx* ctx, const float* X, int B, int H, int W, int Cin, int upsample2x, int stride, int pad_mode,
                         const float* Wkc, int64_t ldw, float* Y, int64_t ldc, int Cout, const float* bias,
                         const float* rowbias, int64_t ld_rowbias, const float* residual, int64_t ldr, float scale, int act);
int fie_softmax_rows_f32(fie_ctx* ctx, float* S, int64_t rows, int cols, int64_t ld, float scale, int causal, int tq);
// ... 171 lines not shown
```

Baseline: 15.33 images/sec.

## Emit LayerNorm row statistics from producer GEMM epilogues for consumer LN-fold GEMMs

The GEMMs that write the transformer residual stream (proj_in, o1, o2, ff2) now accumulate per-row sum and sum-of-squares in their epilogue. They use fixed-point integer atomics into a row-stats table. The downstream LayerNorm-folded GEMMs (qkv, q2, ff1) load these precomputed mean/rstd instead of recomputing row statistics from the A operand during the main loop. This aims to remove the redundant statistics pass in the consumer. In exchange it adds double-precision accumulation and atomics in producer epilogues, plus a table clear per encode/decode.

Measured after the change: 15.52 images/sec (median of 6 runs). 1.01x the previous value.

```diff
diff --git a/fast-image-editing-with-generative-models_amd/csrc/gemm_common.h b/fast-image-editing-with-generative-models_amd/csrc/gemm_common.h
--- a/fast-image-editing-with-generative-models_amd/csrc/gemm_common.h
+++ b/fast-image-editing-with-generative-models_amd/csrc/gemm_common.h
@@ -36,6 +36,9 @@
     const float* gna_tab; int gna_silu;
 };
 
+__host__ __device__ __forceinline__ unsigned long long* rs_table(const GemmArgs& p) { return reinterpret_cast<unsigned long long*>(const_cast<half_t*>(p.A3)); }
+__host__ __device__ __forceinline__ const long long* ln_table(const GemmArgs& p) { return reinterpret_cast<const long long*>(p.gna_tab); }
+
 __device__ __forceinline__ int take_parity(GemmArgs& p, int bid) {
     if (p.oscat != 2) return bid;
     const int par = bid & 3;
@@ -104,8 +107,64 @@
     }
 }
 
-template <int FM, int FN, int WM, int WN>
-__device__ __forceinline__ void epilogue_lean(const GemmArgs& p, f32x4 (&acc)[FN][FM], int m0, int n0, int wm, int wn, int lane, const EpiPre<FM, FN>& pre) {
+constexpr double kRsSumMagic = 1.5 * 268435456.0;
+constexpr double kRsSqMagic = 1.5 * 16777216.0;
+__device__ __forceinline__ void rs_add(double& s, unsigned long long& q, float x) {
+    s += (double)fminf(fmaxf(x, -65504.f), 65504.f);
+    const double xq = (double)fminf(fmaxf(x, -2048.f), 2048.f);
+    q += __builtin_bit_cast(unsigned long long, __builtin_fma(xq, xq, kRsSqMagic));
+}
+__device__ __forceinline__ void rs_add_fast(double& s, unsigned long long& q, float& mx, float x) {
+    mx = fmaxf(mx, fabsf(x));
+    const double xd = (double)x;
+    s += xd;
+    q += __builtin_bit_cast(unsigned long long, __builtin_fma(xd, xd, kRsSqMagic));
+}
+__device__ __forceinline__ bool rs_fast_ok(double s, float mx) { return mx <= 2048.f && __builtin_fabs(s) <= 1.0e300; }
+template <int FM, int WM, int WGN, int BM>
+__device__ __forceinline__ void row_stats_emit(const GemmArgs& p, const double (&s)[FM], const unsigned long long (&q)[FM], int cnt, int m0, int wm, int wn, int lane,
+                                               int tid, void* lds) {
+    const int fr = lane & 15;
+    unsigned long long si[FM], qi[FM];
+#pragma unroll
+    for (int j = 0; j < FM; ++j) {
+        si[j] = __builtin_bit_cast(unsigned long long, s[j] + kRsSumMagic) - __builtin_bit_cast(unsigned long long, kRsSumMagic);
+        qi[j] = q[j] - (unsigned long long)cnt * __builtin_bit_cast(unsigned long long, kRsSqMagic);
+        si[j] += __shfl_xor(si[j], 16); si[j] += __shfl_xor(si[j], 32);
+        qi[j] += __shfl_xor(qi[j], 16); qi[j] += __shfl_xor(qi[j], 32);
+    }
+    if constexpr (WGN == 1) {
+        if (lane < 16) {
+#pragma unroll
+            for (int j = 0; j < FM; ++j) {
+                const int m = m0 + wm * WM + j * 16 + fr;
+                if (m < p.M) { atomicAdd(rs_table(p) + 2 * (size_t)m, si[j]); atomicAdd(rs_table(p) + 2 * (size_t)m + 1, qi[j]); }
+            }
+        }
+    } else {
+        unsigned long long* sh = reinterpret_cast<unsigned long long*>(lds);
+        __syncthreads();
+        if (lane < 16) {
+#pragma unroll
+            for (int j = 0; j < FM; ++j) {
+                const int r = wn * BM + wm * WM + j * 16 + fr;
+                sh[2 * r] = si[j]; sh[2 * r + 1] = qi[j];
+            }
+        }
+        __syncthreads();
+        if (tid < BM) {
+            unsigned long long a = 0, b = 0;
+#pragma unroll
+            for (int w = 0; w < WGN; ++w) { a += sh[2 * (w * BM + tid)]; b += sh[2 * (w * BM + tid) + 1]; }
+            const int m = m0 + tid;
+            if (m < p.M) { atomicAdd(rs_table(p) + 2 * (size_t)m, a); atomicAdd(rs_table(p) + 2 * (size_t)m + 1, b); }
+        }
+    }
+}
+
+template <int FM, int FN, int WM, int WN, bool STATS = false>
+__device__ __forceinline__ void epilogue_lean(const GemmArgs& p, f32x4 (&acc)[FN][FM], int m0, int n0, int wm, int wn, int lane, const EpiPre<FM, FN>& pre,
+                                              double* rs_s = nullptr, unsigned long long* rs_q = nullptr) {
     const int fr = lane & 15, fq = lane >> 4;
     const int mrow = m0 + wm * WM + fr, ncol = n0 + wn * WN + fq * 4;
     const __amdgpu_buffer_rsrc_t rs_c = buf_rsrc(p.C, (int)(((int64_t)(p.M - 1) * p.ldc + p.N) * 2));
@@ -113,6 +172,7 @@
     for (int j = 0; j < FM; ++j) {
         const int m = mrow + j * 16;
         const unsigned ro = m < p.M ? (unsigned)m * (unsigned)p.ldc * 2u : 0x80000000u;
+        float mx = 0.f;
 #pragma unroll
         for (int i = 0; i < FN; ++i) {
             const int n = ncol + i * 16;
@@ -121,9 +181,29 @@
             __builtin_memcpy(&r, &pre.res[j][i], 8);
 #pragma unroll
             for (int q = 0; q < 4; ++q) o[q] = (half_t)(acc[i][j][q] + (float)b[q] + (float)r[q]);
+            if constexpr (STATS) {
+#pragma unroll
+                for (int q = 0; q < 4; ++q) rs_add_fast(rs_s[j], rs_q[j], mx, (float)o[q]);
+            }
             u32x2 bits;
             __builtin_memcpy(&bits, &o, 8);
             __builtin_amdgcn_raw_buffer_store_b64(bits, rs_c, ro + (n < p.N ? (unsigned)n << 1 : 0xC0000000u), 0, 0);
+        }
+        if constexpr (STATS) {
+            if (!rs_fast_ok(rs_s[j], mx)) {
+                double s2 = 0.0;
+                unsigned long long q2 = 0;
+#pragma unroll
+                for (int i = 0; i < FN; ++i) {
+                    f16x4 b, r;
+                    __builtin_memcpy(&b, &pre.bias[i], 8);
+                    __builtin_memcpy(&r, &pre.res[j][i], 8);
+#pragma unroll
+                    for (int q = 0; q < 4; ++q) rs_add(s2, q2, (float)(half_t)(acc[i][j][q] + (float)b[q] + (float)r[q]));
+                }
+                rs_s[j] = s2;
+                rs_q[j] = q2;
+            }
         }
     }
 }
@@ -169,6 +249,26 @@
     const __amdgpu_buffer_rsrc_t rt = buf_rsrc(p.ln_tab, p.N * 8);
     lo = __builtin_bit_cast(f32x4, __builtin_amdgcn_raw_buffer_load_b128(rt, (unsigned)n * 8u, 0, 0));
     hi = __builtin_bit_cast(f32x4, __builtin_amdgcn_raw_buffer_load_b128(rt, (unsigned)n * 8u + 16u, 0, 0));
+}
+
+template <int FM, int WM>
+__device__ __forceinline__ void ln_stats_load(const GemmArgs& p, int m0, int wm, int lane, u32x4 (&v)[FM]) {
+    const __amdgpu_buffer_rsrc_t rs = buf_rsrc(ln_table(p), (int64_t)p.M * 16);
+#pragma unroll
+    for (int j = 0; j < FM; ++j) v[j] = __builtin_amdgcn_raw_buffer_load_b128(rs, (unsigned)(m0 + wm * WM + j * 16 + (lane & 15)) * 16u, 0, 0);
+}
+template <int FM>
+__device__ __forceinline__ void ln_stats_finish(const GemmArgs& p, const u32x4 (&v)[FM], float (&mean)[FM], float (&rstd)[FM]) {
+    const double inv_k = 1.0 / (double)p.K;
+#pragma unroll
+    for (int j = 0; j < FM; ++j) {
+        const long long si = (long long)((unsigned long long)v[j][0] | ((unsigned long long)v[j][1] << 32));
+        const unsigned long long qi = (unsigned long long)v[j][2] | ((unsigned long long)v[j][3] << 32);
+        const double mu = (double)si * (1.0 / 16777216.0) * inv_k;
+        const double var = (double)qi * (1.0 / 268435456.0) * inv_k - mu * mu;
+        mean[j] = (float)mu;
+        rstd[j] = rsqrtf((float)((var > 0.0 ? var : 0.0) + (double)p.ln_eps));
+    }
 }
 
 template <int FM, int FN, int WM, int WN>
@@ -283,8 +383,9 @@
     }, std::make_integer_sequence<int, FN % 4>{});
 }
 
-template <int FM, int FN, int WM, int WN, bool BUF = false, bool PATCH = false>
-__device__ __forceinline__ void epilogue(const GemmArgs& p, f32x4 (&acc)[FN][FM], int m0, int n0, int wm, int wn, int lane, const EpiPre<FM, FN>* pre = nullptr) {
+template <int FM, int FN, int WM, int WN, bool BUF = false, bool PATCH = false, bool STATS = false>
+__device__ __forceinline__ void epilogue(const GemmArgs& p, f32x4 (&acc)[FN][FM], int m0, int n0, int wm, int wn, int lane, const EpiPre<FM, FN>* pre = nullptr,
+                                         double* rs_s = nullptr, unsigned long long* rs_q = nullptr) {
     const int fr = lane & 15, fq = lane >> 4;
     const bool have_pre = pre != nullptr && pre->on;
     if (p.probe == 4 && p.M > 0) return;
@@ -428,6 +529,16 @@
             }
         }
     }
+    if constexpr (STATS) {
+#pragma unroll
+        for (int i = 0; i < FN; ++i) {
+            const bool in_n = ncol + i * 16 < p.N;
+#pragma unroll
+            for (int j = 0; j < FM; ++j)
+#pragma unroll
+                for (int r = 0; r < 4; ++r) rs_add(rs_s[j], rs_q[j], in_n ? (float)(half_t)acc[i][j][r] : 0.f);
+        }
+    }
     if constexpr (BUF) {
         if (p.out_f8) {
             const __amdgpu_buffer_rsrc_t rs8 = buf_rsrc(p.C, (int64_t)(p.M - 1) * p.ldc + (geglu ? p.N >> 1 : p.N));
diff --git a/fast-image-editing-with-generative-models_amd/csrc/gemm_conv.hip b/fast-image-editing-with-generative-models_amd/csrc/gemm_conv.hip
--- a/fast-image-editing-with-generative-models_amd/csrc/gemm_conv.hip
+++ b/fast-image-editing-with-generative-models_amd/csrc/gemm_conv.hip
@@ -146,8 +146,10 @@
 
 template <int BM, int BN, int ST, int MODE, int NW, bool PF = false, bool STAMP = false, bool ALT = false, int LEAN = 0>
 __global__ __launch_bounds__(NW * 64) void gemm3_kernel(GemmArgs p) {
-    constexpr bool LNF = LEAN == 2;
-    static_assert(!LNF || (MODE == 0 && !STAMP), "LayerNorm fold: GEMM view only");
+    constexpr bool LNF = LEAN == 2, LNS = LEAN == 5, STATS = LEAN == 3 || LEAN == 4;
+    constexpr bool LEAN_EPI = LEAN == 1 || LEAN == 3, FULL_EPI = LEAN == 0 || LEAN == 4;
+    static_assert(!(LNF || LNS) || (MODE == 0 && !STAMP), "LayerNorm fold: GEMM view only");
+    static_assert(!STATS || (MODE == 0 && !STAMP && BM * BN / (NW * 64) <= 64), "row statistics: GEMM view, tiles with <= 16 accumulator fragments per lane");
     static_assert(!ALT || (NW == 8 && MODE == 0 && !PF && !STAMP), "ALT: 8-wave GEMM-view tiles without the fragment prefetch");
     constexpr int WGN = (LEAN == 2 && BM * BN / (NW * 256) <= 16 && (BM / NW) % 16 == 0) ? 1 : (BN / (NW / 2)) % 16 == 0 ? NW / 2 : 1, WGM = NW / WGN;
     constexpr int WM = BM / WGM, WN = BN / WGN;
@@ -296,10 +298,10 @@
 
     EpiPre<FM, FN> pre;
     pre.on = false;
-    LnTab<(LNF && FM * FN <= 16) ? FN : 1> ln_pre;
+    LnTab<((LNF || LNS) && FM * FN <= 16) ? FN : 1> ln_pre;
     if constexpr (FM * FN <= 16) {
-        if constexpr (LNF) {
-        } else if (LEAN || (nsplit == 1 && p.epi_prefetch)) epilogue_prefetch<FM, FN, WM, WN>(p, pre, m0, n0, wm, wn, lane);
+        if constexpr (LNF || LNS) {
+        } else if (LEAN_EPI || (nsplit == 1 && p.epi_prefetch)) epilogue_prefetch<FM, FN, WM, WN>(p, pre, m0, n0, wm, wn, lane);
     }
     constexpr int LJ = LNF ? FM : 1;
     float ln_s[LJ], ln_q[LJ];
@@ -330,9 +332,14 @@
     };
     using c0_t = std::integral_constant<int, 0>;
 
+    float ln_mean[(LNF || LNS) ? FM : 1], ln_rstd[(LNF || LNS) ? FM : 1];
+    u32x4 ln_raw[LNS ? FM : 1];
+    constexpr bool LNS_EARLY = LNS && FM * FN <= 16;
+    if constexpr (LNS_EARLY) ln_stats_load<FM, WM>(p, m0, wm, lane, ln_raw);
 #pragma unroll
     for (int s = 0; s < ST - 1; ++s)
         if (s < nk) { issue(kbeg + s, s); issue_w(kbeg + s, s); }
+    if constexpr (LNS_EARLY) ln_stats_finish<FM>(p, ln_raw, ln_mean, ln_rstd);
 
     const int fr = lane & 15, fq = lane >> 4;
     int stage = 0, fill = ST - 1;
@@ -464,8 +471,7 @@
         fill = fill + 1 == ST ? 0 : fill + 1;
     }
     stamp(11);
-    float ln_mean[LNF ? FM : 1], ln_rstd[LNF ? FM : 1];
-    if constexpr (LNF && FM * FN <= 16) {
+    if constexpr ((LNF || LNS) && FM * FN <= 16) {
 #pragma unroll
         for (int i = 0; i < FN; ++i) ln_tab_load(p, n0 + wn * WN + i * 16 + (lane >> 4) * 4, ln_pre.lo[i], ln_pre.hi[i]);
     }
@@ -481,12 +487,16 @@
             ln_rstd[j] = rsqrtf(fmaxf(sq * inv_k - mu * mu, 0.f) + p.ln_eps);
         }
     }
-    if constexpr (FM * FN <= 16 && !LEAN) {
+    if constexpr (LNS && !LNS_EARLY) {
+        ln_stats_load<FM, WM>(p, m0, wm, lane, ln_raw);
+        ln_stats_finish<FM>(p, ln_raw, ln_mean, ln_rstd);
+    }
+    if constexpr (FM * FN <= 16 && FULL_EPI) {
         if (nsplit > 1 && !splitk_reduce<FM, FN, NW>(p, acc, tile_all, slice, tid, smem)) return;
     }
-    if constexpr (LNF && FM * FN > 16) {
+    if constexpr ((LNF || LNS) && FM * FN > 16) {
         epilogue_geglu_lean<FM, FN, WM, WN, true>(p, acc, m0, n0, wm, wn, lane, ln_mean, ln_rstd);
-    } else if constexpr (LNF) {
+    } else if constexpr (LNF || LNS) {
         epilogue_lean_ln<FM, FN, WM, WN>(p, acc, m0, n0, wm, wn, lane, ln_pre, ln_mean, ln_rstd);
     } else
     if constexpr (FM * FN > 16) {
@@ -500,6 +510,14 @@
         if constexpr (FN & 1)
             epilogue<FM, 1, WM, WN, true>(p, reinterpret_cast<f32x4(&)[1][FM]>(acc[FN - 1]), m0, n0 + 16 * (FN - 1), wm, wn, lane);
         }
+    } else if constexpr (STATS) {
+        double rs_s[FM];
+        unsigned long long rs_q[FM];
+#pragma unroll
+        for (int j = 0; j < FM; ++j) { rs_s[j] = 0.0; rs_q[j] = 0; }
+        if constexpr (LEAN_EPI) epilogue_lean<FM, FN, WM, WN, true>(p, acc, m0, n0, wm, wn, lane, pre, rs_s, rs_q);
+        else epilogue<FM, FN, WM, WN, true, false, true>(p, acc, m0, n0, wm, wn, lane, &pre, rs_s, rs_q);
+        row_stats_emit<FM, WM, WGN, BM>(p, rs_s, rs_q, 4 * FN, m0, wm, wn, lane, tid, smem);
     } else {
         if constexpr (LEAN == 1) epilogue_lean<FM, FN, WM, WN>(p, acc, m0, n0, wm, wn, lane, pre);
         else epilogue<FM, FN, WM, WN, true>(p, acc, m0, n0, wm, wn, lane, &pre);
@@ -516,7 +534,7 @@
 }
 
 enum Family { kGeneric, kRing, kPhased, kHalo, kHaloEdge, kThin };
-enum : unsigned { kSplitK = 1, kStamps = 2, kGemmOnly = 4, kLnFold = 8, kPF = 16, kAlt = 32 };
+enum : unsigned { kSplitK = 1, kStamps = 2, kGemmOnly = 4, kLnFold = 8, kPF = 16, kAlt = 32, kRowStats = 64 };
 using LaunchFn = int (*)(fie_ctx*, GemmArgs&, dim3 grid);
 struct Tile {
     int code, bm, bn;
@@ -540,10 +558,14 @@
     template <int MODE, bool LN = false>
     static int launch(fie_ctx* ctx, GemmArgs& a, dim3 grid) {
         auto k = kernel<MODE, LN ? 2 : 0>();
+        if constexpr (LN) {
+            if (ln_table(a)) k = kernel<MODE, 5>();
+        }
         if constexpr (!LN && has_lean<MODE>) {
-            if (a.epi_prefetch && a.splitk <= 1 && !a.rowbias && a.act == FIE_ACT_NONE && a.scale == 1.f && !a.gn_partial && !a.out_f8 && !a.w_scale && !a.oscat &&
-                a.probe == 0)
-                k = kernel<MODE, 1>();
+            const bool lean = a.epi_prefetch && a.splitk <= 1 && !a.rowbias && a.act == FIE_ACT_NONE && a.scale == 1.f && !a.gn_partial && !a.out_f8 && !a.w_scale &&
+                              !a.oscat && a.probe == 0;
+            if (rs_table(a)) k = lean ? kernel<MODE, 3>() : kernel<MODE, 4>();
+            else if (lean) k = kernel<MODE, 1>();
         }
         fie_launch(ctx, k, grid, dim3(NW * 64), lds, a);
         FIE_LAUNCH_CHECK();
@@ -553,13 +575,13 @@
         hipError_t e = hipSuccess;
         auto set = [&](auto* k) { if (e == hipSuccess) e = hipFuncSetAttribute(reinterpret_cast<const void*>(k), hipFuncAttributeMaxDynamicSharedMemorySize, lds); };
         set(kernel<0, 0>());
-        if constexpr (has_lean<0>) set(kernel<0, 1>());
+        if constexpr (has_lean<0>) { set(kernel<0, 1>()); set(kernel<0, 3>()); set(kernel<0, 4>()); }
         if constexpr (!(F & kGemmOnly)) set(kernel<2, 0>());
-        if constexpr (F & kLnFold) set(kernel<0, 2>());
+        if constexpr (F & kLnFold) { set(kernel<0, 2>()); set(kernel<0, 5>()); }
         return e;
     }
     static constexpr Tile row(int code, const char* name, int w8, int x8) {
-        Tile t = {code, BM, BN, kRing, name, F, w8, x8, &launch<0>, nullptr, nullptr, &attr};
+        Tile t = {code, BM, BN, kRing, name, F | (has_lean<0> ? kRowStats : 0u), w8, x8, &launch<0>, nullptr, nullptr, &attr};
         if constexpr (!(F & kGemmOnly)) t.conv = &launch<2>;
         if constexpr (F & kLnFold) t.ln = &launch<0, true>;
         return t;
@@ -734,6 +756,7 @@
         t = find_tile(t->w8);
     }
     code = t->code;
+    FIE_REQUIRE(MODE != 0 || !rs_table(a) || (!a.w_scale && (t->flags & kRowStats)), "tile code %d has no build that emits LayerNorm row statistics", code);
     a.nbm = (a.M + t->bm - 1) / t->bm;
     a.nbn = (a.N + t->bn - 1) / t->bn;
     split = splitk_fit(ctx, a, *t, split);
@@ -753,12 +776,13 @@
         snprintf(rebuild, sizeof(rebuild), " | b=%d pad=%d C2=%d C3=%d K1=%d parity=%d w8=%d bias=%d rowbias=%d rpb=%d res=%d act=%d scale=%.9g gn=%d gnrows=%d f8out=%d ln=%d gna=%d",
                  MODE == 1 ? a.M / (a.OH * a.OW) : 1, MODE == 1 && !a.taps2 && a.pt == 0 ? 1 : 0, a.C2x, a.C3x, a.K1, a.taps2, a.w_scale ? (a.a_scale != 0.f ? 2 : 1) : 0,
                  a.bias != nullptr, a.rowbias != nullptr, a.rowbias ? a.rows_per_batch : 0, a.res != nullptr, a.act, (double)a.scale, a.gn_partial ? a.gn_G : 0,
-                 a.gn_partial ? a.gn_rows : 0, a.out_f8, a.ln_tab != nullptr, a.gna_tab != nullptr);
+                 a.gn_partial ? a.gn_rows : 0, a.out_f8, a.ln_tab != nullptr, MODE == 1 && a.gna_tab != nullptr);
         if (MODE == 1)
             FIE_DESC(ctx, "conv M=%d N=%d K=%d in=%dx%dx%d s%d u%d%s%s code=%d flop=%.0f%s", a.M * (a.oscat == 2 ? 4 : 1), a.N, a.K, a.H, a.W, a.Cin, a.stride, a.ups,
                      a.taps2 ? " up2x-parity" : "", a.A2 ? " +1x1" : "", code + 10000 * (split > 1 ? split : 0), 2.0 * a.M * a.N * a.K * (a.oscat == 2 ? 4 : 1), rebuild);
         else
-            FIE_DESC(ctx, "gemm M=%d N=%d K=%d act=%d%s%s%s code=%d flop=%.0f%s", a.M, a.N, a.K, a.act, a.res ? " +res" : "", a.ln_tab ? " +ln" : "", a.w_scale ? (a.a_scale != 0.f ? " a8w8" : " w8") : "",
+            FIE_DESC(ctx, "gemm M=%d N=%d K=%d act=%d%s%s%s%s code=%d flop=%.0f%s", a.M, a.N, a.K, a.act, a.res ? " +res" : "", rs_table(a) ? " +rowstats" : "",
+                     a.ln_tab ? (ln_table(a) ? " +ln +stats" : " +ln") : "", a.w_scale ? (a.a_scale != 0.f ? " a8w8" : " w8") : "",
                      code + 10000 * (split > 1 ? split : 0), 2.0 * a.M * a.N * a.K, rebuild);
     }
     if (x8) return fie_launch_gemm_x8(ctx, a, code, MODE == 1);
@@ -792,6 +816,7 @@
     for (size_t i = 0; i < ncand; ++i) {
         const int c = cand[i];
         if (c == guess || excluded(c)) continue;
+        if (MODE == 0 && rs_table(a) && !(find_tile(c)->flags & kRowStats)) continue;
         if ((c == 43 || c == 46) && blocks(64, 64) > 64 * ctx->num_cus) continue;
         if ((c == 81 || c == 96 || c == 62) && 2 * blocks(256, 128) < ctx->num_cus) continue;
         if ((c == 63 || c == 64) && (MODE != 0 || a.N % 320 != 0 || 2 * blocks(256, 320) < ctx->num_cus)) continue;
@@ -836,6 +861,7 @@
     (void)hipDeviceSynchronize();
     GemmArgs t = a;
     t.C = static_cast<half_t*>(ctx->tune_buf);
+    if (MODE == 0) t.A3 = nullptr;
     auto time_of = [&](int code, int split = 1) -> float {
         float ms[7];
         for (int rep = -1; rep < 7; ++rep) {
@@ -897,6 +923,15 @@
     int split = 1;
     bool pinned = false;
     auto decode = [&](int v) { split = v / 10000 > 1 ? v / 10000 : 1; v %= 10000; order = v >= 2000 ? 1 : v >= 1000 ? 0 : -1; code = v % 1000; };
+    FIE_REQUIRE(MODE != 0 || !rs_table(a) || (dma_ok && !a.w_scale), "fie_gemm_stats_f16: f16 GEMM view on the LDS-DMA kernels only (operands < 2 GiB)");
+    auto stats_fallback = [&]() {
+        const Tile* t = find_tile(code);
+        if (MODE != 0 || !rs_table(a) || (t && (t->flags & kRowStats))) return;
+        code = (a.N % 128 == 0 && (int64_t)((a.M + 255) / 256) * ((a.N + 127) / 128) >= 150) ? 96 : 42;
+        order = -1;
+        split = 1;
+    };
+    stats_fallback();
     for (int i = 0; i < ctx->n_overrides; ++i) {
         const fie_tile_override& o = ctx->overrides[i];
         if (o.mode == (MODE == 1) && o.M == a.M && o.N == a.N && o.K == a.K) { decode(o.code); pinned = true; }
@@ -936,6 +971,7 @@
         order = -1;
         split = 1;
     }
+    stats_fallback();
     return run_code<MODE>(ctx, a, code, order, dma_ok, split);
 }
 
@@ -1152,7 +1188,7 @@
 
 static int gemm_impl(const char* who, fie_ctx* ctx, const void* A1, int64_t lda1, int K1, const void* A2, int64_t lda2,
                      const void* Wpacked, int64_t ldw, const float* w_scale, void* C, int64_t ldc, int M, int N, int K, const void* bias,
-                     const void* rowbias, int64_t ld_rowbias, int rows_per_batch, const void* residual, int64_t ldr, float scale, int act) {
+                     const void* rowbias, int64_t ld_rowbias, int rows_per_batch, const void* residual, int64_t ldr, float scale, int act, void* row_stats = nullptr) {
     const GnTarget gn = grab_gn_target(ctx);
     FIE_REQUIRE(ctx && A1 && Wpacked && C, "%s: NULL ctx/A1/W/C", who);
     FIE_REQUIRE(M > 0 && N > 0 && K > 0, "%s: bad shape M=%d N=%d K=%d", who, M, N, K);
@@ -1172,7 +1208,32 @@
     a.a2_bytes = A2 ? ((int64_t)(M - 1) * lda2 + (K - K1)) * 2 : 0;
     a.w_bytes = fie_roundup(N, 128) * ldw * (w_scale ? 1 : 2);
     if (int rc = take_gn_target(who, gn, a)) return rc;
+    if (row_stats) {
+        FIE_REQUIRE(act != FIE_ACT_GEGLU && N <= 4096 && (reinterpret_cast<uintptr_t>(row_stats) & 15) == 0, "%s: row statistics: no GEGLU, N <= 4096 (the sum of squares must not wrap), table 16-byte aligned", who);
+        a.A3 = static_cast<const half_t*>(row_stats);
+    }
     return launch<0>(ctx, a);
+}
+
+int fie_gemm_stats_f16(fie_ctx* ctx, const void* A1, int64_t lda1, int K1, const void* A2, int64_t lda2, const void* Wpacked, int64_t ldw, void* C, int64_t ldc, int M, int N,
+                       int K, const void* bias, const void* rowbias, int64_t ld_rowbias, int rows_per_batch, const void* residual, int64_t ldr, float scale, int act,
+                       void* row_stats) {
+    FIE_REQUIRE(row_stats != nullptr, "fie_gemm_stats_f16: row_stats is NULL (fie_gemm_f16 is the entry without)");
+    return gemm_impl("fie_gemm_stats_f16", ctx, A1, lda1, K1, A2, lda2, Wpacked, ldw, nullptr, C, ldc, M, N, K, bias, rowbias, ld_rowbias, rows_per_batch, residual, ldr,
+                     scale, act, row_stats);
+}
+
+__global__ void row_stats_clear_kernel(u32x4* p, int64_t n16) {
+    for (int64_t i = blockIdx.x * (int64_t)blockDim.x + threadIdx.x; i < n16; i += (int64_t)gridDim.x * blockDim.x) p[i] = (u32x4){0u, 0u, 0u, 0u};
+}
+
+int fie_row_stats_clear(fie_ctx* ctx, void* row_stats, int64_t rows) {
+    FIE_REQUIRE(ctx && row_stats && rows > 0 && (reinterpret_cast<uintptr_t>(row_stats) & 15) == 0, "fie_row_stats_clear: bad argument");
+    FIE_DESC(ctx, "row_stats_clear rows=%lld", (long long)rows);
+    const int64_t blocks = (rows + 255) / 256;
+    fie_launch(ctx, row_stats_clear_kernel, dim3((unsigned)(blocks < 1024 ? blocks : 1024)), dim3(256), 0, static_cast<u32x4*>(row_stats), rows);
+    FIE_LAUNCH_CHECK();
+    return FIE_OK;
 }
 
 int fie_gemm_f16(fie_ctx* ctx, const void* A1, int64_t lda1, int K1, const void* A2, int64_t lda2,
@@ -1183,8 +1244,8 @@
                      rows_per_batch, residual, ldr, scale, act);
 }
 
-int fie_gemm_ln_f16(fie_ctx* ctx, const void* X, int64_t ldx, const void* Wfolded, int64_t ldw, const float* ln_tab, float eps, void* C, int64_t ldc,
-                    int M, int N, int K, int act) {
+static int gemm_ln_impl(fie_ctx* ctx, const void* X, int64_t ldx, const void* Wfolded, int64_t ldw, const float* ln_tab, float eps, void* C, int64_t ldc,
+                        int M, int N, int K, int act, const void* row_stats) {
     const GnTarget gn = grab_gn_target(ctx);
     (void)gn;
     FIE_REQUIRE(ctx && X && Wfolded && ln_tab && C, "fie_gemm_ln_f16: NULL ctx/X/W/ln_tab/C");
@@ -1201,7 +1262,19 @@
     a.a1_bytes = ((int64_t)(M - 1) * ldx + K) * 2;
     a.w_bytes = fie_roundup(N, 128) * ldw * 2;
     a.ln_tab = ln_tab; a.ln_eps = eps;
+    a.gna_tab = static_cast<const float*>(row_stats);
     return launch<0>(ctx, a);
+}
+
+int fie_gemm_ln_f16(fie_ctx* ctx, const void* X, int64_t ldx, const void* Wfolded, int64_t ldw, const float* ln_tab, float eps, void* C, int64_t ldc,
+                    int M, int N, int K, int act) {
+    return gemm_ln_impl(ctx, X, ldx, Wfolded, ldw, ln_tab, eps, C, ldc, M, N, K, act, nullptr);
+}
+
+int fie_gemm_ln_stats_f16(fie_ctx* ctx, const void* X, int64_t ldx, const void* Wfolded, int64_t ldw, const float* ln_tab, float eps, void* C, int64_t ldc,
+                          int M, int N, int K, int act, const void* row_stats) {
+    FIE_REQUIRE(row_stats != nullptr && (reinterpret_cast<uintptr_t>(row_stats) & 15) == 0, "fie_gemm_ln_stats_f16: row_stats is NULL or not 16-byte aligned");
+    return gemm_ln_impl(ctx, X, ldx, Wfolded, ldw, ln_tab, eps, C, ldc, M, N, K, act, row_stats);
 }
 
 int fie_gemm_w8_f16(fie_ctx* ctx, const void* A1, int64_t lda1, int K1, const void* A2, int64_t lda2, const void* W8packed,
diff --git a/fast-image-editing-with-generative-models_amd/hip.py b/fast-image-editing-with-generative-models_amd/hip.py
--- a/fast-image-editing-with-generative-models_amd/hip.py
+++ b/fast-image-editing-with-generative-models_amd/hip.py
@@ -61,6 +61,24 @@
     if geglu:
         tab = torch.stack([tab[: n // 2], tab[n // 2:]], 1).reshape(n, 2)
     return wf, tab.contiguous()
+
+
+ROW_STATS_SUM_BITS, ROW_STATS_SQ_BITS, ROW_STATS_SQ_CLAMP = 24, 28, 2048.0
+
+
+def row_stats_encode(x):
+    v = x.detach().to("cpu", torch.float64).clamp(-65504.0, 65504.0)
+    s = (v * 2.0 ** ROW_STATS_SUM_BITS).to(torch.int64).sum(1)
+    c = v.clamp(-ROW_STATS_SQ_CLAMP, ROW_STATS_SQ_CLAMP)
+    q = torch.round(c * c * 2.0 ** ROW_STATS_SQ_BITS).to(torch.int64).sum(1)
+    return torch.stack([s, q], 1)
+
+
+def row_stats_decode(tab, k, eps=1e-5):
+    t = tab.detach().to("cpu")
+    mean = t[:, 0].to(torch.float64) / (2.0 ** ROW_STATS_SUM_BITS * k)
+    var = (t[:, 1].to(torch.float64) / (2.0 ** ROW_STATS_SQ_BITS * k) - mean * mean).clamp_min(0.0)
+    return mean, 1.0 / torch.sqrt(var + eps)
 
 
 def _chk(rc):
@@ -157,6 +175,10 @@
         self.kv_group = os.environ.get("FIE_KV_GROUP", "1") != "0"
         self.ln_fold_which = os.environ.get("FIE_LN_FOLD_WHICH", "qkv,q2")
         self.ln_fold_ff1 = os.environ.get("FIE_LN_FOLD_FF1", "0") != "0"
+        self.ln_stats = os.environ.get("FIE_LN_STATS", "1") != "0"
+        self.ln_stats_which = os.environ.get("FIE_LN_STATS_WHICH", "qkv,q2,ff1")
+        self._ln_arena = {}
+        self._ln_cur = None
         self.conv_plus_shortcut = os.environ.get("FIE_CONV_PLUS", "1") != "0"
         self._resize_tables = {}
         self.ws_tag = 0
@@ -407,8 +429,33 @@
         self._gn_gen += 1
         return (buf, groups, n, rows_per_image, b, self._gn_gen, key, pgroups)
 
+    def ln_stats_begin(self, rows):
+        if not self.ln_stats or not self.ln_fold or self.f32 or rows <= 0 or self._ln_cur is not None:
+            return False
+        self.sync_stream()
+        buf = self._scratch(self._ln_arena, (self._stream, self.ws_tag), rows * 16)
+        if self._keep is not None:
+            self._keep.append(buf)
+        tab = buf[:rows * 16].view(torch.int64).view(rows, 2)
+        _chk(lib().fie_row_stats_clear(self.h, _p(tab), rows))
+        self._ln_cur = [tab, 0]
+        return True
+
+    def ln_stats_end(self):
+        self._ln_cur = None
+
+    def _ln_stats_take(self, m):
+        cur = self._ln_cur
+        if cur is not None and cur[1] + m <= cur[0].shape[0]:
+            tab = cur[0][cur[1]:cur[1] + m]
+            cur[1] += m
+            return tab
+        tab = self._alloc((m, 2), torch.int64)
+        _chk(lib().fie_row_stats_clear(self.h, _p(tab), m))
+        return tab
+
     def gemm(self, a, wp, n, out=None, a2=None, bias=None, rowbias=None, rows_per_batch=0, residual=None, scale=1.0,
-             act=ACT_NONE, k=None, gn_stats=None, a_scale=1.0, out_f8=False, out_inv_scale=1.0):
+             act=ACT_NONE, k=None, gn_stats=None, a_scale=1.0, out_f8=False, out_inv_scale=1.0, row_stats=False):
         self.sync_stream()
         self._bind_splitk()
         m, k1 = a.shape
@@ -436,11 +483,21 @@
                                        residual.stride(0) if residual is not None else 0, float(scale), act))
             return out
         tag = self._gn_stats_arm(m, n, gn_stats[0], gn_stats[1]) if gn_stats and act != ACT_GEGLU and out.stride(0) == n else None
+        if row_stats and act != ACT_GEGLU and n <= 4096:
+            tab = self._ln_stats_take(m)
+            _chk(lib().fie_gemm_stats_f16(self.h, _p(a), a.stride(0), k1, _p(a2), a2.stride(0) if a2 is not None else 0,
+                                          _p(wp), wp.stride(0), _p(out), out.stride(0), m, n, ktot, _p(bias), _p(rowbias),
+                                          rowbias.stride(0) if rowbias is not None else 0, rows_per_batch, _p(residual),
+                                          residual.stride(0) if residual is not None else 0, float(scale), act, _p(tab)))
+            out._gn_tag = tag
+            out._ln_stats = tab
+            return out
         _chk(lib().fie_gemm_f16(self.h, _p(a), a.stride(0), k1, _p(a2), a2.stride(0) if a2 is not None else 0,
                                 _p(wp), wp.stride(0), _p(out), out.stride(0), m, n, ktot, _p(bias), _p(rowbias),
                                 rowbias.stride(0) if rowbias is not None else 0, rows_per_batch, _p(residual),
                                 residual.stride(0) if residual is not None else 0, float(scale), act))
         out._gn_tag = tag
+        out._ln_stats = None
         return out
 
     def gemm_f32(self, a, wp, n, out=None, a2=None, bias=None, rowbias=None, rows_per_batch=0, residual=None, scale=1.0, act=ACT_NONE):
@@ -461,13 +518,18 @@
         wf, tab = fold_layernorm_tables(dev(w), dev(bias), dev(gamma), dev(beta), geglu=geglu)
         return self.pack_linear(wf, geglu=geglu, quant=False), tab
 
-    def gemm_ln(self, x, wp, n, tab, eps=1e-5, act=ACT_NONE, out=None):
+    def gemm_ln(self, x, wp, n, tab, eps=1e-5, act=ACT_NONE, out=None, stats=None):
         self.sync_stream()
         m, k = x.shape
         nout = n // 2 if act == ACT_GEGLU else n
         if out is None:
             out = self._alloc((m, nout))
         assert x.stride(1) == 1 and out.stride(1) == 1 and tab.dtype == torch.float32 and tab.shape == (n, 2) and not self.f32
+        if stats is not None:
+            assert stats.dtype == torch.int64 and stats.shape == (m, 2) and stats.is_contiguous()
+            _chk(lib().fie_gemm_ln_stats_f16(self.h, _p(x), x.stride(0), _p(wp), wp.stride(0), _p(tab), float(eps), _p(out), out.stride(0), m, n, k, act, _p(stats)))
+            out._gn_tag = None
+            return out
         _chk(lib().fie_gemm_ln_f16(self.h, _p(x), x.stride(0), _p(wp), wp.stride(0), _p(tab), float(eps), _p(out), out.stride(0), m, n, k, act))
         out._gn_tag = None
         return out
diff --git a/fast-image-editing-with-generative-models_amd/nn.py b/fast-image-editing-with-generative-models_amd/nn.py
--- a/fast-image-editing-with-generative-models_amd/nn.py
+++ b/fast-image-editing-with-generative-models_amd/nn.py
@@ -26,10 +26,10 @@
         self.a8 = isinstance(self.wp, hip.W8) and ctx.a8 and self.wp.stride(0) % 128 == 0 and self.k % 16 == 0
 
     def __call__(self, ctx, a, a2=None, residual=None, act=None, scale=1.0, out=None, rowbias=None, rows_per_batch=0, gn_stats=None,
-                 a_scale=1.0, out_f8=False, out_inv_scale=1.0):
+                 a_scale=1.0, out_f8=False, out_inv_scale=1.0, row_stats=False):
         return ctx.gemm(a, self.wp, self.n, a2=a2, bias=self.b, residual=residual, scale=scale, out=out,
                         act=self.act if act is None else act, rowbias=rowbias, rows_per_batch=rows_per_batch, gn_stats=gn_stats,
-                        a_scale=a_scale, out_f8=out_f8, out_inv_scale=out_inv_scale)
+                        a_scale=a_scale, out_f8=out_f8, out_inv_scale=out_inv_scale, row_stats=row_stats)
 
 
 class Conv3:
@@ -176,7 +176,13 @@
         f = self.ff1(ctx, y, a_scale=s[4], out_f8=True, out_inv_scale=1.0 / s[5])
         return self.ff2(ctx, f, residual=h, a_scale=s[5])
 
-    def __call__(self, ctx, h, text, batch, tokens, text_len):
+    def stats_sites(self, ctx):
+        if self.folded is None or not ctx.ln_fold or not ctx.ln_stats or self.a8 or ctx.calib:
+            return set()
+        on = {s for s in ("qkv", "q2", "ff1") if s in ctx.ln_stats_which}
+        return {s for s in on if s == "ff1" or s in ctx.ln_fold_which}
+
+    def __call__(self, ctx, h, text, batch, tokens, text_len, next_stats=False):
         am = self.amax if ctx.calib and self.a8 else None
         if self.a8 and am is None:
             return self._call_a8(ctx, h, text, batch, tokens, text_len)
@@ -185,15 +191,21 @@
         if self.folded is not None and ctx.ln_fold and am is None:
             (wq, tq), (w2, t2), (wf, tf) = self.folded
             which = ctx.ln_fold_which
-            qkv = ctx.gemm_ln(h, wq, 3 * c, tq) if "qkv" in which else self.qkv(ctx, ctx.layernorm(h, self.ln[0].g, self.ln[0].b))
+            sites = self.stats_sites(ctx)
+            st = getattr(h, "_ln_stats", None) if "qkv" in sites else None
+            qkv = ctx.gemm_ln(h, wq, 3 * c, tq, stats=st) if "qkv" in which else self.qkv(ctx, ctx.layernorm(h, self.ln[0].g, self.ln[0].b))
             a = ctx.attention(qkv[:, :c], qkv[:, c:2 * c], qkv[:, 2 * c:], self.heads, self.hd, tokens, tokens, batch)
-            h = self.o1(ctx, a, residual=h)
-            q = ctx.gemm_ln(h, w2, c, t2) if "q2" in which else self.q2(ctx, ctx.layernorm(h, self.ln[1].g, self.ln[1].b))
+            h = self.o1(ctx, a, residual=h, row_stats="q2" in sites)
+            q = ctx.gemm_ln(h, w2, c, t2, stats=getattr(h, "_ln_stats", None)) if "q2" in which else self.q2(ctx, ctx.layernorm(h, self.ln[1].g, self.ln[1].b))
             kv = self._text_kv(ctx, text)[:batch * text_len]
             a = ctx.attention(q, kv[:, :c], kv[:, c:], self.heads, self.hd, tokens, text_len, batch)
-            h = self.o2(ctx, a, residual=h)
-            f = ctx.gemm_ln(h, wf, 8 * c, tf, act=hip.ACT_GEGLU) if ctx.ln_fold_ff1 else self.ff1(ctx, ctx.layernorm(h, self.ln[2].g, self.ln[2].b))
-            return self.ff2(ctx, f, residual=h)
+            h = self.o2(ctx, a, residual=h, row_stats="ff1" in sites)
+            st = getattr(h, "_ln_stats", None)
+            if st is not None or ctx.ln_fold_ff1:
+                f = ctx.gemm_ln(h, wf, 8 * c, tf, act=hip.ACT_GEGLU, stats=st)
+            else:
+                f = self.ff1(ctx, ctx.layernorm(h, self.ln[2].g, self.ln[2].b))
+            return self.ff2(ctx, f, residual=h, row_stats=next_stats)
         y = ctx.layernorm(h, self.ln[0].g, self.ln[0].b)
         rec(y, 0)
         qkv = self.qkv(ctx, y)
@@ -225,13 +237,17 @@
         b, hh, ww, c = x.shape
         xt = x.view(b * hh * ww, c)
         h = ctx.groupnorm(x, self.norm.g, self.norm.b, self.groups, 1e-6, False).view(b * hh * ww, c)
-        h = self.pin(ctx, h)
-        for blk in self.blocks:
-            h = blk(ctx, h, text, b, hh * ww, text_len)
+        want = ["qkv" in blk.stats_sites(ctx) for blk in self.blocks] + [False]
+        h = self.pin(ctx, h, row_stats=want[0])
+        for i, blk in enumerate(self.blocks):
+            h = blk(ctx, h, text, b, hh * ww, text_len, next_stats=want[i + 1])
         o = self.pout(ctx, h, residual=xt, gn_stats=(hh * ww, self.groups))
         y = o.view(b, hh, ww, c)
         y._gn_tag = getattr(o, "_gn_tag", None)
         return y
+
+    def stats_tables(self, ctx):
+        return sum(len(blk.stats_sites(ctx)) for blk in self.blocks)
 
     def reset(self):
         for blk in self.blocks:
@@ -338,7 +354,24 @@
         semb = self.t2(ctx, self.t1(ctx, s, act=hip.ACT_SILU), rowbias=add_emb, rows_per_batch=1, act=hip.ACT_SILU)
         return self.temb_proj(ctx, semb)
 
+    def _ln_rows_encode(self, x):
+        b, h, w, _ = x.shape
+        rows = 0
+        for layers, ds in self.down:
+            rows += sum(t.stats_tables(self.ctx) * b * h * w for _, t in layers if t)
+            if ds is not None:
+                h, w = (h + 1) // 2, (w + 1) // 2
+        return rows + sum(t.stats_tables(self.ctx) * b * h * w for _, t in self.mid if t)
+
     def encode(self, x, temb_all, text, text_len):
+        opened = self.ctx.ln_stats_begin(self._ln_rows_encode(x))
+        try:
+            return self._encode(x, temb_all, text, text_len)
+        finally:
+            if opened:
+                self.ctx.ln_stats_end()
+
+    def _encode(self, x, temb_all, text, text_len):
         ctx = self.ctx
         skips = [x]
         for layers, ds in self.down:
@@ -384,6 +417,19 @@
                     yield t
 
     def decode(self, x, skips, temb_all, text, text_len):
+        sk, rows = list(skips), 0
+        for layers, _ in self.up:
+            for _, t in layers:
+                s = sk.pop()
+                rows += t.stats_tables(self.ctx) * s.shape[0] * s.shape[1] * s.shape[2] if t else 0
+        opened = self.ctx.ln_stats_begin(rows)
+        try:
+            return self._decode(x, skips, temb_all, text, text_len)
+        finally:
+            if opened:
+                self.ctx.ln_stats_end()
+
+    def _decode(self, x, skips, temb_all, text, text_len):
         ctx, cfg = self.ctx, self.cfg
         skips = list(skips)
         for layers, us in self.up:
diff --git a/include/fie.h b/include/fie.h
--- a/include/fie.h
+++ b/include/fie.h
@@ -113,6 +113,14 @@
 int fie_gemm_ln_f16(fie_ctx* ctx, const void* X, int64_t ldx, const void* Wfolded, int64_t ldw, const float* ln_tab, float eps, void* C, int64_t ldc,
                     int M, int N, int K, int act);
 
+int fie_gemm_stats_f16(fie_ctx* ctx, const void* A1, int64_t lda1, int K1, const void* A2, int64_t lda2,
+                       const void* Wpacked, int64_t ldw, void* C, int64_t ldc, int M, int N, int K,
+                       const void* bias, const void* rowbias, int64_t ld_rowbias, int rows_per_batch,
+                       const void* residual, int64_t ldr, float scale, int act, void* row_stats);
+int fie_gemm_ln_stats_f16(fie_ctx* ctx, const void* X, int64_t ldx, const void* Wfolded, int64_t ldw, const float* ln_tab, float eps, void* C, int64_t ldc,
+                          int M, int N, int K, int act, const void* row_stats);
+int fie_row_stats_clear(fie_ctx* ctx, void* row_stats, int64_t rows);
+
 int fie_conv3x3_nhwc_f16(fie_ctx* ctx, const void* X, int B, int H, int W, int Cin, int upsample2x, int stride,
                          int pad_mode, const void* Wpacked, int64_t ldw, void* Y, int64_t ldc, int Cout,
                          const void* bias, const void* rowbias, int64_t ld_rowbias,
```
